# isunLt/U2MKD

Measured on AMD Instinct MI355X. Metric: LiDAR points/sec/node fwd+bwd (teacher+student+KD), 1/2/4/8 MI355X, higher is better.
Workload: dtype f32 (fp32 products emulated on the 16-bit matrix pipe: f16x2 forward / input gradient, bf16x3 weight gradient; fp32 accumulate)

## Files before the change

include/u2mkd_hip.h:

```cpp
#ifndef U2MKD_HIP_H
#define U2MKD_HIP_H

#include <stddef.h>
#include <stdint.h>

#ifdef __cplusplus
extern "C" {
#endif

typedef void *u2mkd_stream_t;

int u2mkd_version(void);
const char *u2mkd_last_error(void);
int u2mkd_stream_wait_stream(u2mkd_stream_t waiter, u2mkd_stream_t signaler);
void *u2mkd_mailbox_alloc(size_t bytes);
int u2mkd_mailbox_free(void *p);
int u2mkd_mailbox_post(const void *const *srcs, uint32_t is64, int32_t n, int64_t *slot, int64_t seq, u2mkd_stream_t s);

int u2mkd_hash(const int32_t *coords , int64_t n, int64_t *out , u2mkd_stream_t s);
int u2mkd_kernel_hash(const int32_t *coords , const int32_t *offsets , int64_t n,
                      int32_t k, int64_t *out , u2mkd_stream_t s);

size_t u2mkd_hash_table_bytes(int64_t n_refs);
int u2mkd_hash_table_build(const int64_t *refs, int64_t n_refs, void *table, u2mkd_stream_t s);
// ... 52 lines not shown
                                const int32_t *n_items, int64_t n_out, int32_t k, int32_t kflip, int32_t arith,
                                const float *scale , const float *shift , const float *res ,
                                int32_t relu, float *out, u2mkd_stream_t s);
int32_t u2mkd_pairs_gather_sum_stats_slab_rows(void);
int32_t u2mkd_pairs_gather_sum_stats_supported(int32_t cout);
int u2mkd_pairs_gather_sum_stats(const float *y, const int32_t *pos, int64_t n_rows, int32_t k, int32_t cout, float *out,
                                 float *partial, u2mkd_stream_t s);
int u2mkd_pairs_gather_sum_ep(const float *y, const int32_t *pos, int64_t n_rows, int32_t k, int32_t cout, const float *scale,
                              const float *shift, const float *res, int32_t relu, float *out, u2mkd_stream_t s);
int u2mkd_debug_conv_forward_sorted(const float *in, int64_t n_in, int32_t cin, const float *wt, int32_t cout,
                                    const int32_t *nbr_sorted, const int32_t *order, const int32_t *tile_order,
                                    int64_t n_out, int32_t k, int32_t kflip, int32_t variant, float *out,
                                    u2mkd_stream_t s);
int u2mkd_debug_conv_tile_pairs_stamps(const float *in, int64_t n_in, const void *wf ,
                                       const int32_t *nbr_sorted, const int32_t *order, const int32_t *items,
                                       const int32_t *n_items, int64_t n_out, int32_t k, int32_t arith, float *out,
                                       uint64_t *stamps, u2mkd_stream_t s);
int u2mkd_debug_wgrad_stamps(const float *a, const float *b, const int32_t *pairs, const int32_t *plan, int64_t n_rows,
                             int32_t k, void *workspace, uint64_t *stamps, u2mkd_stream_t s);
int u2mkd_conv_forward_pairs(const float *in, int64_t n_in, int32_t cin, const float *wt, int32_t cout,
                             const int32_t *pair_idx, const int32_t *tile_k, const int32_t *meta, int64_t capacity,
                             int32_t k, int32_t kc, float *y , u2mkd_stream_t s);
int32_t u2mkd_conv_pairs_x3_supported(int32_t cin, int32_t cout);
int u2mkd_conv_forward_pairs_x3(const float *in, int64_t n_in, int32_t cin, const void *wf, int32_t cout,
                                const int32_t *pair_idx, const int32_t *tile_k, const int32_t *meta, int64_t capacity,
                                int32_t k, float *y , u2mkd_stream_t s);
int u2mkd_linear_forward(const float *x , int64_t n, int32_t cin, const float *w , int32_t cout,
                         const float *bias , int32_t kc, float *y, u2mkd_stream_t s);
int u2mkd_linear_forward_x3(const float *x , int64_t n, int32_t cin, const void *wf, int32_t cout,
                            const float *bias , float *y , u2mkd_stream_t s);
int32_t u2mkd_conv_pairs_f16x2_supported(int32_t cin, int32_t cout);
int u2mkd_conv_forward_pairs_f16x2(const float *in, int64_t n_in, int32_t cin, const void *wf, int32_t cout,
                                    const int32_t *pair_idx, const int32_t *tile_k, const int32_t *meta, int64_t capacity,
                                    int32_t k, float *y, u2mkd_stream_t s);
int u2mkd_linear_forward_f16x2(const float *x, int64_t n, int32_t cin, const void *wf, int32_t cout, const float *bias,
                               float *y, u2mkd_stream_t s);
int u2mkd_pairs_gather_sum(const float *y, const int32_t *pos , int64_t n_rows, int32_t k, int32_t cout,
                           float *out , u2mkd_stream_t s);
int u2mkd_kmap_rowmask(const int32_t *nbr , int64_t n_out, int32_t k, int32_t *mask ,
                       u2mkd_stream_t s);
int u2mkd_conv_forward_tiles_bf16(const void *in , int64_t n_in, int32_t cin, const void *wf, int32_t cout,
                                  const int32_t *nbr_sorted, const int32_t *order, const int32_t *items,
                                  const int32_t *n_items, int64_t n_out, int32_t k, int32_t kflip,
                                  void *out , u2mkd_stream_t s);
int u2mkd_conv_wgrad_pairs_bf16(const void *a , int32_t ca, const void *b , int32_t cb,
                                const int32_t *pairs, const int32_t *plan, int64_t n_rows, int32_t k, int32_t swap,
                                void *workspace, size_t workspace_bytes, float *dw , u2mkd_stream_t s);
int u2mkd_conv_forward_tiles_f16(const void *in , int64_t n_in, int32_t cin, const void *wf, int32_t cout,
                                 const int32_t *nbr_sorted, const int32_t *order, const int32_t *items,
                                 const int32_t *n_items, int64_t n_out, int32_t k, int32_t kflip,
                                 void *out , u2mkd_stream_t s);
int u2mkd_conv_wgrad_pairs_f16(const void *a , int32_t ca, const void *b , int32_t cb,
                               const int32_t *pairs, const int32_t *plan, int64_t n_rows, int32_t k, int32_t swap,
                               void *workspace, size_t workspace_bytes, float *dw , u2mkd_stream_t s);
int u2mkd_conv_forward_pairs_f16(const void *in , int64_t n_in, int32_t cin, const void *wf, int32_t cout,
                                  const int32_t *pair_idx, const int32_t *tile_k, const int32_t *meta, int64_t capacity,
                                  int32_t k, void *y , u2mkd_stream_t s);
int u2mkd_linear_forward_f16(const void *x , int64_t n, int32_t cin, const void *wf, int32_t cout,
                             const float *bias , void *y , u2mkd_stream_t s);
int u2mkd_pairs_gather_sum_f16(const void *y , const int32_t *pos , int64_t n_rows, int32_t k,
                               int32_t cout, void *out , u2mkd_stream_t s);
int u2mkd_conv_forward_pairs_bf16(const void *in , int64_t n_in, int32_t cin, const void *wf, int32_t cout,
                                   const int32_t *pair_idx, const int32_t *tile_k, const int32_t *meta, int64_t capacity,
                                   int32_t k, void *y , u2mkd_stream_t s);
int u2mkd_linear_forward_bf16(const void *x , int64_t n, int32_t cin, const void *wf, int32_t cout,
                              const float *bias , void *y , u2mkd_stream_t s);
int u2mkd_pairs_gather_sum_bf16(const void *y , const int32_t *pos , int64_t n_rows, int32_t k,
                                int32_t cout, void *out , u2mkd_stream_t s);
size_t u2mkd_tile_schedule_workspace_bytes(int64_t n_rows);
int u2mkd_tile_schedule(const int32_t *mask , const int32_t *order , int64_t n_rows,
                        int32_t k, int32_t split0, int32_t split1, void *workspace, int32_t *tile_order,
                        int32_t *items, int32_t *n_items, u2mkd_stream_t s);
int32_t u2mkd_wgrad_plan_ints(int32_t k);
int u2mkd_wgrad_plan(const int32_t *nbsizes , int32_t k, int64_t n_rows, int32_t *plan, u2mkd_stream_t s);
size_t u2mkd_conv_wgrad_pairs_workspace_bytes(int64_t n_rows, int32_t ca, int32_t cb, int32_t k);
int u2mkd_conv_wgrad_pairs(const float *a, int32_t ca, const float *b, int32_t cb, const int32_t *pairs ,
                           const int32_t *plan, int64_t n_rows, int32_t k, int32_t swap, void *workspace,
                           size_t workspace_bytes, float *dw , u2mkd_stream_t s);

size_t u2mkd_convolution_workspace_bytes(int64_t n_in_rows, int64_t n_out_rows, int32_t cin, int32_t cout,
                                         const int32_t *nbsizes_host , int32_t k);
int u2mkd_convolution_forward(const float *in_feat , int64_t n_in_rows, int32_t cin,
                              float *out_feat , int64_t n_out_rows, int32_t cout,
                              const float *kernel , const int32_t *nbmaps ,
                              const int32_t *nbsizes_host , int32_t k, int32_t transpose, void *workspace,
                              size_t workspace_bytes, u2mkd_stream_t s);
int u2mkd_convolution_backward(const float *in_feat , int64_t n_in_rows, int32_t cin,
                               float *grad_in_feat , const float *grad_out_feat ,
                               int64_t n_out_rows, int32_t cout, const float *kernel ,
                               float *grad_kernel , const int32_t *nbmaps, const int32_t *nbsizes_host,
                               int32_t k, int32_t transpose, void *workspace, size_t workspace_bytes, u2mkd_stream_t s);

int u2mkd_count(const int32_t *idx , int64_t n, int32_t *counts , int64_t num,
                u2mkd_stream_t s);
int u2mkd_voxelize_forward(const float *feats , const int32_t *idx , const int32_t *counts ,
                           int64_t n, int64_t nv, int32_t c, float *out , u2mkd_stream_t s);
int u2mkd_voxelize_backward(const float *grad_out , const int32_t *idx, const int32_t *counts, int64_t n,
                            int64_t nv, int32_t c, float *grad_feats , u2mkd_stream_t s);
int u2mkd_devoxelize_forward(const float *feats , const int32_t *idx , const float *w ,
                             int64_t n, int32_t c, float *out , u2mkd_stream_t s);
int u2mkd_devoxelize_backward(const float *grad_out , const int32_t *idx , const float *w ,
                              int64_t n, int64_t nv, int32_t c, float *grad_feats ,
                              u2mkd_stream_t s);
int u2mkd_segment_sum(const float *src , int32_t c, const int32_t *entry_row ,
                      const float *entry_w , const int32_t *seg_offsets , int64_t nv,
                      int32_t mean, float *out , u2mkd_stream_t s);
int u2mkd_voxelize_backward_bf16(const void *grad_out , const int32_t *idx, const int32_t *counts, int64_t n,
                                 int64_t nv, int32_t c, void *grad_feats , u2mkd_stream_t s);
int u2mkd_devoxelize_forward_bf16(const void *feats , const int32_t *idx , const float *w ,
                                  int64_t n, int32_t c, void *out , u2mkd_stream_t s);
int u2mkd_segment_sum_bf16(const void *src , int32_t c, const int32_t *entry_row ,
                           const float *entry_w , const int32_t *seg_offsets , int64_t nv,
                           int32_t mean, void *out , u2mkd_stream_t s);
int u2mkd_voxelize_backward_f16(const void *grad_out , const int32_t *idx, const int32_t *counts, int64_t n,
                                int64_t nv, int32_t c, void *grad_feats , u2mkd_stream_t s);
int u2mkd_devoxelize_forward_f16(const void *feats , const int32_t *idx , const float *w ,
                                 int64_t n, int32_t c, void *out , u2mkd_stream_t s);
int u2mkd_segment_sum_f16(const void *src , int32_t c, const int32_t *entry_row ,
                          const float *entry_w , const int32_t *seg_offsets , int64_t nv,
                          int32_t mean, void *out , u2mkd_stream_t s);
size_t u2mkd_csr_workspace_bytes(int64_t n_entries, int64_t nv);
int u2mkd_csr_build(const int32_t *keys , int64_t n_entries, int64_t nv, void *workspace,
                    int32_t *order , int32_t *seg , u2mkd_stream_t s);
size_t u2mkd_devoxelize_plan_workspace_bytes(int64_t n, int64_t nv);
int u2mkd_devoxelize_plan(const int32_t *idx8 , const float *w8 , int64_t n, int64_t nv, void *workspace,
                          int32_t *entry_row , float *entry_w , int32_t *seg , u2mkd_stream_t s);
int u2mkd_ti_weights(const float *coords , const int64_t *idx_kn , int64_t n,
                     float scale, float *w_n8 , int32_t *idx_n8 , u2mkd_stream_t s);

int u2mkd_up_plan(const int32_t *idx8 , int64_t n, int32_t H, int32_t W, int32_t h, int32_t w, float rh, float rw,
                  int32_t *idx_out , float *w_out , u2mkd_stream_t s);
int u2mkd_upbn_stats(const float *x, int32_t n_img, int32_t c, int32_t h, int32_t w, const float *a, const float *b,
                     const float *ay, const float *ax, int32_t rows_per_chunk, float *partial, u2mkd_stream_t s);
int u2mkd_upbn_dense_grad(const float *x, int32_t n_img, int32_t c, int32_t h, int32_t w, const float *a, const float *b,
                          const float *ay, const float *ax, const float *c0 , const float *c1 ,
                          int32_t rows_per_chunk, float *dx, u2mkd_stream_t s);

int u2mkd_up_bilinear_forward(const float *x, const float *skip , int64_t planes, int32_t h, int32_t w, int32_t H,
                              int32_t W, float rh, float rw, float *y, u2mkd_stream_t s);
int u2mkd_up_bilinear_backward(const float *g, int64_t planes, int32_t h, int32_t w, int32_t H, int32_t W, const int32_t *taps_y,
                               const float *wy, const int32_t *taps_x, const float *wx, int32_t tiled, float *dx, u2mkd_stream_t s);

int u2mkd_maxpool3s2_forward(const float *x, int64_t planes, int32_t h, int32_t w, float *y, uint8_t *code, u2mkd_stream_t s);
int u2mkd_maxpool3s2_backward(const float *dy, const uint8_t *code, int64_t planes, int32_t h, int32_t w, float *dx,
                              u2mkd_stream_t s);

int u2mkd_transpose_batched(const float *in, float *out, int32_t batch, int32_t rows, int32_t cols, u2mkd_stream_t s);
int u2mkd_transpose_batched_scaled(const float *in, float *out, int32_t batch, int32_t rows, int32_t cols, float scale,
                                   u2mkd_stream_t s);

int u2mkd_l2c_combine_forward(const float *g0, const float *g1, const float *g2, const float *g3, int32_t n_grids, int32_t n_img,
                              int32_t h, int32_t w, int32_t c, int32_t ch1, int32_t cw1, int32_t ch2, int32_t cw2, int32_t ch3,
                              int32_t cw3, float *out_rows, u2mkd_stream_t s);
int u2mkd_l2c_combine_backward(const float *g_rows, int32_t n_img, int32_t h, int32_t w, int32_t c, int32_t ch, int32_t cw,
                               float *d_grid, u2mkd_stream_t s);

int32_t u2mkd_select_mse_partials(void);
int u2mkd_select_mse_forward(const float *gathered, const float *pseudo, const uint8_t *fov, int64_t n, int32_t c, float *out,
                             float *partial, float *stats, u2mkd_stream_t s);
int u2mkd_select_mse_backward(const float *g_out, const float *g_loss, const float *stats, const float *gathered,
                              const float *pseudo, const uint8_t *fov, int64_t n, int32_t c, float *d_gathered, float *d_pseudo,
                              u2mkd_stream_t s);
int u2mkd_lovasz_errors(const float *probas, const int64_t *labels, int32_t ignore_index, int64_t n, int32_t c, float *errors,
                        double *keys, u2mkd_stream_t s);
int u2mkd_lovasz_gather(const int64_t *perm, const int64_t *labels, int32_t ignore_index, int64_t n, int32_t c,
                        int32_t *fg_sorted, u2mkd_stream_t s);
int64_t u2mkd_lovasz_partials(int64_t n, int32_t c);
int u2mkd_lovasz_terms(const int64_t *perm, const float *errors, const int64_t *csum, const int32_t *fg_sorted, int64_t n,
                       int32_t c, float *jgrad, float *partial, float *stats, u2mkd_stream_t s);
int u2mkd_lovasz_backward(const float *g_out, const float *stats, const int64_t *perm, const float *jgrad, const float *probas,
                          const int64_t *labels, int32_t ignore_index, int64_t n, int32_t c, float *d_probas, u2mkd_stream_t s);
int64_t u2mkd_ce_partials(int64_t n);
int u2mkd_ce_forward(const float *x, const int64_t *labels, int32_t ignore_index, int64_t n, int32_t c, float *lse, float *partial,
                     float *stats, u2mkd_stream_t s);
int u2mkd_ce_backward(const float *g_out, const float *stats, const float *x, const float *lse, const int64_t *labels,
                      int32_t ignore_index, int64_t n, int32_t c, float *dx, u2mkd_stream_t s);
int u2mkd_kl_forward(const float *s_logits, const float *t_logits, const int64_t *t_index, int64_t n, int32_t c, float *rows,
                     float *partial, float *stats, u2mkd_stream_t s);
int u2mkd_kl_backward(const float *g_out, const float *s_logits, const float *t_logits, const int64_t *t_index, const float *rows,
                      int64_t n, int32_t c, float *ds, u2mkd_stream_t s);
int u2mkd_c2l_plan(const float *pixel_coords, const uint8_t *mask, int32_t ncam, int64_t n, int32_t sample, int32_t h,
                   int32_t w, int32_t *idx8 , float *w8 , u2mkd_stream_t s);
int u2mkd_l2c_keys(const float *pixel_coords, const uint8_t *mask, int32_t ncam, int64_t n, int32_t sample, int64_t row0,
                   int64_t e0, int32_t ch, int32_t cw, int32_t *pix, int32_t *key_d, int32_t *key_s, int32_t *row,
                   u2mkd_stream_t s);
int u2mkd_l2c_finish(const int32_t *order_d, const int32_t *seg_d, const int32_t *order_s, const int32_t *pix,
                     const int32_t *row, int64_t n_entries, int32_t *fwd_row, float *fwd_w, int32_t *bwd_pix, float *bwd_w,
                     u2mkd_stream_t s);

int64_t u2mkd_bn_num_slabs(int64_t n);
int u2mkd_bn_train_forward(const void *x, const void *res, int32_t row_dtype, int64_t n, int32_t c, const float *gamma,
                           const float *beta, float eps, float momentum, float *running_mean, float *running_var,
                           int64_t *num_batches_tracked, int32_t relu, float *partial, float *mean ,
                           float *invstd , void *y, u2mkd_stream_t s);
int u2mkd_bn_train_forward_from_partial(const float *x, const float *res, int64_t n, int32_t c, const float *gamma,
                                        const float *beta, float eps, float momentum, float *running_mean, float *running_var,
                                        int64_t *num_batches_tracked, int32_t relu, const float *partial, int32_t slab_rows,
                                        float *mean , float *invstd , float *y, u2mkd_stream_t s);
int u2mkd_bn_eval_forward(const void *x, const void *res, int32_t row_dtype, int64_t n, int32_t c, const float *gamma,
                          const float *beta, float eps, const float *running_mean, const float *running_var, int32_t relu,
                          float *invstd , void *y, u2mkd_stream_t s);
int u2mkd_bn_backward(const void *dy, const void *x, const void *res, int32_t row_dtype, int64_t n, int32_t c,
                      const float *mean, const float *invstd, const float *gamma, const float *beta, int32_t relu,
                      int32_t training, float *partial, float *dgamma , float *dbeta , void *dx, void *dres,
                      u2mkd_stream_t s);

int u2mkd_bn_local_stats(const void *x, int32_t row_dtype, int64_t n, int32_t c, float *partial ,
                         float *stats , u2mkd_stream_t s);
int u2mkd_bn_merge_stats(const float *gathered , int32_t world, int32_t c, float eps, float momentum,
                         float *running_mean, float *running_var, float *mean , float *invstd ,
                         float *total , int64_t *num_batches_tracked, u2mkd_stream_t s);
int u2mkd_bn_apply(const void *x, const void *res, int32_t row_dtype, int64_t n, int32_t c, const float *mean,
                   const float *invstd, const float *gamma, const float *beta, int32_t relu, void *y, u2mkd_stream_t s);
int u2mkd_bn_backward_local(const void *dy, const void *x, const void *res, int32_t row_dtype, int64_t n, int32_t c,
                            const float *mean, const float *invstd, const float *gamma, const float *beta, int32_t relu,
                            float *partial , float *sums , float *keep ,
                            u2mkd_stream_t s);
int u2mkd_bn_backward_apply(const void *dy, const void *x, const void *res, int32_t row_dtype, int64_t n, int32_t c,
                            const float *total_n , const float *mean, const float *invstd, const float *gamma,
                            const float *beta, int32_t relu, const float *sums , void *dx, void *dres,
                            u2mkd_stream_t s);

int u2mkd_sptr_window_keys(const float *xyz , const int32_t *batch , int64_t n, const float *lo4,
                           const float *hi4, float sx, float sy, float sz, int64_t *keys , u2mkd_stream_t s);
size_t u2mkd_sptr_plan_prepare_workspace_bytes(void);
int u2mkd_sptr_plan_prepare(const float *xyz , const int32_t *batch , int64_t n, float cx, float cy, float cz,
                            float sx, float sy, float sz, float *sphere, float *bounds, int64_t *keys_cubic,
                            int64_t *keys_sphere, void *workspace, u2mkd_stream_t s);
int u2mkd_sptr_window_ranges(const int64_t *sorted_keys, int64_t n, int32_t *wstart , int32_t *wlen ,
                             u2mkd_stream_t s);
int u2mkd_sptr_quant_coords(const float *xyz , const int32_t *sort_idx , int64_t n, const float *lo,
                            float wx, float wy, float wz, float qx, float qy, float qz, int32_t *qc ,
                            float *radial , u2mkd_stream_t s);
int u2mkd_sptr_attention_forward(const float *q, const float *k, const float *v, const int32_t *sort_idx,
                                 const int32_t *wstart, const int32_t *wlen, const int32_t *qc, const float *radial,
                                 const float *tq, const float *tk, const float *tv, int32_t L, int32_t qgl,
                                 float split_a, int64_t n, int32_t h, int32_t hdim, float *out, float *lse,
                                 u2mkd_stream_t s);
size_t u2mkd_sptr_backward_workspace_bytes(int64_t n, int32_t h, int32_t L);
int u2mkd_sptr_attention_backward(const float *q, const float *k, const float *v, const float *out, const float *dout,
                                  const float *lse, const int32_t *sort_idx, const int32_t *wstart,
                                  const int32_t *wlen, const int32_t *qc, const float *radial, const float *tq,
                                  const float *tk, const float *tv, int32_t L, int32_t qgl, float split_a,
                                  int32_t qc_span, int64_t n, int32_t h, int32_t hdim, float *delta ,
                                  void *workspace, size_t workspace_bytes, float *dq, float *dk, float *dv, float *dtq,
                                  float *dtk, float *dtv, u2mkd_stream_t s);
int u2mkd_sptr_attention_forward_strided(const float *q, const float *k, const float *v, int64_t ld_qkv, float q_scale,
                                         const int32_t *sort_idx, const int32_t *wstart, const int32_t *wlen,
                                         const int32_t *qc, const float *radial, const float *tq, const float *tk,
                                         const float *tv, int32_t L, int32_t qgl, float split_a, int64_t n, int32_t h,
                                         int32_t hdim, float *out, int64_t ld_out, float *lse, u2mkd_stream_t s);
int u2mkd_sptr_attention_backward_strided(const float *q, const float *k, const float *v, int64_t ld_qkv, float q_scale,
                                          const float *out, const float *dout, int64_t ld_out, const float *lse,
                                          const int32_t *sort_idx, const int32_t *wstart, const int32_t *wlen,
                                          const int32_t *qc, const float *radial, const float *tq, const float *tk,
                                          const float *tv, int32_t L, int32_t qgl, float split_a, int32_t qc_span,
                                          int64_t n, int32_t h, int32_t hdim, float *delta ,
                                          void *workspace, size_t workspace_bytes, float *dq, float *dk, float *dv,
                                          int64_t ld_grad, float *dtq, float *dtk, float *dtv, u2mkd_stream_t s);

int u2mkd_sptr_table_reduce(const void *workspace, int64_t n, int32_t h, int32_t L, float split_a, float *dtq, float *dtk,
                            float *dtv, u2mkd_stream_t s);

int u2mkd_sptr_precompute_all(int32_t N, int32_t n, uint32_t n_max, const int32_t *counts, const int32_t *offsets,
                              const int32_t *sq_offsets, int32_t *index_0_offsets, int32_t *index_1_offsets,
                              int32_t *index_0, int32_t *index_1, u2mkd_stream_t s);
int u2mkd_sptr_attention_step1_forward(int32_t N_q, int32_t N_k, int32_t M, int32_t h, int32_t hdim, uint32_t n_max,
                                       const float *q, const float *k, const int32_t *index0, const int32_t *index1,
                                       float *attn, u2mkd_stream_t s);
int u2mkd_sptr_attention_step1_backward(int32_t N, int32_t M, int32_t h, int32_t hdim, uint32_t n_max,
                                        const float *grad_out, const int32_t *index0, const int32_t *index0_offsets,
                                        const int32_t *index1, const int32_t *index1_offsets, const float *q,
                                        const float *k, float *grad_q, float *grad_k, u2mkd_stream_t s);
int u2mkd_sptr_attention_step2_forward(int32_t N, int32_t M, int32_t h, int32_t hdim, int32_t n_max, const float *attn,
                                       const float *v, const int32_t *index0_offsets, const int32_t *index1,
                                       float *output, u2mkd_stream_t s);
int u2mkd_sptr_attention_step2_backward(int32_t N, int32_t M, int32_t h, int32_t hdim, int32_t n_max,
                                        const float *grad_out, const int32_t *index0, const int32_t *index0_offsets,
                                        const int32_t *index1, const int32_t *index1_offsets, const float *attn,
                                        const float *v, float *grad_attn, float *grad_v, u2mkd_stream_t s);
int u2mkd_sptr_dot_prod_with_idx_forward(int32_t N, int32_t M, int32_t h, int32_t hdim, int32_t n_max, int32_t L,
                                         const float *q, const int32_t *index_q, const int32_t *index_q_offsets,
                                         const float *k, const int32_t *index_k, const float *table_q,
                                         const float *table_k, const int32_t *rel_idx, float *output,
                                         u2mkd_stream_t s);
int u2mkd_sptr_dot_prod_with_idx_all_forward(int32_t N, int32_t M, int32_t h, int32_t hdim, int32_t n_max, int32_t L,
                                             const float *q, const int32_t *index_q, const int32_t *index_q_offsets,
                                             const float *k, const int32_t *index_k, const float *table_q,
                                             const float *table_k, const int32_t *rel_idx, float *output,
                                             u2mkd_stream_t s);
int u2mkd_sptr_dot_prod_with_idx_backward(int32_t N, int32_t M, int32_t h, int32_t hdim, int32_t n_max, int32_t L,
                                          const float *grad_out, const float *q, const int32_t *index_q_offsets,
                                          const float *k, const int32_t *index_k_offsets, const int32_t *index_k,
                                          const float *table_q, const float *table_k, const int32_t *rel_idx,
                                          float *grad_q, float *grad_k, float *grad_table_q, float *grad_table_k,
                                          u2mkd_stream_t s);
int u2mkd_sptr_attention_step2_with_rel_pos_value_forward(int32_t N, int32_t M, int32_t h, int32_t hdim, int32_t n_max,
                                                          const float *attn, const float *v,
                                                          const int32_t *index0_offsets, const int32_t *index1,
                                                          const float *table, const int32_t *rel_idx, float *output,
                                                          u2mkd_stream_t s);
int u2mkd_sptr_attention_step2_with_rel_pos_value_backward(int32_t N, int32_t M, int32_t h, int32_t hdim, int32_t L,
                                                           int32_t n_max, const float *grad_out, const int32_t *index0,
                                                           const int32_t *index0_offsets, const int32_t *index1,
                                                           const int32_t *index1_offsets, const float *attn,
                                                           const float *v, const float *table, const int32_t *rel_idx,
                                                           float *grad_attn, float *grad_v, float *grad_table,
                                                           u2mkd_stream_t s);
// ... 47 lines not shown
```

u2mkd_amd/_lib.py:

```python
from __future__ import annotations

import ctypes as C
import os

import torch

_HERE = os.path.dirname(os.path.abspath(__file__))
LIB_PATH = os.path.join(_HERE, 'lib', 'libu2mkd_hip%s.so' % os.environ.get('U2MKD_LIB_SUFFIX', ''))

_i32, _i64, _sz, _f32, _p = C.c_int32, C.c_int64, C.c_size_t, C.c_float, C.c_void_p

SIGNATURES = {
    'u2mkd_version': (C.c_int, []),
    'u2mkd_last_error': (C.c_char_p, []),
    'u2mkd_hash': (C.c_int, [_p, _i64, _p, _p]),
    'u2mkd_kernel_hash': (C.c_int, [_p, _p, _i64, _i32, _p, _p]),
    'u2mkd_hash_table_bytes': (_sz, [_i64]),
    'u2mkd_hash_table_build': (C.c_int, [_p, _i64, _p, _p]),
    'u2mkd_hash_table_query': (C.c_int, [_p, _i64, _p, _i64, _p, _p]),
    'u2mkd_hash_table_query2': (C.c_int, [_p, _i64, _p, _i64, _p, _p, _p]),
    'u2mkd_kmap_build_table': (C.c_int, [_p, _i64, _p, _i64, _p, _i32, _p, _p]),
    'u2mkd_kmap_invert': (C.c_int, [_p, _i64, _i32, _i64, _p, _p]),
    'u2mkd_kmap_sizes': (C.c_int, [_p, _i64, _i32, _p, _p, _p]),
    'u2mkd_kmap_compact': (C.c_int, [_p, _i64, _i32, _p, _p, _p, _p]),
    'u2mkd_downsample_keys': (C.c_int, [_p, _i64, _i32, _i32, _i32, _p, _p]),
    'u2mkd_downsample_keys_checked': (C.c_int, [_p, _i64, _i32, _i32, _i32, _p, _p, _p]),
    'u2mkd_downsample_keys_general': (C.c_int, [_p, _i64] + [_i32] * 9 + [_p, _i32, _p, _p, _p]),
    'u2mkd_floor_coords': (C.c_int, [_p, _i64, _i32, _p, _p]),
    'u2mkd_unpack_keys': (C.c_int, [_p, _i64, _p, _p]),
    'u2mkd_transpose_weights': (C.c_int, [_p, _i32, _i32, _i32, _p, _p]),
    'u2mkd_conv_forward': (C.c_int, [_p, _i64, _i32, _p, _i32, _p, _i64, _i32, _i32, _p, _p]),
    'u2mkd_conv_forward_sorted': (C.c_int, [_p, _i64, _i32, _p, _i32, _p, _p, _p, _i64, _i32, _i32, _p, _p]),
    'u2mkd_debug_conv_forward_sorted': (C.c_int, [_p, _i64, _i32, _p, _i32, _p, _p, _p, _i64, _i32, _i32, _i32, _p, _p]),
    'u2mkd_stream_wait_stream': (C.c_int, [_p, _p]),
    'u2mkd_sgd_chunk_elements': (_i32, []),
    'u2mkd_sgd_batch': (C.c_int, [_p, _i32, _i64, _f32, _f32, _f32, _i32, _i32, _p]),
    'u2mkd_grads_unscale_check': (C.c_int, [_p, _i32, _i64, _p, _p, _p]),
    'u2mkd_sgd_batch_amp': (C.c_int, [_p, _i32, _i64, _f32, _f32, _f32, _i32, _i32, _p, _p, _p]),
    'u2mkd_mailbox_alloc': (_p, [_sz]),
    'u2mkd_mailbox_free': (C.c_int, [_p]),
    'u2mkd_mailbox_post': (C.c_int, [_p, C.c_uint32, _i32, _p, _i64, _p]),
    'u2mkd_conv_tiles_supported': (_i32, [_i32, _i32, _i32]),
    'u2mkd_conv_tiles_arith': (_i32, [_i32, _i32, _i32]),
    'u2mkd_weight_fragments_bytes': (_sz, [_i32, _i32, _i32, _i32]),
    'u2mkd_weight_fragments': (C.c_int, [_p, _i32, _i32, _i32, _i32, _i32, _p, _p]),
    'u2mkd_weight_fragments_batch': (C.c_int, [_p, _i32, _i64, _p]),
    'u2mkd_conv_forward_tiles': (C.c_int, [_p, _i64, _i32, _p, _i32, _p, _p, _p, _p, _i64, _i32, _i32, _i32, _p, _p]),
    'u2mkd_conv_forward_tiles_ep': (C.c_int, [_p, _i64, _i32, _p, _i32, _p, _p, _p, _p, _i64, _i32, _i32, _i32, _p, _p, _p, _i32, _p, _p]),
    'u2mkd_pairs_gather_sum_ep': (C.c_int, [_p, _p, _i64, _i32, _i32, _p, _p, _p, _i32, _p, _p]),
    'u2mkd_pairs_gather_sum_stats_slab_rows': (_i32, []),
    'u2mkd_pairs_gather_sum_stats_supported': (_i32, [_i32]),
    'u2mkd_pairs_gather_sum_stats': (C.c_int, [_p, _p, _i64, _i32, _i32, _p, _p, _p]),
    'u2mkd_debug_conv_tile_pairs_stamps': (C.c_int, [_p, _i64, _p, _p, _p, _p, _p, _i64, _i32, _i32, _p, _p, _p]),
    'u2mkd_debug_wgrad_stamps': (C.c_int, [_p, _p, _p, _p, _i64, _i32, _p, _p, _p]),
    'u2mkd_conv_forward_pairs': (C.c_int, [_p, _i64, _i32, _p, _i32, _p, _p, _p, _i64, _i32, _i32, _p, _p]),
    'u2mkd_conv_pairs_x3_supported': (_i32, [_i32, _i32]),
    'u2mkd_conv_forward_pairs_x3': (C.c_int, [_p, _i64, _i32, _p, _i32, _p, _p, _p, _i64, _i32, _p, _p]),
    'u2mkd_linear_forward': (C.c_int, [_p, _i64, _i32, _p, _i32, _p, _i32, _p, _p]),
    'u2mkd_bn2d_workspace_bytes': (C.c_size_t, [_i64, _i32, _i64]),
    'u2mkd_bn2d_train_forward': (C.c_int, [_p, _p, _i64, _i32, _i64, _p, _p, C.c_float, C.c_float, _i32, _p, _p, _p, _p, _p, _p, _p, _p]),
    'u2mkd_bn2d_eval_forward': (C.c_int, [_p, _p, _i64, _i32, _i64, _p, _p, C.c_float, _i32, _p, _p, _p, _p]),
    'u2mkd_bn2d_backward': (C.c_int, [_p, _p, _p, _i64, _i32, _i64, _p, _p, _p, _p, _i32, _i32, _p, _p, _p, _p, _p, _p]),
    'u2mkd_bn2d_local_stats': (C.c_int, [_p, _i64, _i32, _i64, _p, _p, _p]),
    'u2mkd_bn2d_apply': (C.c_int, [_p, _p, _i64, _i32, _i64, _p, _p, _p, _p, _i32, _p, _p]),
    'u2mkd_bn2d_backward_local': (C.c_int, [_p, _p, _p, _i64, _i32, _i64, _p, _p, _p, _p, _i32, _p, _p, _p, _p]),
    'u2mkd_bn2d_backward_apply': (C.c_int, [_p, _p, _p, _i64, _i32, _i64, _p, _p, _p, _p, _p, _i32, _p, _p, _p, _p]),
    'u2mkd_linear_forward_x3': (C.c_int, [_p, _i64, _i32, _p, _i32, _p, _p, _p]),
    'u2mkd_conv_pairs_f16x2_supported': (_i32, [_i32, _i32]),
    'u2mkd_conv_forward_pairs_f16x2': (C.c_int, [_p, _i64, _i32, _p, _i32, _p, _p, _p, _i64, _i32, _p, _p]),
    'u2mkd_linear_forward_f16x2': (C.c_int, [_p, _i64, _i32, _p, _i32, _p, _p, _p]),
    'u2mkd_pairs_capacity': (_i64, [_i64, _i64, _i32]),
    'u2mkd_pairs_build': (C.c_int, [_p, _i64, _i64, _i32, _p, _p, _p, _p, _p, _p, _p, _p, _p]),
    'u2mkd_pairs_gather_sum': (C.c_int, [_p, _p, _i64, _i32, _i32, _p, _p]),
    'u2mkd_kmap_rowmask': (C.c_int, [_p, _i64, _i32, _p, _p]),
    'u2mkd_tile_schedule_workspace_bytes': (_sz, [_i64]),
    'u2mkd_tile_schedule': (C.c_int, [_p, _p, _i64, _i32, _i32, _i32, _p, _p, _p, _p, _p]),
    'u2mkd_wgrad_plan_ints': (_i32, [_i32]),
    'u2mkd_wgrad_plan': (C.c_int, [_p, _i32, _i64, _p, _p]),
    'u2mkd_conv_wgrad_pairs_workspace_bytes': (_sz, [_i64, _i32, _i32, _i32]),
    'u2mkd_conv_wgrad_pairs': (C.c_int, [_p, _i32, _p, _i32, _p, _p, _i64, _i32, _i32, _p, _sz, _p, _p]),
    'u2mkd_conv_forward_tiles_bf16': (C.c_int, [_p, _i64, _i32, _p, _i32, _p, _p, _p, _p, _i64, _i32, _i32, _p, _p]),
    'u2mkd_conv_forward_tiles_f16': (C.c_int, [_p, _i64, _i32, _p, _i32, _p, _p, _p, _p, _i64, _i32, _i32, _p, _p]),
    'u2mkd_conv_wgrad_pairs_bf16': (C.c_int, [_p, _i32, _p, _i32, _p, _p, _i64, _i32, _i32, _p, _sz, _p, _p]),
    'u2mkd_conv_wgrad_pairs_f16': (C.c_int, [_p, _i32, _p, _i32, _p, _p, _i64, _i32, _i32, _p, _sz, _p, _p]),
    'u2mkd_conv_forward_pairs_bf16': (C.c_int, [_p, _i64, _i32, _p, _i32, _p, _p, _p, _i64, _i32, _p, _p]),
    'u2mkd_conv_forward_pairs_f16': (C.c_int, [_p, _i64, _i32, _p, _i32, _p, _p, _p, _i64, _i32, _p, _p]),
    'u2mkd_linear_forward_bf16': (C.c_int, [_p, _i64, _i32, _p, _i32, _p, _p, _p]),
    'u2mkd_linear_forward_f16': (C.c_int, [_p, _i64, _i32, _p, _i32, _p, _p, _p]),
    'u2mkd_pairs_gather_sum_bf16': (C.c_int, [_p, _p, _i64, _i32, _i32, _p, _p]),
    'u2mkd_pairs_gather_sum_f16': (C.c_int, [_p, _p, _i64, _i32, _i32, _p, _p]),
    'u2mkd_convolution_workspace_bytes': (_sz, [_i64, _i64, _i32, _i32, _p, _i32]),
    'u2mkd_convolution_forward': (C.c_int, [_p, _i64, _i32, _p, _i64, _i32, _p, _p, _p, _i32, _i32, _p, _sz, _p]),
    'u2mkd_convolution_backward': (C.c_int, [_p, _i64, _i32, _p, _p, _i64, _i32, _p, _p, _p, _p, _i32, _i32, _p, _sz, _p]),
    'u2mkd_bn_num_slabs': (_i64, [_i64]),
    'u2mkd_bn_train_forward': (C.c_int, [_p, _p, _i32, _i64, _i32, _p, _p, _f32, _f32, _p, _p, _p, _i32, _p, _p, _p, _p, _p]),
    'u2mkd_bn_train_forward_from_partial': (C.c_int, [_p, _p, _i64, _i32, _p, _p, _f32, _f32, _p, _p, _p, _i32, _p, _i32, _p, _p, _p, _p]),
    'u2mkd_bn_eval_forward': (C.c_int, [_p, _p, _i32, _i64, _i32, _p, _p, _f32, _p, _p, _i32, _p, _p, _p]),
    'u2mkd_bn_backward': (C.c_int, [_p, _p, _p, _i32, _i64, _i32, _p, _p, _p, _p, _i32, _i32, _p, _p, _p, _p, _p, _p]),
    'u2mkd_bn_local_stats': (C.c_int, [_p, _i32, _i64, _i32, _p, _p, _p]),
    'u2mkd_bn_merge_stats': (C.c_int, [_p, _i32, _i32, _f32, _f32, _p, _p, _p, _p, _p, _p, _p]),
    'u2mkd_bn_apply': (C.c_int, [_p, _p, _i32, _i64, _i32, _p, _p, _p, _p, _i32, _p, _p]),
    'u2mkd_bn_backward_local': (C.c_int, [_p, _p, _p, _i32, _i64, _i32, _p, _p, _p, _p, _i32, _p, _p, _p, _p]),
    'u2mkd_bn_backward_apply': (C.c_int, [_p, _p, _p, _i32, _i64, _i32, _p, _p, _p, _p, _p, _i32, _p, _p, _p, _p]),
    'u2mkd_sptr_window_keys': (C.c_int, [_p, _p, _i64, _p, _p, _f32, _f32, _f32, _p, _p]),
    'u2mkd_select_mse_partials': (_i32, []),
    'u2mkd_select_mse_forward': (C.c_int, [_p, _p, _p, _i64, _i32, _p, _p, _p, _p]),
    'u2mkd_select_mse_backward': (C.c_int, [_p, _p, _p, _p, _p, _p, _i64, _i32, _p, _p, _p]),
    'u2mkd_sptr_plan_prepare_workspace_bytes': (_sz, []),
    'u2mkd_sptr_plan_prepare': (C.c_int, [_p, _p, _i64, _f32, _f32, _f32, _f32, _f32, _f32, _p, _p, _p, _p, _p, _p]),
    'u2mkd_sptr_window_ranges': (C.c_int, [_p, _i64, _p, _p, _p]),
    'u2mkd_sptr_quant_coords': (C.c_int, [_p, _p, _i64, _p, _f32, _f32, _f32, _f32, _f32, _f32, _p, _p, _p]),
    'u2mkd_sptr_attention_forward': (C.c_int, [_p, _p, _p, _p, _p, _p, _p, _p, _p, _p, _p, _i32, _i32, _f32, _i64, _i32, _i32, _p, _p, _p]),
    'u2mkd_sptr_backward_workspace_bytes': (_sz, [_i64, _i32, _i32]),
    'u2mkd_sptr_attention_backward': (C.c_int, [_p] * 14 + [_i32, _i32, _f32, _i32, _i64, _i32, _i32] + [_p, _p, _sz] + [_p] * 7),
    'u2mkd_sptr_tiles_workspace_bytes': (_sz, [_i64, _i32]),
    'u2mkd_sptr_attention_forward_tiles': (C.c_int, [_p, _p, _p, _i64, _f32] + [_p] * 8 + [_i32, _i32, _f32, _i64, _i32, _i32, _p, _i64, _p, _p, _sz, _p]),
    'u2mkd_sptr_attention_forward_strided': (C.c_int, [_p, _p, _p, _i64, _f32] + [_p] * 8 + [_i32, _i32, _f32, _i64, _i32, _i32, _p, _i64, _p, _p]),
    'u2mkd_sptr_attention_backward_strided': (C.c_int, [_p, _p, _p, _i64, _f32, _p, _p, _i64] + [_p] * 9 + [_i32, _i32, _f32, _i32, _i64, _i32, _i32]
                                              + [_p, _p, _sz] + [_p, _p, _p, _i64, _p, _p, _p, _p]),
    'u2mkd_sptr_table_reduce': (C.c_int, [_p, _i64, _i32, _i32, _f32, _p, _p, _p, _p]),
    'u2mkd_sptr_precompute_all': (C.c_int, [_i32, _i32, C.c_uint32] + [_p] * 8),
    'u2mkd_sptr_attention_step1_forward': (C.c_int, [_i32, _i32, _i32, _i32, _i32, C.c_uint32] + [_p] * 6),
    'u2mkd_sptr_attention_step1_backward': (C.c_int, [_i32, _i32, _i32, _i32, C.c_uint32] + [_p] * 10),
    'u2mkd_sptr_attention_step2_forward': (C.c_int, [_i32] * 5 + [_p] * 6),
    'u2mkd_sptr_attention_step2_backward': (C.c_int, [_i32] * 5 + [_p] * 10),
    'u2mkd_sptr_dot_prod_with_idx_forward': (C.c_int, [_i32] * 6 + [_p] * 10),
    'u2mkd_sptr_dot_prod_with_idx_all_forward': (C.c_int, [_i32] * 6 + [_p] * 10),
    'u2mkd_sptr_dot_prod_with_idx_backward': (C.c_int, [_i32] * 6 + [_p] * 14),
    'u2mkd_sptr_attention_step2_with_rel_pos_value_forward': (C.c_int, [_i32] * 5 + [_p] * 8),
    'u2mkd_sptr_attention_step2_with_rel_pos_value_backward': (C.c_int, [_i32] * 6 + [_p] * 13),
    'u2mkd_count': (C.c_int, [_p, _i64, _p, _i64, _p]),
    'u2mkd_voxelize_forward': (C.c_int, [_p, _p, _p, _i64, _i64, _i32, _p, _p]),
    'u2mkd_voxelize_backward': (C.c_int, [_p, _p, _p, _i64, _i64, _i32, _p, _p]),
    'u2mkd_devoxelize_forward': (C.c_int, [_p, _p, _p, _i64, _i32, _p, _p]),
    'u2mkd_devoxelize_backward': (C.c_int, [_p, _p, _p, _i64, _i64, _i32, _p, _p]),
    'u2mkd_segment_sum': (C.c_int, [_p, _i32, _p, _p, _p, _i64, _i32, _p, _p]),
    'u2mkd_voxelize_backward_bf16': (C.c_int, [_p, _p, _p, _i64, _i64, _i32, _p, _p]),
    'u2mkd_voxelize_backward_f16': (C.c_int, [_p, _p, _p, _i64, _i64, _i32, _p, _p]),
    'u2mkd_devoxelize_forward_bf16': (C.c_int, [_p, _p, _p, _i64, _i32, _p, _p]),
    'u2mkd_devoxelize_forward_f16': (C.c_int, [_p, _p, _p, _i64, _i32, _p, _p]),
    'u2mkd_segment_sum_bf16': (C.c_int, [_p, _i32, _p, _p, _p, _i64, _i32, _p, _p]),
    'u2mkd_segment_sum_f16': (C.c_int, [_p, _i32, _p, _p, _p, _i64, _i32, _p, _p]),
    'u2mkd_c2l_plan': (C.c_int, [_p, _p, _i32, _i64, _i32, _i32, _i32, _p, _p, _p]),
    'u2mkd_l2c_keys': (C.c_int, [_p, _p, _i32, _i64, _i32, _i64, _i64, _i32, _i32, _p, _p, _p, _p, _p]),
    'u2mkd_l2c_finish': (C.c_int, [_p, _p, _p, _p, _p, _i64, _p, _p, _p, _p, _p]),
    'u2mkd_up_bilinear_forward': (C.c_int, [_p, _p, _i64, _i32, _i32, _i32, _i32, _f32, _f32, _p, _p]),
    'u2mkd_up_bilinear_backward': (C.c_int, [_p, _i64, _i32, _i32, _i32, _i32, _p, _p, _p, _p, _i32, _p, _p]),
    'u2mkd_maxpool3s2_forward': (C.c_int, [_p, _i64, _i32, _i32, _p, _p, _p]),
    'u2mkd_maxpool3s2_backward': (C.c_int, [_p, _p, _i64, _i32, _i32, _p, _p]),
    'u2mkd_transpose_batched': (C.c_int, [_p, _p, _i32, _i32, _i32, _p]),
    'u2mkd_transpose_batched_scaled': (C.c_int, [_p, _p, _i32, _i32, _i32, C.c_float, _p]),
    'u2mkd_l2c_combine_forward': (C.c_int, [_p, _p, _p, _p] + [_i32] * 11 + [_p, _p]),
    'u2mkd_l2c_combine_backward': (C.c_int, [_p] + [_i32] * 6 + [_p, _p]),
    'u2mkd_up_plan': (C.c_int, [_p, _i64, _i32, _i32, _i32, _i32, _f32, _f32, _p, _p, _p]),
    'u2mkd_upbn_stats': (C.c_int, [_p, _i32, _i32, _i32, _i32, _p, _p, _p, _p, _i32, _p, _p]),
    'u2mkd_upbn_dense_grad': (C.c_int, [_p, _i32, _i32, _i32, _i32, _p, _p, _p, _p, _p, _p, _i32, _p, _p]),
    'u2mkd_csr_workspace_bytes': (_sz, [_i64, _i64]),
    'u2mkd_lovasz_errors': (C.c_int, [_p, _p, _i32, _i64, _i32, _p, _p, _p]),
    'u2mkd_lovasz_gather': (C.c_int, [_p, _p, _i32, _i64, _i32, _p, _p]),
    'u2mkd_lovasz_partials': (_i64, [_i64, _i32]),
    'u2mkd_lovasz_terms': (C.c_int, [_p, _p, _p, _p, _i64, _i32, _p, _p, _p, _p]),
    'u2mkd_ce_partials': (_i64, [_i64]),
    'u2mkd_ce_forward': (C.c_int, [_p, _p, _i32, _i64, _i32, _p, _p, _p, _p]),
    'u2mkd_ce_backward': (C.c_int, [_p, _p, _p, _p, _p, _i32, _i64, _i32, _p, _p]),
    'u2mkd_kl_forward': (C.c_int, [_p, _p, _p, _i64, _i32, _p, _p, _p, _p]),
    'u2mkd_kl_backward': (C.c_int, [_p, _p, _p, _p, _p, _i64, _i32, _p, _p]),
    'u2mkd_lovasz_backward': (C.c_int, [_p, _p, _p, _p, _p, _p, _i32, _i64, _i32, _p, _p]),
    'u2mkd_csr_build': (C.c_int, [_p, _i64, _i64, _p, _p, _p, _p]),
    'u2mkd_devoxelize_plan_workspace_bytes': (C.c_size_t, [_i64, _i64]),
    'u2mkd_devoxelize_plan': (C.c_int, [_p, _p, _i64, _i64, _p, _p, _p, _p, _p]),
    'u2mkd_ti_weights': (C.c_int, [_p, _p, _i64, _f32, _p, _p, _p]),
}

_lib = None
_raw_stream = torch._C._cuda_getCurrentRawStream
_current_device = torch._C._cuda_getDevice


def load():
    global _lib
    if _lib is not None:
        return _lib
    if not os.path.exists(LIB_PATH):
        raise RuntimeError(
            f'{LIB_PATH} is missing: build it with `python -m u2mkd_amd.build` '
            '(u2mkd_amd has no CPU or PyTorch fallback path)')
    lib = C.CDLL(LIB_PATH)
    for name, (res, args) in SIGNATURES.items():
        fn = getattr(lib, name)
        fn.restype = res
        fn.argtypes = args
    _lib = lib
    return lib


def stream() -> int:
    return _raw_stream(_current_device())


def ptr(t):
    if t is None:
        return None
    return t.data_ptr()


_fns = {}


def call(name: str, *args):
    fn = _fns.get(name)
    if fn is None:
        fn = _fns[name] = getattr(load(), name)
    rc = fn(*args)
    if rc != 0:
        msg = load().u2mkd_last_error().decode('utf-8', 'replace')
        raise RuntimeError(f'{name} failed (rc={rc}): {msg}')


def require_cuda(*tensors):
    for t in tensors:
        if t is not None and not t.is_cuda:
            raise RuntimeError('u2mkd_amd operators run on the HIP device only (got a CPU tensor); '
                               'there is no CPU fallback')
```

u2mkd_amd/csrc/bn.hip:

```cpp
#include "common.h"

#include <cstdlib>

namespace u2mkd {

constexpr int kBnThreads = 256;
constexpr int kBnSlabRows = 128;

struct BnLayout {
    int c4, rl;
};
__device__ __forceinline__ BnLayout bn_layout(int c) {
    BnLayout l;
    l.c4 = c >> 2;
    l.rl = kBnThreads / l.c4;
    if (l.rl < 1) l.rl = 1;
    return l;
}

constexpr int kBnRegRows = 16;

template <typename T>
__global__ void __launch_bounds__(kBnThreads)
bn_stats_partial_reg_kernel(const T *__restrict__ x, int64_t n, int c, float *__restrict__ partial) {
// ... 244 lines not shown
    const int nloop = (c4 + kBnThreads - 1) / kBnThreads;
    const int64_t r0 = (int64_t)blockIdx.x * kBnSlabRows;
    const int rows = (int)min((int64_t)kBnSlabRows, n - r0);
    for (int it = 0; it < nloop; ++it) {
        const int rl = c4 >= kBnThreads ? 1 : kBnThreads / c4;
        const int j = c4 >= kBnThreads ? it * kBnThreads + threadIdx.x : threadIdx.x % c4;
        const int ry = c4 >= kBnThreads ? 0 : threadIdx.x / c4;
        const bool live = j < c4 && ry < rl;
        const int cw = c4 >= kBnThreads ? kBnThreads : c4;
        const int jl = c4 >= kBnThreads ? threadIdx.x : j;
        float4 s1 = make_float4(0.f, 0.f, 0.f, 0.f), s2 = s1;
        if (live) {
            float4 m = *reinterpret_cast<const float4 *>(mean + 4 * j);
            float4 is = *reinterpret_cast<const float4 *>(invstd + 4 * j);
            float4 g = gamma ? *reinterpret_cast<const float4 *>(gamma + 4 * j) : make_float4(1.f, 1.f, 1.f, 1.f);
            float4 b = beta ? *reinterpret_cast<const float4 *>(beta + 4 * j) : make_float4(0.f, 0.f, 0.f, 0.f);
            for (int rr0 = ry; rr0 < rows; rr0 += 4 * rl) {
                float4 vv[4], dd[4], rr4[4];
#pragma unroll
                for (int u = 0; u < 4; ++u) {
                    const int rr = rr0 + u * rl;
                    const bool ok = rr < rows;
                    vv[u] = ok ? ld4(x, (r0 + rr) * c4 + j) : make_float4(0.f, 0.f, 0.f, 0.f);
                    dd[u] = ok ? ld4(dy, (r0 + rr) * c4 + j) : make_float4(0.f, 0.f, 0.f, 0.f);
                    rr4[u] = (ok && relu && res) ? ld4(res, (r0 + rr) * c4 + j) : make_float4(0.f, 0.f, 0.f, 0.f);
                }
#pragma unroll
                for (int u = 0; u < 4; ++u) {
                    if (rr0 + u * rl >= rows) break;
                    const float4 v = vv[u], rv = rr4[u];
                    float4 d = dd[u];
                    float hx = (v.x - m.x) * is.x, hy = (v.y - m.y) * is.y, hz = (v.z - m.z) * is.z, hw = (v.w - m.w) * is.w;
                    if (relu) {
                        if (hx * g.x + b.x + rv.x <= 0.f) d.x = 0.f;
                        if (hy * g.y + b.y + rv.y <= 0.f) d.y = 0.f;
                        if (hz * g.z + b.z + rv.z <= 0.f) d.z = 0.f;
                        if (hw * g.w + b.w + rv.w <= 0.f) d.w = 0.f;
                    }
                    s1.x += d.x; s1.y += d.y; s1.z += d.z; s1.w += d.w;
                    s2.x += d.x * hx; s2.y += d.y * hy; s2.z += d.z * hz; s2.w += d.w * hw;
                }
            }
            red[ry * cw + jl] = s1;
            red[(rl + ry) * cw + jl] = s2;
        }
        __syncthreads();
        if (live && ry == 0) {
            float4 t1 = make_float4(0.f, 0.f, 0.f, 0.f), t2 = t1;
            for (int gq = 0; gq < rl; ++gq) {
                float4 a = red[gq * cw + jl], bq = red[(rl + gq) * cw + jl];
                t1.x += a.x; t1.y += a.y; t1.z += a.z; t1.w += a.w;
                t2.x += bq.x; t2.y += bq.y; t2.z += bq.z; t2.w += bq.w;
            }
            float *p = partial + (size_t)blockIdx.x * 2 * c;
            *reinterpret_cast<float4 *>(p + 4 * j) = t1;
            *reinterpret_cast<float4 *>(p + c + 4 * j) = t2;
        }
        __syncthreads();
    }
}

__global__ void __launch_bounds__(256)
bn_bwd_finalize_kernel(const float *__restrict__ partial, int nslab, int c, float *__restrict__ dbeta,
                       float *__restrict__ dgamma, float *__restrict__ keep = nullptr) {
    __shared__ float s_1[kBnFinLanes][kBnFinCh], s_2[kBnFinLanes][kBnFinCh];
    const int cl = threadIdx.x & (kBnFinCh - 1), g = threadIdx.x / kBnFinCh;
    const int ch = blockIdx.x * kBnFinCh + cl;
    float s1 = 0.f, s2 = 0.f;
    if (ch < c) {
        for (int b0 = g; b0 < nslab; b0 += 4 * kBnFinLanes) {
            float p1[4], p2[4];
#pragma unroll
            for (int u = 0; u < 4; ++u) {
                int b = b0 + u * kBnFinLanes;
                p1[u] = b < nslab ? partial[(size_t)b * 2 * c + ch] : 0.f;
                p2[u] = b < nslab ? partial[(size_t)b * 2 * c + c + ch] : 0.f;
            }
#pragma unroll
            for (int u = 0; u < 4; ++u) { s1 += p1[u]; s2 += p2[u]; }
        }
    }
    s_1[g][cl] = s1; s_2[g][cl] = s2;
    __syncthreads();
    if (g != 0 || ch >= c) return;
    for (int i = 1; i < kBnFinLanes; ++i) { s1 += s_1[i][cl]; s2 += s_2[i][cl]; }
    dbeta[ch] = s1;
    dgamma[ch] = s2;
    if (keep) { keep[ch] = s1; keep[c + ch] = s2; }
}

template <typename T>
__global__ void bn_bwd_apply_kernel(const T *__restrict__ dy, const T *__restrict__ x, int64_t total4, int c4,
                                    float inv_n_host, const float *__restrict__ total_n,
                                    const float *__restrict__ mean, const float *__restrict__ invstd,
                                    const float *__restrict__ gamma, const float *__restrict__ beta, int relu,
                                    const float *__restrict__ dbeta, const float *__restrict__ dgamma,
                                    T *__restrict__ dx, const T *__restrict__ res = nullptr,
                                    T *__restrict__ dres = nullptr) {
    int64_t t = (int64_t)blockIdx.x * blockDim.x + threadIdx.x;
    if (t >= total4) return;
    const float inv_n = total_n ? 1.f / *total_n : inv_n_host;
    int j = (int)(t % c4) * 4;
    float4 v = ld4(x, t);
    float4 d = ld4(dy, t);
    float4 m = *reinterpret_cast<const float4 *>(mean + j);
    float4 is = *reinterpret_cast<const float4 *>(invstd + j);
    float4 g = gamma ? *reinterpret_cast<const float4 *>(gamma + j) : make_float4(1.f, 1.f, 1.f, 1.f);
    float4 b = beta ? *reinterpret_cast<const float4 *>(beta + j) : make_float4(0.f, 0.f, 0.f, 0.f);
    float4 db = *reinterpret_cast<const float4 *>(dbeta + j);
    float4 dg = *reinterpret_cast<const float4 *>(dgamma + j);
    float hx = (v.x - m.x) * is.x, hy = (v.y - m.y) * is.y, hz = (v.z - m.z) * is.z, hw = (v.w - m.w) * is.w;
    if (relu) {
        const float4 rv = res ? ld4(res, t) : make_float4(0.f, 0.f, 0.f, 0.f);
        if (hx * g.x + b.x + rv.x <= 0.f) d.x = 0.f;
        if (hy * g.y + b.y + rv.y <= 0.f) d.y = 0.f;
        if (hz * g.z + b.z + rv.z <= 0.f) d.z = 0.f;
        if (hw * g.w + b.w + rv.w <= 0.f) d.w = 0.f;
    }
    if (dres) st4(dres, t, d);
    float4 o;
    o.x = g.x * is.x * (d.x - db.x * inv_n - hx * dg.x * inv_n);
    o.y = g.y * is.y * (d.y - db.y * inv_n - hy * dg.y * inv_n);
    o.z = g.z * is.z * (d.z - db.z * inv_n - hz * dg.z * inv_n);
    o.w = g.w * is.w * (d.w - db.w * inv_n - hw * dg.w * inv_n);
    st4(dx, t, o);
}

template <typename T>
__global__ void bn_bwd_eval_kernel(const T *__restrict__ dy, const T *__restrict__ x, int64_t total4, int c4,
                                   const float *__restrict__ mean, const float *__restrict__ invstd,
                                   const float *__restrict__ gamma, const float *__restrict__ beta, int relu,
                                   T *__restrict__ dx, const T *__restrict__ res = nullptr,
                                   T *__restrict__ dres = nullptr) {
    int64_t t = (int64_t)blockIdx.x * blockDim.x + threadIdx.x;
    if (t >= total4) return;
    int j = (int)(t % c4) * 4;
    float4 v = ld4(x, t);
    float4 d = ld4(dy, t);
    float4 m = *reinterpret_cast<const float4 *>(mean + j);
    float4 is = *reinterpret_cast<const float4 *>(invstd + j);
    float4 g = gamma ? *reinterpret_cast<const float4 *>(gamma + j) : make_float4(1.f, 1.f, 1.f, 1.f);
    float4 b = beta ? *reinterpret_cast<const float4 *>(beta + j) : make_float4(0.f, 0.f, 0.f, 0.f);
    if (relu) {
        const float4 rv = res ? ld4(res, t) : make_float4(0.f, 0.f, 0.f, 0.f);
        if ((v.x - m.x) * is.x * g.x + b.x + rv.x <= 0.f) d.x = 0.f;
        if ((v.y - m.y) * is.y * g.y + b.y + rv.y <= 0.f) d.y = 0.f;
        if ((v.z - m.z) * is.z * g.z + b.z + rv.z <= 0.f) d.z = 0.f;
        if ((v.w - m.w) * is.w * g.w + b.w + rv.w <= 0.f) d.w = 0.f;
    }
    if (dres) st4(dres, t, d);
    st4(dx, t, make_float4(d.x * g.x * is.x, d.y * g.y * is.y, d.z * g.z * is.z, d.w * g.w * is.w));
}

__global__ void bn_invstd_kernel(const float *__restrict__ var, int c, float eps, float *__restrict__ invstd) {
    int ch = blockIdx.x * blockDim.x + threadIdx.x;
    if (ch < c) invstd[ch] = 1.f / sqrtf(var[ch] + eps);
}

__global__ void bn_sync_merge_kernel(const float *__restrict__ gathered, int world, int c, float eps, float momentum,
                                     float *__restrict__ running_mean, float *__restrict__ running_var,
                                     float *__restrict__ mean_out, float *__restrict__ invstd_out,
                                     float *__restrict__ total_out, int64_t *__restrict__ num_batches_tracked = nullptr) {
    int ch = blockIdx.x * blockDim.x + threadIdx.x;
    if (num_batches_tracked && ch == 0) *num_batches_tracked += 1;
    if (ch >= c) return;
    const int row = 2 * c + 1;
    float na = 0.f, mean = 0.f, m2 = 0.f;
    for (int r = 0; r < world; ++r) {
        float nb = gathered[(size_t)r * row + 2 * c];
        if (nb == 0.f) continue;
        float mb = gathered[(size_t)r * row + ch], qb = gathered[(size_t)r * row + c + ch];
        float tot = na + nb;
        float delta = mb - mean;
        mean += delta * (nb / tot);
        m2 += qb + delta * delta * (na * nb / tot);
        na = tot;
    }
    float var = na > 0.f ? m2 / na : 0.f;
    mean_out[ch] = mean;
    invstd_out[ch] = 1.f / sqrtf(var + eps);
    if (ch == 0) *total_out = na;
    if (running_mean) {
        float unbiased = na > 1.f ? m2 / (na - 1.f) : var;
        running_mean[ch] = (1.f - momentum) * running_mean[ch] + momentum * mean;
        running_var[ch] = (1.f - momentum) * running_var[ch] + momentum * unbiased;
    }
}

static size_t bn_lds_bytes(int c, int arrays) {
    int c4 = c / 4;
    int rl = c4 >= kBnThreads ? 1 : kBnThreads / c4;
    int cw = c4 >= kBnThreads ? kBnThreads : c4;
    return (size_t)arrays * rl * cw * sizeof(float4);
}

static bool bn_stats_serial() {
    static const bool on = [] { const char *e = getenv("U2MKD_BN_STATS_SERIAL"); return e && e[0] == '1'; }();
    return on;
}

template <typename T>
static void bn_launch_stats_partial(hipStream_t st, int nslab, const T *x, int64_t n, int c, float *partial) {
    const int c4 = c / 4;
    if (c4 <= 32 && kBnSlabRows / (kBnThreads / c4) <= kBnRegRows && !bn_stats_serial())
        hipLaunchKernelGGL(bn_stats_partial_reg_kernel<T>, dim3(nslab), dim3(kBnThreads), bn_lds_bytes(c, 1), st, x, n, c, partial);
    else
        hipLaunchKernelGGL(bn_stats_partial_kernel<T>, dim3(nslab), dim3(kBnThreads), bn_lds_bytes(c, 1), st, x, n, c, partial);
}

template <typename T>
static int bn_train_forward_impl(const T *x, const T *res, int64_t n, int32_t c, const float *gamma, const float *beta,
                                 float eps, float momentum, float *running_mean, float *running_var,
                                 int64_t *num_batches_tracked, int32_t relu, float *partial, float *mean, float *invstd, T *y,
                                 u2mkd_stream_t s) {
    U2_REQUIRE(c > 0 && c % 4 == 0 && c <= 1024, "u2mkd_bn_train_forward: c=%d must be a multiple of 4 in 4..1024", c);
    U2_REQUIRE(n > 0, "u2mkd_bn_train_forward: empty batch (n=%lld)", (long long)n);
    U2_REQUIRE(x && partial && mean && invstd && y, "u2mkd_bn_train_forward: null pointer");
    hipStream_t st = as_stream(s);
    int nslab = (int)u2mkd_bn_num_slabs(n);
#ifndef U2MKD_EXP_SKIP_BN_STATS
    bn_launch_stats_partial<T>(st, nslab, x, n, c, partial);
#endif
    hipLaunchKernelGGL(bn_stats_finalize_kernel, dim3((unsigned)ceil_div(c, kBnFinCh)), dim3(256), 0, st, partial, nslab, n, c,
                       eps, momentum, running_mean, running_var, mean, invstd, (float *)nullptr, num_batches_tracked);
    int64_t total4 = n * (c / 4);
    hipLaunchKernelGGL(bn_apply_kernel<T>, dim3((unsigned)ceil_div(total4, 256)), dim3(256), 0, st, x, total4, c / 4, mean,
                       invstd, gamma, beta, relu, y, res);
    return check_launch("u2mkd_bn_train_forward");
}

static int bn_train_forward_from_partial_impl(const float *x, const float *res, int64_t n, int32_t c, const float *gamma,
                                              const float *beta, float eps, float momentum, float *running_mean,
                                              float *running_var, int64_t *num_batches_tracked, int32_t relu,
                                              const float *partial, int32_t slab_rows, float *mean, float *invstd, float *y,
                                              u2mkd_stream_t s) {
    U2_REQUIRE(c > 0 && c % 4 == 0 && c <= 1024, "u2mkd_bn_train_forward_from_partial: c=%d must be a multiple of 4 in 4..1024", c);
    U2_REQUIRE(n > 0 && slab_rows > 0, "u2mkd_bn_train_forward_from_partial: n=%lld rows in slabs of %d", (long long)n, slab_rows);
    U2_REQUIRE(x && partial && mean && invstd && y, "u2mkd_bn_train_forward_from_partial: null pointer");
    U2_REQUIRE(res == nullptr || relu, "u2mkd_bn_train_forward_from_partial: a residual input is only fused with the ReLU form");
    hipStream_t st = as_stream(s);
    const int64_t nslab = ceil_div(n, (int64_t)slab_rows);
    U2_REQUIRE(nslab < ((int64_t)1 << 31), "u2mkd_bn_train_forward_from_partial: too many slabs");
    hipLaunchKernelGGL(bn_stats_finalize_kernel, dim3((unsigned)ceil_div(c, kBnFinCh)), dim3(256), 0, st, partial, (int)nslab, n, c,
                       eps, momentum, running_mean, running_var, mean, invstd, (float *)nullptr, num_batches_tracked, (int)slab_rows);
    int64_t total4 = n * (c / 4);
    hipLaunchKernelGGL(bn_apply_kernel<float>, dim3((unsigned)ceil_div(total4, 256)), dim3(256), 0, st, x, total4, c / 4, mean,
                       invstd, gamma, beta, relu, y, res);
    return check_launch("u2mkd_bn_train_forward_from_partial");
}

template <typename T>
static int bn_eval_forward_impl(const T *x, const T *res, int64_t n, int32_t c, const float *gamma, const float *beta,
                                float eps, const float *running_mean, const float *running_var, int32_t relu, float *invstd,
                                T *y, u2mkd_stream_t s) {
    U2_REQUIRE(c > 0 && c % 4 == 0, "u2mkd_bn_eval_forward: c=%d must be a positive multiple of 4", c);
    if (n == 0) return 0;
    U2_REQUIRE(x && running_mean && running_var && invstd && y, "u2mkd_bn_eval_forward: null pointer");
    hipStream_t st = as_stream(s);
    int64_t total4 = n * (c / 4);
    hipLaunchKernelGGL(bn_apply_eval_kernel<T>, dim3((unsigned)ceil_div(total4, 256)), dim3(256), 0, st, x, total4, c / 4,
                       running_mean, running_var, eps, gamma, beta, relu, invstd, y, res);
    return check_launch("u2mkd_bn_eval_forward");
}

template <typename T>
static int bn_backward_impl(const T *dy, const T *x, const T *res, int64_t n, int32_t c, const float *mean,
                            const float *invstd, const float *gamma, const float *beta, int32_t relu, int32_t training,
                            float *partial, float *dgamma, float *dbeta, T *dx, T *dres, u2mkd_stream_t s) {
    U2_REQUIRE(c > 0 && c % 4 == 0 && c <= 1024, "u2mkd_bn_backward: c=%d must be a multiple of 4 in 4..1024", c);
    U2_REQUIRE((res == nullptr) == (dres == nullptr), "u2mkd_bn_backward: res and dres go together");
    U2_REQUIRE(res == nullptr || relu, "u2mkd_bn_backward: a residual input is only fused with the ReLU form");
    if (n == 0) return 0;
    U2_REQUIRE(dy && x && mean && invstd && partial && dgamma && dbeta && dx, "u2mkd_bn_backward: null pointer");
    hipStream_t st = as_stream(s);
    int nslab = (int)u2mkd_bn_num_slabs(n);
    hipLaunchKernelGGL(bn_bwd_partial_kernel<T>, dim3(nslab), dim3(kBnThreads), bn_lds_bytes(c, 2), st, dy, x, n, c, mean,
                       invstd, gamma, beta, relu, partial, res);
    hipLaunchKernelGGL(bn_bwd_finalize_kernel, dim3((unsigned)ceil_div(c, kBnFinCh)), dim3(256), 0, st, partial, nslab, c,
                       dbeta, dgamma);
    int64_t total4 = n * (c / 4);
    if (training)
        hipLaunchKernelGGL(bn_bwd_apply_kernel<T>, dim3((unsigned)ceil_div(total4, 256)), dim3(256), 0, st, dy, x, total4,
                           c / 4, 1.f / (float)n, (const float *)nullptr, mean, invstd, gamma, beta, relu, dbeta, dgamma,
                           dx, res, dres);
    else
        hipLaunchKernelGGL(bn_bwd_eval_kernel<T>, dim3((unsigned)ceil_div(total4, 256)), dim3(256), 0, st, dy, x, total4,
                           c / 4, mean, invstd, gamma, beta, relu, dx, res, dres);
    return check_launch("u2mkd_bn_backward");
}

template <typename T>
static int bn_local_stats_impl(const T *x, int64_t n, int32_t c, float *partial, float *stats, u2mkd_stream_t s) {
    U2_REQUIRE(c > 0 && c % 4 == 0 && c <= 1024, "u2mkd_bn_local_stats: c=%d must be a multiple of 4 in 4..1024", c);
    U2_REQUIRE(stats && (n == 0 || (x && partial)), "u2mkd_bn_local_stats: null pointer");
    hipStream_t st = as_stream(s);
    if (n == 0) {
        (void)hipMemsetAsync(stats, 0, (size_t)(2 * c + 1) * sizeof(float), st);
        return check_launch("u2mkd_bn_local_stats");
    }
    int nslab = (int)u2mkd_bn_num_slabs(n);
    bn_launch_stats_partial<T>(st, nslab, x, n, c, partial);
    hipLaunchKernelGGL(bn_stats_finalize_kernel, dim3((unsigned)ceil_div(c, kBnFinCh)), dim3(256), 0, st, partial, nslab,
                       n, c, 0.f, 0.f, (float *)nullptr, (float *)nullptr, stats, (float *)nullptr, stats + c);
    return check_launch("u2mkd_bn_local_stats");
}

template <typename T>
static int bn_apply_impl(const T *x, const T *res, int64_t n, int32_t c, const float *mean, const float *invstd,
                         const float *gamma, const float *beta, int32_t relu, T *y, u2mkd_stream_t s) {
    U2_REQUIRE(c > 0 && c % 4 == 0, "u2mkd_bn_apply: c=%d must be a positive multiple of 4", c);
    if (n == 0) return 0;
    U2_REQUIRE(x && mean && invstd && y, "u2mkd_bn_apply: null pointer");
    int64_t total4 = n * (c / 4);
    hipLaunchKernelGGL(bn_apply_kernel<T>, dim3((unsigned)ceil_div(total4, 256)), dim3(256), 0, as_stream(s), x, total4,
                       c / 4, mean, invstd, gamma, beta, relu, y, res);
    return check_launch("u2mkd_bn_apply");
}

template <typename T>
static int bn_backward_local_impl(const T *dy, const T *x, const T *res, int64_t n, int32_t c, const float *mean,
                                  const float *invstd, const float *gamma, const float *beta, int32_t relu, float *partial,
                                  float *sums, float *keep, u2mkd_stream_t s) {
    U2_REQUIRE(c > 0 && c % 4 == 0 && c <= 1024, "u2mkd_bn_backward_local: c=%d must be a multiple of 4 in 4..1024", c);
    U2_REQUIRE(sums, "u2mkd_bn_backward_local: null pointer");
    hipStream_t st = as_stream(s);
    if (n == 0) {
        (void)hipMemsetAsync(sums, 0, (size_t)2 * c * sizeof(float), st);
        if (keep) (void)hipMemsetAsync(keep, 0, (size_t)2 * c * sizeof(float), st);
        return check_launch("u2mkd_bn_backward_local");
    }
    U2_REQUIRE(dy && x && mean && invstd && partial, "u2mkd_bn_backward_local: null pointer");
    int nslab = (int)u2mkd_bn_num_slabs(n);
    hipLaunchKernelGGL(bn_bwd_partial_kernel<T>, dim3(nslab), dim3(kBnThreads), bn_lds_bytes(c, 2), st, dy, x, n, c, mean,
                       invstd, gamma, beta, relu, partial, res);
    hipLaunchKernelGGL(bn_bwd_finalize_kernel, dim3((unsigned)ceil_div(c, kBnFinCh)), dim3(256), 0, st, partial, nslab, c,
                       sums, sums + c, keep);
    return check_launch("u2mkd_bn_backward_local");
}

template <typename T>
static int bn_backward_apply_impl(const T *dy, const T *x, const T *res, int64_t n, int32_t c, const float *total_n,
                                  const float *mean, const float *invstd, const float *gamma, const float *beta, int32_t relu,
                                  const float *sums, T *dx, T *dres, u2mkd_stream_t s) {
    U2_REQUIRE(c > 0 && c % 4 == 0, "u2mkd_bn_backward_apply: c=%d must be a positive multiple of 4", c);
    if (n == 0) return 0;
    U2_REQUIRE(dy && x && total_n && mean && invstd && sums && dx, "u2mkd_bn_backward_apply: null pointer");
    int64_t total4 = n * (c / 4);
    hipLaunchKernelGGL(bn_bwd_apply_kernel<T>, dim3((unsigned)ceil_div(total4, 256)), dim3(256), 0, as_stream(s), dy, x,
                       total4, c / 4, 0.f, total_n, mean, invstd, gamma, beta, relu, sums, sums + c, dx, res, dres);
    return check_launch("u2mkd_bn_backward_apply");
}

}

using namespace u2mkd;

#define BF(p) reinterpret_cast<const bf16row *>(p)
#define BFW(p) reinterpret_cast<bf16row *>(p)
#define H16(p) reinterpret_cast<const _Float16 *>(p)
#define H16W(p) reinterpret_cast<_Float16 *>(p)
#define U2_ROW_DTYPE(who) U2_REQUIRE(row_dtype >= 0 && row_dtype <= 2, who ": row dtype %d must be 0 (fp32), 1 (bf16) or 2 (fp16)", row_dtype)
#define F32(p) reinterpret_cast<const float *>(p)
#define F32W(p) reinterpret_cast<float *>(p)

extern "C" {

int64_t u2mkd_bn_num_slabs(int64_t n) { return n > 0 ? (n + kBnSlabRows - 1) / kBnSlabRows : 0; }

int u2mkd_bn_train_forward(const void *x, const void *res, int32_t row_dtype, int64_t n, int32_t c, const float *gamma,
                           const float *beta, float eps, float momentum, float *running_mean, float *running_var,
                           int64_t *num_batches_tracked, int32_t relu, float *partial, float *mean, float *invstd, void *y,
                           u2mkd_stream_t s) {
    U2_ROW_DTYPE("u2mkd_bn_train_forward");
    if (row_dtype == 2)
        return bn_train_forward_impl<_Float16>(H16(x), H16(res), n, c, gamma, beta, eps, momentum, running_mean, running_var,
                                              num_batches_tracked, relu, partial, mean, invstd, H16W(y), s);
    if (row_dtype == 1)
        return bn_train_forward_impl<bf16row>(BF(x), BF(res), n, c, gamma, beta, eps, momentum, running_mean, running_var,
                                              num_batches_tracked, relu, partial, mean, invstd, BFW(y), s);
    return bn_train_forward_impl<float>(F32(x), F32(res), n, c, gamma, beta, eps, momentum, running_mean, running_var,
                                        num_batches_tracked, relu, partial, mean, invstd, F32W(y), s);
}

int u2mkd_bn_train_forward_from_partial(const float *x, const float *res, int64_t n, int32_t c, const float *gamma,
                                        const float *beta, float eps, float momentum, float *running_mean, float *running_var,
                                        int64_t *num_batches_tracked, int32_t relu, const float *partial, int32_t slab_rows,
                                        float *mean, float *invstd, float *y, u2mkd_stream_t s) {
    return bn_train_forward_from_partial_impl(x, res, n, c, gamma, beta, eps, momentum, running_mean, running_var,
                                              num_batches_tracked, relu, partial, slab_rows, mean, invstd, y, s);
}

int u2mkd_bn_eval_forward(const void *x, const void *res, int32_t row_dtype, int64_t n, int32_t c, const float *gamma,
                          const float *beta, float eps, const float *running_mean, const float *running_var, int32_t relu,
                          float *invstd, void *y, u2mkd_stream_t s) {
    U2_ROW_DTYPE("u2mkd_bn_eval_forward");
    if (row_dtype == 2)
        return bn_eval_forward_impl<_Float16>(H16(x), H16(res), n, c, gamma, beta, eps, running_mean, running_var, relu, invstd,
                                             H16W(y), s);
    if (row_dtype == 1)
        return bn_eval_forward_impl<bf16row>(BF(x), BF(res), n, c, gamma, beta, eps, running_mean, running_var, relu, invstd,
                                             BFW(y), s);
    return bn_eval_forward_impl<float>(F32(x), F32(res), n, c, gamma, beta, eps, running_mean, running_var, relu, invstd,
                                       F32W(y), s);
}

int u2mkd_bn_backward(const void *dy, const void *x, const void *res, int32_t row_dtype, int64_t n, int32_t c,
                      const float *mean, const float *invstd, const float *gamma, const float *beta, int32_t relu,
                      int32_t training, float *partial, float *dgamma, float *dbeta, void *dx, void *dres, u2mkd_stream_t s) {
    U2_ROW_DTYPE("u2mkd_bn_backward");
    if (row_dtype == 2)
        return bn_backward_impl<_Float16>(H16(dy), H16(x), H16(res), n, c, mean, invstd, gamma, beta, relu, training, partial,
                                         dgamma, dbeta, H16W(dx), H16W(dres), s);
    if (row_dtype == 1)
        return bn_backward_impl<bf16row>(BF(dy), BF(x), BF(res), n, c, mean, invstd, gamma, beta, relu, training, partial,
                                         dgamma, dbeta, BFW(dx), BFW(dres), s);
    return bn_backward_impl<float>(F32(dy), F32(x), F32(res), n, c, mean, invstd, gamma, beta, relu, training, partial, dgamma,
                                   dbeta, F32W(dx), F32W(dres), s);
}

int u2mkd_bn_local_stats(const void *x, int32_t row_dtype, int64_t n, int32_t c, float *partial, float *stats,
                         u2mkd_stream_t s) {
    U2_ROW_DTYPE("u2mkd_bn_local_stats");
    if (row_dtype == 2) return bn_local_stats_impl<_Float16>(H16(x), n, c, partial, stats, s);
    if (row_dtype == 1) return bn_local_stats_impl<bf16row>(BF(x), n, c, partial, stats, s);
    return bn_local_stats_impl<float>(F32(x), n, c, partial, stats, s);
}

int u2mkd_bn_merge_stats(const float *gathered, int32_t world, int32_t c, float eps, float momentum, float *running_mean,
                         float *running_var, float *mean, float *invstd, float *total, int64_t *num_batches_tracked,
                         u2mkd_stream_t s) {
    U2_REQUIRE(gathered && mean && invstd && total && world > 0 && c > 0, "u2mkd_bn_merge_stats: bad arguments");
    hipLaunchKernelGGL(bn_sync_merge_kernel, dim3((unsigned)ceil_div(c, 64)), dim3(64), 0, as_stream(s), gathered, world, c,
                       eps, momentum, running_mean, running_var, mean, invstd, total, num_batches_tracked);
    return check_launch("u2mkd_bn_merge_stats");
}

int u2mkd_bn_apply(const void *x, const void *res, int32_t row_dtype, int64_t n, int32_t c, const float *mean,
                   const float *invstd, const float *gamma, const float *beta, int32_t relu, void *y, u2mkd_stream_t s) {
    U2_ROW_DTYPE("u2mkd_bn_apply");
    if (row_dtype == 2) return bn_apply_impl<_Float16>(H16(x), H16(res), n, c, mean, invstd, gamma, beta, relu, H16W(y), s);
    if (row_dtype == 1) return bn_apply_impl<bf16row>(BF(x), BF(res), n, c, mean, invstd, gamma, beta, relu, BFW(y), s);
    return bn_apply_impl<float>(F32(x), F32(res), n, c, mean, invstd, gamma, beta, relu, F32W(y), s);
}

int u2mkd_bn_backward_local(const void *dy, const void *x, const void *res, int32_t row_dtype, int64_t n, int32_t c,
                            const float *mean, const float *invstd, const float *gamma, const float *beta, int32_t relu,
                            float *partial, float *sums, float *keep, u2mkd_stream_t s) {
    U2_ROW_DTYPE("u2mkd_bn_backward_local");
    if (row_dtype == 2)
        return bn_backward_local_impl<_Float16>(H16(dy), H16(x), H16(res), n, c, mean, invstd, gamma, beta, relu, partial, sums,
                                               keep, s);
    if (row_dtype == 1)
        return bn_backward_local_impl<bf16row>(BF(dy), BF(x), BF(res), n, c, mean, invstd, gamma, beta, relu, partial, sums,
                                               keep, s);
    return bn_backward_local_impl<float>(F32(dy), F32(x), F32(res), n, c, mean, invstd, gamma, beta, relu, partial, sums, keep,
                                         s);
}

int u2mkd_bn_backward_apply(const void *dy, const void *x, const void *res, int32_t row_dtype, int64_t n, int32_t c,
                            const float *total_n, const float *mean, const float *invstd, const float *gamma,
                            const float *beta, int32_t relu, const float *sums, void *dx, void *dres, u2mkd_stream_t s) {
    U2_ROW_DTYPE("u2mkd_bn_backward_apply");
    if (row_dtype == 2)
        return bn_backward_apply_impl<_Float16>(H16(dy), H16(x), H16(res), n, c, total_n, mean, invstd, gamma, beta, relu, sums,
                                               H16W(dx), H16W(dres), s);
    if (row_dtype == 1)
        return bn_backward_apply_impl<bf16row>(BF(dy), BF(x), BF(res), n, c, total_n, mean, invstd, gamma, beta, relu, sums,
                                               BFW(dx), BFW(dres), s);
    return bn_backward_apply_impl<float>(F32(dy), F32(x), F32(res), n, c, total_n, mean, invstd, gamma, beta, relu, sums,
                                         F32W(dx), F32W(dres), s);
}

}
```

u2mkd_amd/csrc/pixhead.hip:

```cpp
#include "common.h"

namespace u2mkd {

constexpr int kPhThreads = 256;

__global__ void __launch_bounds__(kPhThreads)
up_plan_kernel(const int32_t *__restrict__ idx8, int64_t n, int H, int W, int h, int w, float rh, float rw,
               int32_t *__restrict__ idx_out, float *__restrict__ w_out) {
#pragma clang fp contract(off)
    const int64_t t = (int64_t)blockIdx.x * blockDim.x + threadIdx.x;
    if (t >= n * 4) return;
    const int64_t f = idx8[(t >> 2) * 8 + (t & 3)];
    int32_t *oi = idx_out + t * 8;
    float *ow = w_out + t * 8;
#pragma unroll
    for (int s = 0; s < 8; ++s) { oi[s] = -1; ow[s] = 0.f; }
    if (f < 0) return;
    const int64_t hw_full = (int64_t)H * W;
    const int64_t img = f / hw_full;
    const int rem = (int)(f - img * hw_full);
    const int y = rem / W, x = rem - y * W;
    const float h1r = rh * (float)y, w1r = rw * (float)x;
    const int h1 = (int)h1r, w1 = (int)w1r;
    const int h1p = h1 < h - 1 ? 1 : 0, w1p = w1 < w - 1 ? 1 : 0;
    const float hl1 = h1r - (float)h1, wl1 = w1r - (float)w1;
    const float hl0 = 1.f - hl1, wl0 = 1.f - wl1;
    const int64_t base = img * (int64_t)h * w;
    oi[0] = (int32_t)(base + (int64_t)h1 * w + w1);                 ow[0] = hl0 * wl0;
    oi[1] = (int32_t)(base + (int64_t)h1 * w + w1 + w1p);           ow[1] = hl0 * wl1;
    oi[2] = (int32_t)(base + (int64_t)(h1 + h1p) * w + w1);         ow[2] = hl1 * wl0;
    oi[3] = (int32_t)(base + (int64_t)(h1 + h1p) * w + w1 + w1p);   ow[3] = hl1 * wl1;
}

__device__ __forceinline__ void stage_rows(const float *__restrict__ xp, int h, int w, int r0, int r1, float k0, float *s_x) {
    const int n = (r1 - r0 + 2) * w;
    for (int e = threadIdx.x; e < n; e += blockDim.x) {
        const int r = r0 - 1 + e / w;
        s_x[e] = (r >= 0 && r < h) ? xp[(int64_t)r * w + (e % w)] - k0 : 0.f;
    }
    __syncthreads();
}

__device__ __forceinline__ float stencil_lds(const float *s_x, int li, int j, int i, int h, int w, const float *__restrict__ ay,
                                             const float *__restrict__ ax) {
    const float al = j > 0 ? ax[j] : 0.f, am = ax[w + j], au = j < w - 1 ? ax[2 * w + j] : 0.f;
    const int jl = j > 0 ? j - 1 : j, ju = j < w - 1 ? j + 1 : j;
    float t = 0.f;
#pragma unroll
    for (int di = 0; di < 3; ++di) {
        const float *row = s_x + (li + di) * w;
        t += ay[di * h + i] * (al * row[jl] + am * row[j] + au * row[ju]);
    }
    return t;
}

__global__ void __launch_bounds__(kPhThreads)
upbn_stats_kernel(const float *__restrict__ X, int C, int h, int w, const float *__restrict__ a, const float *__restrict__ b,
                  const float *__restrict__ ay, const float *__restrict__ ax, int rows_per_chunk,
                  float *__restrict__ partial) {
    extern __shared__ __attribute__((aligned(16))) float s_x[];
    __shared__ float red[2][kPhThreads / 64];
    const int plane = blockIdx.x, chunk = blockIdx.y;
    const int c = plane % C;
    const float k0 = X[(int64_t)c * h * w];
    const float *xp = X + (int64_t)plane * h * w;
    const int r0 = chunk * rows_per_chunk, r1 = min(h, r0 + rows_per_chunk);
    stage_rows(xp, h, w, r0, r1, k0, s_x);
    float s1 = 0.f, s2 = 0.f;
    for (int e = threadIdx.x; e < (r1 - r0) * w; e += kPhThreads) {
        const int li = e / w, j = e - li * w, i = r0 + li;
        const float xc = s_x[(li + 1) * w + j];
        s1 += a[i] * b[j] * xc;
        s2 += xc * stencil_lds(s_x, li, j, i, h, w, ay, ax);
    }
#pragma unroll
    for (int off = 32; off >= 1; off >>= 1) {
        s1 += __shfl_down(s1, off);
        s2 += __shfl_down(s2, off);
    }
    if ((threadIdx.x & 63) == 0) {
        red[0][threadIdx.x >> 6] = s1;
        red[1][threadIdx.x >> 6] = s2;
    }
    __syncthreads();
    if (threadIdx.x == 0) {
        float *o = partial + ((int64_t)plane * gridDim.y + chunk) * 2;
        o[0] = red[0][0] + red[0][1] + red[0][2] + red[0][3];
        o[1] = red[1][0] + red[1][1] + red[1][2] + red[1][3];
    }
}

__global__ void __launch_bounds__(kPhThreads)
upbn_dense_grad_kernel(const float *__restrict__ X, int C, int h, int w, const float *__restrict__ a,
                       const float *__restrict__ b, const float *__restrict__ ay, const float *__restrict__ ax,
                       const float *__restrict__ c0, const float *__restrict__ c1, int rows_per_chunk,
                       float *__restrict__ dX) {
    extern __shared__ __attribute__((aligned(16))) float s_x[];
    const int plane = blockIdx.x, chunk = blockIdx.y;
    const int c = plane % C;
    const float *xp = X + (int64_t)plane * h * w;
    float *dp = dX + (int64_t)plane * h * w;
    const int r0 = chunk * rows_per_chunk, r1 = min(h, r0 + rows_per_chunk);
    stage_rows(xp, h, w, r0, r1, 0.f, s_x);
    const float k0c = c0[c], k1c = c1[c];
    for (int e = threadIdx.x; e < (r1 - r0) * w; e += kPhThreads) {
        const int li = e / w, j = e - li * w, i = r0 + li;
        dp[(int64_t)i * w + j] = k0c * a[i] * b[j] + k1c * stencil_lds(s_x, li, j, i, h, w, ay, ax);
    }
}

constexpr int kTrTile = 64;
__global__ void __launch_bounds__(256)
transpose_kernel(const float *__restrict__ in, float *__restrict__ out, int rows, int cols, float scale = 1.f) {
    __shared__ float tile[kTrTile][kTrTile + 1];
    const size_t plane = (size_t)blockIdx.z * rows * cols;
    const int c0 = blockIdx.x * kTrTile, r0 = blockIdx.y * kTrTile;
    const int tx = threadIdx.x & 63, ty = threadIdx.x >> 6;
#pragma unroll
    for (int k = 0; k < kTrTile; k += 4) {
        const int r = r0 + ty + k, c = c0 + tx;
        if (r < rows && c < cols) tile[ty + k][tx] = in[plane + (size_t)r * cols + c];
    }
    __syncthreads();
#pragma unroll
    for (int k = 0; k < kTrTile; k += 4) {
        const int c = c0 + ty + k, r = r0 + tx;
        if (c < cols && r < rows) out[plane + (size_t)c * rows + r] = tile[tx][ty + k] * scale;
    }
}

struct L2cGrids {
    const float *g[4];
    int ch[4], cw[4];
    float ry[4], rx[4];
    int n;
};

__device__ __forceinline__ void l2c_taps(int d, float r, int n_src, int &i0, int &i1, float &f) {
    const float s = r * (float)d;
    i0 = (int)s;
    if (i0 > n_src - 1) i0 = n_src - 1;
    f = s - (float)i0;
    i1 = i0 + (i0 < n_src - 1 ? 1 : 0);
}

__global__ void __launch_bounds__(256)
l2c_combine_rows_kernel(L2cGrids G, int n_img, int H, int W, int c4, float4 *__restrict__ out) {
    const int64_t t = (int64_t)blockIdx.x * 256 + threadIdx.x;
    if (t >= (int64_t)n_img * H * W * c4) return;
    const int c = (int)(t % c4);
    const int64_t pix = t / c4;
    const int x = (int)(pix % W), y = (int)((pix / W) % H), img = (int)(pix / ((int64_t)W * H));
    float4 acc = reinterpret_cast<const float4 *>(G.g[0])[t];
#pragma unroll
    for (int s = 1; s < 4; ++s) {
        if (s >= G.n) break;
        int y0, y1, x0, x1;
        float fy, fx;
        l2c_taps(y, G.ry[s], G.ch[s], y0, y1, fy);
        l2c_taps(x, G.rx[s], G.cw[s], x0, x1, fx);
        const float4 *g = reinterpret_cast<const float4 *>(G.g[s]) + (int64_t)img * G.ch[s] * G.cw[s] * c4 + c;
        const float4 a = g[((int64_t)y0 * G.cw[s] + x0) * c4], b = g[((int64_t)y0 * G.cw[s] + x1) * c4];
        const float4 d = g[((int64_t)y1 * G.cw[s] + x0) * c4], e = g[((int64_t)y1 * G.cw[s] + x1) * c4];
        const float w00 = (1.f - fy) * (1.f - fx), w01 = (1.f - fy) * fx, w10 = fy * (1.f - fx), w11 = fy * fx;
        acc.x += w00 * a.x + w01 * b.x + w10 * d.x + w11 * e.x;
        acc.y += w00 * a.y + w01 * b.y + w10 * d.y + w11 * e.y;
        acc.z += w00 * a.z + w01 * b.z + w10 * d.z + w11 * e.z;
        acc.w += w00 * a.w + w01 * b.w + w10 * d.w + w11 * e.w;
    }
    out[t] = acc;
}

__global__ void __launch_bounds__(256)
l2c_combine_rows_bwd_kernel(const float4 *__restrict__ g, int n_img, int H, int W, int c4, int ch, int cw, float ry, float rx,
                            float4 *__restrict__ d) {
    const int64_t t = (int64_t)blockIdx.x * 256 + threadIdx.x;
    if (t >= (int64_t)n_img * ch * cw * c4) return;
    const int c = (int)(t % c4);
    const int64_t cell = t / c4;
    const int j = (int)(cell % cw), i = (int)((cell / cw) % ch), img = (int)(cell / ((int64_t)cw * ch));
    int ylo = 0, yhi = H - 1, xlo = 0, xhi = W - 1;
    if (ry > 0.f) { ylo = max(0, (int)floorf((float)(i - 1) / ry) - 1); yhi = min(H - 1, (int)ceilf((float)(i + 1) / ry) + 1); }
    if (rx > 0.f) { xlo = max(0, (int)floorf((float)(j - 1) / rx) - 1); xhi = min(W - 1, (int)ceilf((float)(j + 1) / rx) + 1); }
    float4 acc = make_float4(0.f, 0.f, 0.f, 0.f);
    for (int y = ylo; y <= yhi; ++y) {
        int y0, y1;
        float fy;
        l2c_taps(y, ry, ch, y0, y1, fy);
        const float wy = (y0 == i ? 1.f - fy : 0.f) + (y1 == i ? fy : 0.f);
        if (wy == 0.f) continue;
        const float4 *row = g + ((int64_t)img * H + y) * W * c4 + c;
        for (int x = xlo; x <= xhi; ++x) {
            int x0, x1;
            float fx;
            l2c_taps(x, rx, cw, x0, x1, fx);
            const float w = wy * ((x0 == j ? 1.f - fx : 0.f) + (x1 == j ? fx : 0.f));
            if (w == 0.f) continue;
            const float4 v = row[(int64_t)x * c4];
            acc.x += w * v.x; acc.y += w * v.y; acc.z += w * v.z; acc.w += w * v.w;
        }
    }
    d[t] = acc;
}

__global__ void __launch_bounds__(256)
maxpool3s2_fwd_kernel(const float *__restrict__ x, int h, int w, int oh, int ow, float *__restrict__ y,
                      uint8_t *__restrict__ code) {
    const uint32_t pix = blockIdx.x * blockDim.x + threadIdx.x;
    if (pix >= (uint32_t)(oh * ow)) return;
    const int oy = (int)(pix / (uint32_t)ow), ox = (int)(pix - (uint32_t)oy * (uint32_t)ow);
    const int64_t plane = blockIdx.y;
    const int64_t e = plane * oh * ow + pix;
    const float *xp = x + plane * (int64_t)h * w;
    const int y0 = 2 * oy - 1, x0 = 2 * ox - 1;
    float best = -INFINITY;
    int bc = 0;
    bool first = true;
#pragma unroll
    for (int dy = 0; dy < 3; ++dy) {
        const int yy = y0 + dy;
        if (yy < 0 || yy >= h) continue;
#pragma unroll
        for (int dx = 0; dx < 3; ++dx) {
            const int xx = x0 + dx;
            if (xx < 0 || xx >= w) continue;
            const float v = xp[(int64_t)yy * w + xx];
            if (first || v > best || v != v) { best = v; bc = dy * 3 + dx; first = false; }
        }
    }
    y[e] = best;
    code[e] = (uint8_t)bc;
}

__global__ void __launch_bounds__(256)
maxpool3s2_bwd_kernel(const float *__restrict__ dy, const uint8_t *__restrict__ code, int h, int w, int oh, int ow,
                      float *__restrict__ dx) {
    const uint32_t pix = blockIdx.x * blockDim.x + threadIdx.x;
    if (pix >= (uint32_t)(h * w)) return;
    const int yy = (int)(pix / (uint32_t)w), xx = (int)(pix - (uint32_t)yy * (uint32_t)w);
    const int64_t plane = blockIdx.y;
    const int64_t e = plane * h * w + pix;
    const float *gp = dy + plane * (int64_t)oh * ow;
    const uint8_t *cp = code + plane * (int64_t)oh * ow;
    float g = 0.f;
    const int oy0 = yy >> 1, oy1 = (yy + 1) >> 1, ox0 = xx >> 1, ox1 = (xx + 1) >> 1;
#pragma unroll
    for (int a = 0; a < 2; ++a) {
        const int oy = a ? oy1 : oy0;
        if ((a && oy1 == oy0) || oy >= oh) continue;
        const int dyw = yy - (2 * oy - 1);
#pragma unroll
        for (int b = 0; b < 2; ++b) {
            const int ox = b ? ox1 : ox0;
            if ((b && ox1 == ox0) || ox >= ow) continue;
            const int dxw = xx - (2 * ox - 1);
            if (cp[(int64_t)oy * ow + ox] == dyw * 3 + dxw) g += gp[(int64_t)oy * ow + ox];
        }
    }
    dx[e] = g;
}

__global__ void __launch_bounds__(256)
maxpool3s2_bwd4_kernel(const float *__restrict__ dy, const uint8_t *__restrict__ code, int h, int w, int oh, int ow,
                       float *__restrict__ dx) {
    const int w4 = w >> 2;
    const uint32_t q = blockIdx.x * blockDim.x + threadIdx.x;
    if (q >= (uint32_t)(h * w4)) return;
    const int yy = (int)(q / (uint32_t)w4), x0 = 4 * (int)(q - (uint32_t)yy * (uint32_t)w4);
    const int64_t plane = blockIdx.y;
    const float *gp = dy + plane * (int64_t)oh * ow;
    const uint8_t *cp = code + plane * (int64_t)oh * ow;
    const int oy0 = yy >> 1, oy1 = (yy + 1) >> 1, oxb = x0 >> 1;
    float g[4] = {0.f, 0.f, 0.f, 0.f};
#pragma unroll
    for (int a = 0; a < 2; ++a) {
        const int oy = a ? oy1 : oy0;
        if ((a && oy1 == oy0) || oy >= oh) continue;
        const int dyw = yy - (2 * oy - 1);
#pragma unroll
        for (int b = 0; b < 3; ++b) {
            const int ox = oxb + b;
            if (ox >= ow) continue;
            const int sel = (int)cp[(int64_t)oy * ow + ox] - 3 * dyw;
            const float v = gp[(int64_t)oy * ow + ox];
            const int col = 2 * ox - 1 + sel - x0;
#pragma unroll
            for (int i = 0; i < 4; ++i) g[i] += (sel >= 0 && sel < 3 && col == i) ? v : 0.f;
        }
    }
    *reinterpret_cast<float4 *>(dx + plane * (int64_t)h * w + (int64_t)yy * w + x0) = make_float4(g[0], g[1], g[2], g[3]);
}

__device__ __forceinline__ void up_source(float scale, int dst, int &i0, float &lambda1) {
#pragma clang fp contract(off)
    const float src = scale * (float)dst;
    i0 = (int)src;
    lambda1 = src - (float)i0;
}

__global__ void __launch_bounds__(256)
up_bilinear_fwd_kernel(const float *__restrict__ x, const float *__restrict__ skip, int64_t total, int h, int w, int H, int W,
                       float rh, float rw, float *__restrict__ y) {
    const int64_t e = (int64_t)blockIdx.x * blockDim.x + threadIdx.x;
    if (e >= total) return;
    const int ox = (int)(e % W);
    const int64_t r = e / W;
    const int oy = (int)(r % H);
    const int64_t plane = r / H;
    int h1, w1;
    float h1l, w1l;
    up_source(rh, oy, h1, h1l);
    up_source(rw, ox, w1, w1l);
    const int h1p = h1 < h - 1 ? 1 : 0, w1p = w1 < w - 1 ? 1 : 0;
    const float h0l = 1.f - h1l, w0l = 1.f - w1l;
    const float *xp = x + plane * (int64_t)h * w + (int64_t)h1 * w + w1;
    float v = h0l * (w0l * xp[0] + w1l * xp[w1p]) + h1l * (w0l * xp[(int64_t)h1p * w] + w1l * xp[(int64_t)h1p * w + w1p]);
    if (skip) v += skip[e];
    y[e] = v;
}

constexpr int kUpTaps = 8;
__global__ void __launch_bounds__(256)
up_bilinear_bwd_kernel(const float *__restrict__ g, int64_t total_in, int h, int w, int H, int W, const int2 *__restrict__ ty,
                       const float *__restrict__ wy, const int2 *__restrict__ tx, const float *__restrict__ wx,
                       float *__restrict__ dx) {
    const int64_t e = (int64_t)blockIdx.x * blockDim.x + threadIdx.x;
    if (e >= total_in) return;
    const int j = (int)(e % w);
    const int64_t r = e / w;
    const int i = (int)(r % h);
    const int64_t plane = r / h;
    const float *gp = g + plane * (int64_t)H * W;
    const int2 ry = ty[i], rx = tx[j];
    float acc = 0.f;
    for (int a = 0; a < ry.y; ++a) {
        const float *row = gp + (int64_t)(ry.x + a) * W + rx.x;
        float t = 0.f;
        for (int b = 0; b < rx.y; ++b) t += wx[j * kUpTaps + b] * row[b];
        acc += wy[i * kUpTaps + a] * t;
    }
    dx[e] = acc;
}

constexpr int kUpTi = 16, kUpTj = 64, kUpLr = 40, kUpLc = 136;
__global__ void __launch_bounds__(256)
up_bilinear_bwd_tiled_kernel(const float *__restrict__ g, int h, int w, int H, int W, const int2 *__restrict__ ty,
                             const float *__restrict__ wy, const int2 *__restrict__ tx, const float *__restrict__ wx,
                             float *__restrict__ dx) {
    __shared__ float win[kUpLr][kUpLc + 1];
    const int j0 = blockIdx.x * kUpTj, i0 = blockIdx.y * kUpTi;
    const int64_t plane = blockIdx.z;
    const int i1 = min(i0 + kUpTi, h) - 1, j1 = min(j0 + kUpTj, w) - 1;
    const int r_lo = ty[i0].x, r_hi = ty[i1].x + ty[i1].y, c_lo = tx[j0].x, c_hi = tx[j1].x + tx[j1].y;
    const int nr = r_hi - r_lo, nc = c_hi - c_lo;
    const float *gp = g + plane * (int64_t)H * W;
    for (int rr = threadIdx.x / 64; rr < nr; rr += 4)
        for (int cc = threadIdx.x % 64; cc < nc; cc += 64) win[rr][cc] = gp[(int64_t)(r_lo + rr) * W + c_lo + cc];
    __syncthreads();
    const int j = j0 + threadIdx.x % 64;
    if (j > j1) return;
    const int2 rx = tx[j];
    float wxj[kUpTaps];
#pragma unroll
    for (int b = 0; b < kUpTaps; ++b) wxj[b] = wx[j * kUpTaps + b];
    const int cb = rx.x - c_lo;
    for (int i = i0 + threadIdx.x / 64; i <= i1; i += 4) {
        const int2 ry = ty[i];
        float acc = 0.f;
        for (int a = 0; a < ry.y; ++a) {
            const float *row = &win[ry.x - r_lo + a][cb];
            float t = 0.f;
#pragma unroll
            for (int b = 0; b < kUpTaps; ++b)
                if (b < rx.y) t += wxj[b] * row[b];
            acc += wy[i * kUpTaps + a] * t;
        }
        dx[plane * (int64_t)h * w + (int64_t)i * w + j] = acc;
    }
}

}

using namespace u2mkd;

extern "C" {

int u2mkd_up_plan(const int32_t *idx8, int64_t n, int32_t H, int32_t W, int32_t h, int32_t w, float rh, float rw,
                  int32_t *idx_out, float *w_out, u2mkd_stream_t s) {
    if (n == 0) return 0;
    U2_REQUIRE(idx8 && idx_out && w_out, "u2mkd_up_plan: null pointer");
    U2_REQUIRE(H > 0 && W > 0 && h > 0 && w > 0 && h <= H && w <= W, "u2mkd_up_plan: bad sizes %dx%d <- %dx%d", H, W, h, w);
    U2_REQUIRE(n * 4 < ((int64_t)1 << 31), "u2mkd_up_plan: more than 2^31 samples");
    hipLaunchKernelGGL(up_plan_kernel, dim3((unsigned)ceil_div(n * 4, kPhThreads)), dim3(kPhThreads), 0, as_stream(s), idx8, n,
                       H, W, h, w, rh, rw, idx_out, w_out);
    return check_launch("u2mkd_up_plan");
}

int u2mkd_upbn_stats(const float *x, int32_t n_img, int32_t c, int32_t h, int32_t w, const float *a, const float *b,
                     const float *ay, const float *ax, int32_t rows_per_chunk, float *partial, u2mkd_stream_t s) {
    U2_REQUIRE(x && a && b && ay && ax && partial, "u2mkd_upbn_stats: null pointer");
    U2_REQUIRE(n_img > 0 && c > 0 && h > 0 && w > 0 && rows_per_chunk > 0, "u2mkd_upbn_stats: bad shape");
    const int chunks = (int)ceil_div(h, rows_per_chunk);
    U2_REQUIRE((int64_t)n_img * c < ((int64_t)1 << 31) && chunks <= 65535, "u2mkd_upbn_stats: grid too large");
    const size_t lds = (size_t)(rows_per_chunk + 2) * w * sizeof(float);
    U2_REQUIRE(lds <= 60 * 1024, "u2mkd_upbn_stats: %d rows of %d floats do not fit the LDS stage", rows_per_chunk + 2, w);
    hipLaunchKernelGGL(upbn_stats_kernel, dim3((unsigned)(n_img * c), (unsigned)chunks), dim3(kPhThreads), lds, as_stream(s), x,
                       c, h, w, a, b, ay, ax, rows_per_chunk, partial);
    return check_launch("u2mkd_upbn_stats");
}

int u2mkd_upbn_dense_grad(const float *x, int32_t n_img, int32_t c, int32_t h, int32_t w, const float *a, const float *b,
                          const float *ay, const float *ax, const float *c0, const float *c1, int32_t rows_per_chunk,
                          float *dx, u2mkd_stream_t s) {
    U2_REQUIRE(x && a && b && ay && ax && c0 && c1 && dx, "u2mkd_upbn_dense_grad: null pointer");
    U2_REQUIRE(n_img > 0 && c > 0 && h > 0 && w > 0 && rows_per_chunk > 0, "u2mkd_upbn_dense_grad: bad shape");
    const int chunks = (int)ceil_div(h, rows_per_chunk);
    const size_t lds = (size_t)(rows_per_chunk + 2) * w * sizeof(float);
    U2_REQUIRE(lds <= 60 * 1024 && chunks <= 65535, "u2mkd_upbn_dense_grad: %d rows of %d floats do not fit the LDS stage",
               rows_per_chunk + 2, w);
    hipLaunchKernelGGL(upbn_dense_grad_kernel, dim3((unsigned)(n_img * c), (unsigned)chunks), dim3(kPhThreads), lds, as_stream(s),
                       x, c, h, w, a, b, ay, ax, c0, c1, rows_per_chunk, dx);
    return check_launch("u2mkd_upbn_dense_grad");
}

int u2mkd_transpose_batched(const float *in, float *out, int32_t batch, int32_t rows, int32_t cols, u2mkd_stream_t s) {
    if (batch == 0 || rows == 0 || cols == 0) return 0;
    U2_REQUIRE(in && out && batch > 0 && rows > 0 && cols > 0, "u2mkd_transpose_batched: bad arguments");
    U2_REQUIRE(batch <= 65535 && ceil_div(rows, kTrTile) <= 65535, "u2mkd_transpose_batched: grid too large");
    hipLaunchKernelGGL(transpose_kernel, dim3((unsigned)ceil_div(cols, kTrTile), (unsigned)ceil_div(rows, kTrTile), (unsigned)batch),
                       dim3(256), 0, as_stream(s), in, out, rows, cols);
    return check_launch("u2mkd_transpose_batched");
}

int u2mkd_transpose_batched_scaled(const float *in, float *out, int32_t batch, int32_t rows, int32_t cols, float scale,
                                   u2mkd_stream_t s) {
    if (batch == 0 || rows == 0 || cols == 0) return 0;
    U2_REQUIRE(in && out && batch > 0 && rows > 0 && cols > 0, "u2mkd_transpose_batched_scaled: bad arguments");
    U2_REQUIRE(batch <= 65535 && ceil_div(rows, kTrTile) <= 65535, "u2mkd_transpose_batched_scaled: grid too large");
    hipLaunchKernelGGL(transpose_kernel, dim3((unsigned)ceil_div(cols, kTrTile), (unsigned)ceil_div(rows, kTrTile), (unsigned)batch),
                       dim3(256), 0, as_stream(s), in, out, rows, cols, scale);
    return check_launch("u2mkd_transpose_batched_scaled");
}

static float l2c_ratio(int n_src, int n_dst) { return n_dst > 1 ? (float)(n_src - 1) / (float)(n_dst - 1) : 0.f; }

int u2mkd_l2c_combine_forward(const float *g0, const float *g1, const float *g2, const float *g3, int32_t n_grids, int32_t n_img,
                              int32_t h, int32_t w, int32_t c, int32_t ch1, int32_t cw1, int32_t ch2, int32_t cw2, int32_t ch3,
                              int32_t cw3, float *out_rows, u2mkd_stream_t s) {
    U2_REQUIRE(n_grids >= 1 && n_grids <= 4 && c > 0 && c % 4 == 0 && n_img > 0 && h > 0 && w > 0,
               "u2mkd_l2c_combine_forward: %d grids of %d channels (1..4 grids, channels a multiple of 4)", n_grids, c);
    U2_REQUIRE(g0 && out_rows && (n_grids < 2 || g1) && (n_grids < 3 || g2) && (n_grids < 4 || g3), "u2mkd_l2c_combine_forward: null pointer");
    L2cGrids G;
    const float *gp[4] = {g0, g1, g2, g3};
    const int chs[4] = {h, ch1, ch2, ch3}, cws[4] = {w, cw1, cw2, cw3};
    for (int i = 0; i < 4; ++i) {
        G.g[i] = gp[i]; G.ch[i] = chs[i]; G.cw[i] = cws[i];
        G.ry[i] = l2c_ratio(chs[i], h); G.rx[i] = l2c_ratio(cws[i], w);
        U2_REQUIRE(i >= n_grids || (chs[i] > 0 && cws[i] > 0 && chs[i] <= h && cws[i] <= w), "u2mkd_l2c_combine_forward: grid %d is %dx%d", i, chs[i], cws[i]);
    }
    G.n = n_grids;
    const int64_t total = (int64_t)n_img * h * w * (c / 4);
    hipLaunchKernelGGL(l2c_combine_rows_kernel, dim3((unsigned)ceil_div(total, 256)), dim3(256), 0, as_stream(s), G, n_img, h, w,
                       c / 4, reinterpret_cast<float4 *>(out_rows));
    return check_launch("u2mkd_l2c_combine_forward");
}

int u2mkd_l2c_combine_backward(const float *g_rows, int32_t n_img, int32_t h, int32_t w, int32_t c, int32_t ch, int32_t cw,
                               float *d_grid, u2mkd_stream_t s) {
    U2_REQUIRE(g_rows && d_grid && c > 0 && c % 4 == 0 && n_img > 0 && h > 0 && w > 0 && ch > 0 && cw > 0 && ch <= h && cw <= w,
               "u2mkd_l2c_combine_backward: bad arguments");
    const int64_t total = (int64_t)n_img * ch * cw * (c / 4);
    hipLaunchKernelGGL(l2c_combine_rows_bwd_kernel, dim3((unsigned)ceil_div(total, 256)), dim3(256), 0, as_stream(s),
                       reinterpret_cast<const float4 *>(g_rows), n_img, h, w, c / 4, ch, cw, l2c_ratio(ch, h), l2c_ratio(cw, w),
                       reinterpret_cast<float4 *>(d_grid));
    return check_launch("u2mkd_l2c_combine_backward");
}

int u2mkd_maxpool3s2_forward(const float *x, int64_t planes, int32_t h, int32_t w, float *y, uint8_t *code, u2mkd_stream_t s) {
    if (planes == 0) return 0;
    U2_REQUIRE(x && y && code && planes > 0 && h > 0 && w > 0, "u2mkd_maxpool3s2_forward: bad arguments");
    const int oh = (h + 2 - 3) / 2 + 1, ow = (w + 2 - 3) / 2 + 1;
    U2_REQUIRE(planes <= 65535 && (int64_t)h * w < ((int64_t)1 << 31), "u2mkd_maxpool3s2_forward: at most 65535 planes of < 2^31 pixels");
    hipLaunchKernelGGL(maxpool3s2_fwd_kernel, dim3((unsigned)ceil_div((int64_t)oh * ow, 256), (unsigned)planes), dim3(256), 0,
                       as_stream(s), x, h, w, oh, ow, y, code);
    return check_launch("u2mkd_maxpool3s2_forward");
}

int u2mkd_maxpool3s2_backward(const float *dy, const uint8_t *code, int64_t planes, int32_t h, int32_t w, float *dx,
                              u2mkd_stream_t s) {
    if (planes == 0) return 0;
    U2_REQUIRE(dy && code && dx && planes > 0 && h > 0 && w > 0, "u2mkd_maxpool3s2_backward: bad arguments");
    const int oh = (h + 2 - 3) / 2 + 1, ow = (w + 2 - 3) / 2 + 1;
    U2_REQUIRE(planes <= 65535 && (int64_t)h * w < ((int64_t)1 << 31), "u2mkd_maxpool3s2_backward: at most 65535 planes of < 2^31 pixels");
    if (w % 4 == 0 && (reinterpret_cast<uintptr_t>(dx) & 15) == 0)
        hipLaunchKernelGGL(maxpool3s2_bwd4_kernel, dim3((unsigned)ceil_div((int64_t)h * (w / 4), 256), (unsigned)planes), dim3(256), 0,
                           as_stream(s), dy, code, h, w, oh, ow, dx);
    else
        hipLaunchKernelGGL(maxpool3s2_bwd_kernel, dim3((unsigned)ceil_div((int64_t)h * w, 256), (unsigned)planes), dim3(256), 0,
                           as_stream(s), dy, code, h, w, oh, ow, dx);
    return check_launch("u2mkd_maxpool3s2_backward");
}

int u2mkd_up_bilinear_forward(const float *x, const float *skip, int64_t planes, int32_t h, int32_t w, int32_t H, int32_t W,
                              float rh, float rw, float *y, u2mkd_stream_t s) {
    if (planes == 0) return 0;
    U2_REQUIRE(x && y && planes > 0 && h > 0 && w > 0 && H > 0 && W > 0, "u2mkd_up_bilinear_forward: bad arguments");
    const int64_t total = planes * H * W;
    hipLaunchKernelGGL(up_bilinear_fwd_kernel, dim3((unsigned)ceil_div(total, 256)), dim3(256), 0, as_stream(s), x, skip, total, h,
                       w, H, W, rh, rw, y);
    return check_launch("u2mkd_up_bilinear_forward");
}

int u2mkd_up_bilinear_backward(const float *g, int64_t planes, int32_t h, int32_t w, int32_t H, int32_t W, const int32_t *taps_y,
                               const float *wy, const int32_t *taps_x, const float *wx, int32_t tiled, float *dx, u2mkd_stream_t s) {
    if (planes == 0) return 0;
    U2_REQUIRE(g && taps_y && wy && taps_x && wx && dx && planes > 0 && h > 0 && w > 0 && H > 0 && W > 0,
               "u2mkd_up_bilinear_backward: bad arguments");
    U2_REQUIRE(!tiled || planes <= 65535, "u2mkd_up_bilinear_backward: the tiled form takes at most 65535 planes");
    const int64_t total = planes * h * w;
    if (tiled) {
        hipLaunchKernelGGL(up_bilinear_bwd_tiled_kernel, dim3((unsigned)ceil_div(w, kUpTj), (unsigned)ceil_div(h, kUpTi), (unsigned)planes),
                           dim3(256), 0, as_stream(s), g, h, w, H, W, reinterpret_cast<const int2 *>(taps_y), wy,
                           reinterpret_cast<const int2 *>(taps_x), wx, dx);
        return check_launch("u2mkd_up_bilinear_backward");
    }
    hipLaunchKernelGGL(up_bilinear_bwd_kernel, dim3((unsigned)ceil_div(total, 256)), dim3(256), 0, as_stream(s), g, total, h, w, H,
                       W, reinterpret_cast<const int2 *>(taps_y), wy, reinterpret_cast<const int2 *>(taps_x), wx, dx);
    return check_launch("u2mkd_up_bilinear_backward");
}

}
```

u2mkd_amd/fusion.py:

```python
import os

import torch
import torch.nn.functional as F
from torch import nn

from .camera import BatchNorm2d, bn_act

__all__ = ['IA_Layer', 'Atten_Fusion_Conv', 'L2CAILayer', 'L2CFusion', 'feature_gather', 'c2l_gather',
           'l2c_scatter', 'feature_fetch', 'l2c_scatter_torch', 'c2l_gather_torch']


def _rows_linear(x, weight, bias, before=None):
    w = weight.squeeze(-1) if weight.dim() == 3 else weight
    if x.is_cuda and w.shape[1] % 4 == 0:
        from .torchsparse.nn import functional as spf
        return spf.linear(x, w, bias, bias_feeds_batchnorm=before is not None and before.training)
    return F.linear(x, w, bias)


def _rows_bn(bn, x, relu=False):
    if x.is_cuda and x.shape[1] % 4 == 0:
        from .torchsparse.nn import functional as spf
        return spf.batch_norm(x, bn, relu)
    y = bn(x)
    return F.relu(y) if relu else y


class IA_Layer(nn.Module):

    def __init__(self, channels):
        super().__init__()
        self.ic, self.pc = channels
        rc = self.pc // 4
        self.conv1 = nn.Sequential(nn.Conv1d(self.ic, self.pc, 1), nn.BatchNorm1d(self.pc), nn.ReLU(True))
        self.fc1 = nn.Sequential(nn.BatchNorm1d(self.ic), nn.ReLU(True), nn.Linear(self.ic, rc))
        self.fc2 = nn.Linear(self.pc, rc)
        self.fc3 = nn.Linear(rc, 1)

    def forward(self, img_feats, point_feats):
        img_feats = img_feats.contiguous()
        ri = _rows_linear(_rows_bn(self.fc1[0], img_feats, relu=True), self.fc1[2].weight, self.fc1[2].bias)
        rp = _rows_linear(point_feats.contiguous(), self.fc2.weight, self.fc2.bias)
        att = torch.sigmoid(_rows_linear(torch.tanh(ri + rp), self.fc3.weight, self.fc3.bias))
        img = _rows_bn(self.conv1[1], _rows_linear(img_feats, self.conv1[0].weight, self.conv1[0].bias, before=self.conv1[1]), relu=True)
        return img * att


class Atten_Fusion_Conv(nn.Module):
    def __init__(self, inplanes_I, inplanes_P, outplanes):
        super().__init__()
        self.ai_layer = IA_Layer(channels=[inplanes_I, inplanes_P])
        self.conv1 = nn.Conv1d(inplanes_P + inplanes_P, outplanes, 1)
        self.bn1 = nn.BatchNorm1d(outplanes)

    def forward(self, point_features, img_features):
        img = self.ai_layer(img_features, point_features)
        fused = torch.cat([point_features, img], dim=1)
        return _rows_bn(self.bn1, _rows_linear(fused, self.conv1.weight, self.conv1.bias, before=self.bn1), relu=True)


class L2CAILayer(nn.Module):
    def __init__(self, channels):
        super().__init__()
        self.ic, self.pc = channels
        rc = self.ic // 4
        self.conv1 = nn.Sequential(nn.Conv2d(self.pc, self.ic, 1), BatchNorm2d(self.ic), nn.ReLU(True))
        self.fc1 = nn.Conv2d(self.ic, rc, kernel_size=1)
        self.fc2 = nn.Conv2d(self.pc, rc, kernel_size=1)
        self.fc3 = nn.Conv2d(rc, 1, kernel_size=1)

    def forward(self, img_feats, point_feats):
        att = torch.sigmoid(self.fc3(torch.tanh(self.fc1(img_feats.contiguous()) + self.fc2(point_feats.contiguous()))))
        return bn_act(self.conv1[1], self.conv1[0](point_feats), relu=True) * att


class L2CFusion(nn.Module):
    def __init__(self, inplanes_I, inplanes_P, outplanes):
        super().__init__()
        self.conv1 = nn.Conv2d(inplanes_I + inplanes_I, outplanes, kernel_size=1)
        self.bn1 = BatchNorm2d(outplanes)
        self.l2c_ai_layer = L2CAILayer(channels=[inplanes_I, inplanes_P])

    def forward(self, point_features, img_features):
        l2c = self.l2c_ai_layer(img_features, point_features)
        fused = self.bn1(self.conv1(torch.cat([img_features, l2c], dim=1)))
        return F.relu(fused), fused


def feature_gather(feature_map, xy, mode='bilinear'):
    return F.grid_sample(feature_map, xy.unsqueeze(1), padding_mode='zeros', align_corners=True, mode=mode).squeeze(2)


def _last_camera(mask):
    ncam = mask.shape[0]
    rank = torch.arange(1, ncam + 1, device=mask.device).view(-1, 1) * mask.to(torch.int64)
    best = rank.max(0)[0]
    return (best - 1).clamp(min=0), best > 0


class _NchwToRows(torch.autograd.Function):

    @staticmethod
    def forward(ctx, fm):
        ctx.shape = fm.shape
        B, ncam, C, h, w = fm.shape
        if fm.is_cuda and fm.dtype == torch.float32 and fm.is_contiguous() and B * ncam <= 65535 and fm.numel():
            from . import _lib as L
            out = torch.empty(B * ncam * h * w, C, dtype=torch.float32, device=fm.device)
            L.call('u2mkd_transpose_batched', L.ptr(fm), L.ptr(out), B * ncam, C, h * w, L.stream())
            return out
        return fm.permute(0, 1, 3, 4, 2).contiguous().view(B * ncam * h * w, C)

    @staticmethod
    def backward(ctx, g):
        B, ncam, C, h, w = ctx.shape
        if g.is_cuda and g.dtype == torch.float32 and B * ncam <= 65535 and g.numel():
            from . import _lib as L
            g = g.contiguous()
            out = torch.empty(B, ncam, C, h, w, dtype=torch.float32, device=g.device)
            L.call('u2mkd_transpose_batched', L.ptr(g), L.ptr(out), B * ncam, h * w, C, L.stream())
            return out
        return g.view(B, ncam, h, w, C).permute(0, 1, 4, 2, 3).contiguous()


def _c2l_plan_torch(pixel_coordinates, masks, h, w):
    ncam = masks[0].shape[0]
    idx, wts = [], []
    for b, (coord, mask) in enumerate(zip(pixel_coordinates, masks)):
        cam, seen = _last_camera(mask)
        xy = coord.gather(0, cam.view(1, -1, 1).expand(1, -1, 2)).squeeze(0).float()
        x = (xy[:, 0] + 1.0) * 0.5 * (w - 1)
        y = (xy[:, 1] + 1.0) * 0.5 * (h - 1)
        x0, y0 = torch.floor(x), torch.floor(y)
        fx, fy = x - x0, y - y0
        base = (b * ncam + cam) * (h * w)
        ii, ww = [], []
        for dy, wy in ((0, 1.0 - fy), (1, fy)):
            for dx, wx in ((0, 1.0 - fx), (1, fx)):
                xi, yi = x0.long() + dx, y0.long() + dy
                ok = seen & (xi >= 0) & (xi < w) & (yi >= 0) & (yi < h)
                ii.append(torch.where(ok, base + yi * w + xi, torch.full_like(xi, -1)))
                ww.append(torch.where(ok, wx * wy, torch.zeros_like(wx)))
        pad_i = torch.full_like(ii[0], -1)
        pad_w = torch.zeros_like(ww[0])
        idx.append(torch.stack(ii + [pad_i] * 4, 1))
        wts.append(torch.stack(ww + [pad_w] * 4, 1))
    return torch.cat(idx, 0).int().contiguous(), torch.cat(wts, 0).float().contiguous()


def _mask_bytes(m):
    return m.contiguous().view(torch.uint8) if m.dtype == torch.bool else m.contiguous().to(torch.uint8)


def _c2l_plan(pixel_coordinates, masks, h, w):
    from . import _lib as L
    ncam = masks[0].shape[0]
    n_tot = sum(m.shape[1] for m in masks)
    dev = masks[0].device
    idx8 = torch.empty(n_tot, 8, dtype=torch.int32, device=dev)
    w8 = torch.empty(n_tot, 8, dtype=torch.float32, device=dev)
    cur = 0
    for b, (coord, mask) in enumerate(zip(pixel_coordinates, masks)):
        n = mask.shape[1]
        pc, mb = coord.contiguous().float(), _mask_bytes(mask)
        L.call('u2mkd_c2l_plan', L.ptr(pc), L.ptr(mb), ncam, n, b, h, w, L.ptr(idx8[cur:]), L.ptr(w8[cur:]), L.stream())
        cur += n
    return idx8, w8


def c2l_plan(pixel_coordinates, masks, h, w):
    from .torchsparse.nn import functional as spf
    return spf._plan(masks[0], 'c2l_%d_%d' % (h, w), lambda: _c2l_plan(pixel_coordinates, masks, h, w),
                     *masks[1:], *pixel_coordinates)


def l2c_plan(pixel_coordinates, masks, ch, cw):
    from .torchsparse.nn import functional as spf
    return spf._plan(masks[0], 'l2c_%d_%d' % (ch, cw), lambda: _l2c_plan(pixel_coordinates, masks, ch, cw),
                     *masks[1:], *pixel_coordinates)


def _l2c_grids(ifh, ifw, n_scales):
    cnt = 1
    for _ in range(n_scales):
        yield int(round(float(ifh) / cnt + 0.01)), int(round(float(ifw) / cnt + 0.01))
        cnt *= 2


def prefetch_plans(pixel_coordinates, masks, shapes):
    from .torchsparse.nn import functional as spf
    n_img = len(masks) * masks[0].shape[0]
    for ifh, ifw, n_scales in shapes:
        idx8, w8 = c2l_plan(pixel_coordinates, masks, ifh, ifw)
        spf.devoxelize_plan(idx8, w8, n_img * ifh * ifw)
        for ch, cw in _l2c_grids(ifh, ifw, n_scales):
            l2c_plan(pixel_coordinates, masks, ch, cw)


def c2l_gather(feature_maps, pixel_coordinates, masks):
    from . import _lib
    _lib.require_cuda(feature_maps)
    from .torchsparse.nn import functional as spf
    B, ncam, C, h, w = feature_maps.shape
    idx8, w8 = c2l_plan(pixel_coordinates, masks, h, w)
    rows = _NchwToRows.apply(feature_maps)
    if C % 4:
        rows = F.pad(rows, (0, 4 - C % 4))
    return spf.spdevoxelize(rows, idx8, w8)[:, :C]


def c2l_gather_torch(feature_maps, pixel_coordinates, masks):
    out = []
    for fmap, coord, mask in zip(feature_maps, pixel_coordinates, masks):
        sampled = feature_gather(fmap, coord)
        cam, seen = _last_camera(mask)
        pick = sampled.gather(0, cam.view(1, 1, -1).expand(1, sampled.shape[1], -1)).squeeze(0)
        out.append((pick * seen.to(pick.dtype).unsqueeze(0)).t())
    return torch.cat(out, dim=0)


def feature_fetch(masks, pixel_coordinates, imfeats, mode='bilinear'):
    return c2l_gather(imfeats, pixel_coordinates, masks)


class _SegmentMap(torch.autograd.Function):

    @staticmethod
    def forward(ctx, src, fwd, bwd, n_dst):
        from .torchsparse.nn import functional as spf
        ctx.bwd, ctx.n_src, ctx.in_dtype = bwd, src.shape[0], src.dtype
        erow, ew, seg = fwd
        return spf._segment_sum(spf._rows(src, spf._moved16(src.dtype)), erow, ew, seg, n_dst, False)

    @staticmethod
    def backward(ctx, g):
        from .torchsparse.nn import functional as spf
        erow, ew, seg = ctx.bwd
        gs = spf._segment_sum(spf._rows(g, spf._moved16(g.dtype)), erow, ew, seg, ctx.n_src, False)
        return (gs if gs.dtype == ctx.in_dtype else gs.to(ctx.in_dtype)), None, None, None


def _flat_entries(pixel_coordinates, masks):
    ncam = masks[0].shape[0]
    dev = masks[0].device
    coords = torch.cat([c.reshape(-1, 2) for c in pixel_coordinates], 0)
    mask = torch.cat([m.reshape(-1) for m in masks], 0)
    slot, row = [], []
    cur = 0
    for b, m in enumerate(masks):
        n = m.shape[1]
        slot.append((torch.arange(ncam, device=dev) + b * ncam).repeat_interleave(n))
        row.append((torch.arange(n, device=dev) + cur).repeat(ncam))
        cur += n
    return coords, mask, torch.cat(slot), torch.cat(row), cur


def _l2c_plan_torch(pixel_coordinates, masks, ch, cw):
    from .torchsparse.nn import functional as spf
    coords, mask, slot, row, n_pts = _flat_entries(pixel_coordinates, masks)
    u = torch.floor((coords[:, 0] + 1.0) / 2 * (cw - 1.0)).long().clamp(0, cw - 1)
    v = torch.floor((coords[:, 1] + 1.0) / 2 * (ch - 1.0)).long().clamp(0, ch - 1)
    pix = (slot * ch + v) * cw + u
    n_dst = len(masks) * masks[0].shape[0] * ch * cw
    key_d = torch.where(mask, pix, torch.full_like(pix, -1)).int()
    num = spf.spcount(key_d, n_dst).clamp(min=1).float()
    w = 1.0 / num[pix]
    order_d, seg_d = spf._csr_by_destination(key_d, n_dst)
    od = order_d.long()
    key_s = torch.where(mask, row, torch.full_like(row, -1)).int()
    order_s, seg_s = spf._csr_by_destination(key_s, n_pts)
    os_ = order_s.long()
    fwd = (row[od].int().contiguous(), w[od].contiguous(), seg_d)
    bwd = (pix[os_].int().contiguous(), w[os_].contiguous(), seg_s)
    return fwd, bwd, n_dst


def _l2c_plan(pixel_coordinates, masks, ch, cw):
    from . import _lib as L
    from .torchsparse.nn import functional as spf
    ncam = masks[0].shape[0]
    dev = masks[0].device
    n_pts = sum(m.shape[1] for m in masks)
    e = ncam * n_pts
    n_dst = len(masks) * ncam * ch * cw
    pix = torch.empty(e, dtype=torch.int32, device=dev)
    key_d = torch.empty_like(pix)
    row = torch.empty_like(pix)

    def keys(key_s):
        row0 = e0 = 0
        for b, (coord, mask) in enumerate(zip(pixel_coordinates, masks)):
            n = mask.shape[1]
            pc, mb = coord.contiguous().float(), _mask_bytes(mask)
            L.call('u2mkd_l2c_keys', L.ptr(pc), L.ptr(mb), ncam, n, b, row0, e0, ch, cw, L.ptr(pix), L.ptr(key_d),
                   L.ptr(key_s), L.ptr(row), L.stream())
            row0 += n
            e0 += ncam * n

    def by_source():
        key_s = torch.empty_like(pix)
        keys(key_s)
        return spf._csr_by_destination(key_s, n_pts) + (True,)
    hit = masks[0].__dict__.get('_u2mkd_plans', {}).get('l2c_by_source')
    order_s, seg_s, fresh = spf._plan(masks[0], 'l2c_by_source', by_source, *masks[1:])
    if hit is not None or not fresh:
        keys(None)
    masks[0].__dict__['_u2mkd_plans']['l2c_by_source'] = (masks[0].__dict__['_u2mkd_plans']['l2c_by_source'][0], (order_s, seg_s, False))
    order_d, seg_d = spf._csr_by_destination(key_d, n_dst)
    fwd_row, bwd_pix = torch.empty_like(pix), torch.empty_like(pix)
    fwd_w = torch.empty(e, dtype=torch.float32, device=dev)
    bwd_w = torch.empty_like(fwd_w)
    L.call('u2mkd_l2c_finish', L.ptr(order_d), L.ptr(seg_d), L.ptr(order_s), L.ptr(pix), L.ptr(row), e, L.ptr(fwd_row),
           L.ptr(fwd_w), L.ptr(bwd_pix), L.ptr(bwd_w), L.stream())
    return (fwd_row, fwd_w, seg_d), (bwd_pix, bwd_w, seg_s), n_dst


_L2C_COMBINE = os.environ.get('U2MKD_L2C_COMBINE', '1') != '0'


class _L2cCombine(torch.autograd.Function):

    @staticmethod
    def forward(ctx, n_img, sizes, *grids):
        from . import _lib as L
        n = len(grids)
        (h, w), c = sizes[0], grids[0].shape[1]
        ctx.meta = (n_img, sizes, c)
        out = torch.empty(n_img, c, h, w, dtype=torch.float32, device=grids[0].device)
        if n == 1:
            rows = grids[0]
        else:
            rows = torch.empty(n_img * h * w, c, dtype=torch.float32, device=grids[0].device)
            gp = [L.ptr(g) for g in grids] + [None] * (4 - n)
            dims = [v for s in list(sizes[1:]) + [(0, 0)] * (4 - n) for v in s]
            L.call('u2mkd_l2c_combine_forward', *gp, n, n_img, h, w, c, *dims, L.ptr(rows), L.stream())
        L.call('u2mkd_transpose_batched_scaled', L.ptr(rows), L.ptr(out), n_img, h * w, c, 1.0 / n, L.stream())
        return out

    @staticmethod
    @torch.autograd.function.once_differentiable
    def backward(ctx, g):
        from . import _lib as L
        n_img, sizes, c = ctx.meta
        n = len(sizes)
        h, w = sizes[0]
        g = g.contiguous()
        g_rows = torch.empty(n_img * h * w, c, dtype=torch.float32, device=g.device)
        L.call('u2mkd_transpose_batched_scaled', L.ptr(g), L.ptr(g_rows), n_img, c, h * w, 1.0 / n, L.stream())
        grads = [g_rows]
        for ch, cw in sizes[1:]:
            d = torch.empty(n_img * ch * cw, c, dtype=torch.float32, device=g.device)
            L.call('u2mkd_l2c_combine_backward', L.ptr(g_rows), n_img, h, w, c, ch, cw, L.ptr(d), L.stream())
            grads.append(d)
        return (None, None) + tuple(grads)


def l2c_scatter(point_feats, pixel_coordinates, masks, ifh, ifw, n_scales):
    from . import _lib
    _lib.require_cuda(point_feats)
    if point_feats.shape[1] % 4:
        return l2c_scatter_torch(point_feats, pixel_coordinates, masks, ifh, ifw, n_scales)
    from .torchsparse.nn import functional as spf
    B, ncam, C = len(masks), masks[0].shape[0], point_feats.shape[1]
    sizes = list(_l2c_grids(ifh, ifw, n_scales))
    if (_L2C_COMBINE and point_feats.dtype == torch.float32 and spf.row_dtype() is None and 1 <= n_scales <= 4 and B * ncam <= 65535
            and sizes[0] == (ifh, ifw)):
        grids = [_SegmentMap.apply(point_feats, *l2c_plan(pixel_coordinates, masks, ch, cw)) for ch, cw in sizes]
        if all(g.dtype == torch.float32 for g in grids):
            return _L2cCombine.apply(B * ncam, tuple(sizes), *grids)
    total = None
    for ch, cw in sizes:
        fwd, bwd, n_dst = l2c_plan(pixel_coordinates, masks, ch, cw)
        grid = _SegmentMap.apply(point_feats, fwd, bwd, n_dst).view(B * ncam, ch, cw, C).permute(0, 3, 1, 2)
        up = grid if (ch, cw) == (ifh, ifw) else F.interpolate(grid, (ifh, ifw), mode='bilinear', align_corners=True)
        total = up if total is None else total + up
    return (total / n_scales).contiguous()


def l2c_scatter_torch(point_feats, pixel_coordinates, masks, ifh, ifw, n_scales):
    B = len(masks)
    ncam = masks[0].shape[0]
    C = point_feats.shape[1]
    dev, dt = point_feats.device, point_feats.dtype
    sizes = [m.shape[1] for m in masks]
    coords = torch.cat([c.reshape(-1, 2) for c in pixel_coordinates], 0)
    mask = torch.cat([m.reshape(-1) for m in masks], 0)
    slot, row = [], []
    cur = 0
    for b, n in enumerate(sizes):
        slot.append((torch.arange(ncam, device=dev) + b * ncam).repeat_interleave(n))
        row.append((torch.arange(n, device=dev) + cur).repeat(ncam))
        cur += n
    slot, row = torch.cat(slot), torch.cat(row)
    w = mask.to(dt).unsqueeze(1)
    feats = point_feats[row] * w
    total = torch.zeros(B * ncam, C, ifh, ifw, device=dev, dtype=dt)
    cnt = 1
    for _ in range(n_scales):
        ch = int(round(float(ifh) / cnt + 0.01))
        cw = int(round(float(ifw) / cnt + 0.01))
        u = torch.floor((coords[:, 0] + 1.0) / 2 * (cw - 1.0)).long().clamp(0, cw - 1)
        v = torch.floor((coords[:, 1] + 1.0) / 2 * (ch - 1.0)).long().clamp(0, ch - 1)
        pix = (slot * ch + v) * cw + u
        acc = torch.zeros(B * ncam * ch * cw, C, device=dev, dtype=dt).index_add_(0, pix, feats)
        num = torch.zeros(B * ncam * ch * cw, 1, device=dev, dtype=dt).index_add_(0, pix, w)
        grid = (acc / num.clamp(min=1.0)).view(B * ncam, ch, cw, C).permute(0, 3, 1, 2)
        total = total + F.interpolate(grid, (ifh, ifw), mode='bilinear', align_corners=True)
        cnt *= 2
    return total / n_scales
```

u2mkd_amd/kd.py:

```python
from copy import deepcopy

import os

import torch
import torch.nn.functional as F
from torch import nn

from . import torchsparse
from .camera import BNReluConv, SwiftNetRes18
from .graphs import PieceCache, StaticPiece
from .fusion import Atten_Fusion_Conv, L2CFusion, c2l_gather, feature_fetch, l2c_scatter
from .pixel_head import sampled_head_applies, sampled_pixel_logits
from .lidar.blocks import (BasicConvolutionBlock, BasicDeconvolutionBlock, FusedSequential, PointBatchNorm1d, PointLinear,
                           ResidualBlock)
from .lidar.point_voxel import (initial_voxelize, point_to_voxel, prepare_geometry, prepare_geometry_many, prepare_geometry_staged,
                                voxel_to_point)
from .torchsparse.nn import functional as spf
from .lidar.sphereformer import SphereFormer
from .lidar.spvcnn_spformer import SPVCNN_SPFORMER
from .losses import MixLovaszCrossEntropy, kl_div_logits
from .torchsparse import PointTensor
from .torchsparse import nn as spnn

__all__ = ['StudentMSP2IFM', 'TSDFull', 'teacher_to_student', 'kd_losses', 'KDCriterion']

_BASE_CHANNELS = (32, 32, 64, 128, 256, 256, 128, 96, 96)


class StudentMSP2IFM(nn.Module):

    def __init__(self, cr, in_channel, num_classes, window_size, window_size_sphere, quant_size, quant_size_sphere,
                 window_size_scale, drop_path_rate, a, pres, vres, imagenet_pretrain=None, run_pix_decoder=True):
        super().__init__()
        cs = [int(cr * c) for c in _BASE_CHANNELS]
        self.cs = cs
        self.pix_branch = SwiftNetRes18(num_feature=(128, 128, 128), pretrained_path=imagenet_pretrain)
        img_cs = self.pix_branch.img_cs
        self.in_channel, self.num_classes, self.out_channel = in_channel, num_classes, cs[-1]
        self.pres, self.vres = pres, vres
        self._fusion_shapes = {}

        self.stem = FusedSequential(
            spnn.Conv3d(in_channel, cs[0], kernel_size=3, stride=1), spnn.BatchNorm(cs[0]), spnn.ReLU(True),
            spnn.Conv3d(cs[0], cs[0], kernel_size=3, stride=1), spnn.BatchNorm(cs[0]), spnn.ReLU(True))
        self.vox_downs = nn.ModuleList([
            nn.Sequential(BasicConvolutionBlock(cs[i], cs[i], ks=2, stride=2, dilation=1),
                          ResidualBlock(cs[i], cs[i + 1], ks=3, stride=1, dilation=1),
                          ResidualBlock(cs[i + 1], cs[i + 1], ks=3, stride=1, dilation=1))
            for i in range(4)])

        self.window_size, self.window_size_sphere = window_size, window_size_sphere
        self.quant_size, self.quant_size_sphere = quant_size, quant_size_sphere
        dpr = [x.item() for x in torch.linspace(0, drop_path_rate, 7)]
        self.transformer_blocks = nn.ModuleList()
        for idx in range(1, 5):
            self.transformer_blocks.append(SphereFormer(
                cs[idx], cs[idx] // 16, self.window_size, self.window_size_sphere, self.quant_size,
                self.quant_size_sphere, indice_key='sphereformer{}'.format(idx + 1), drop_path=dpr[idx], a=a))
            sc, ss = window_size_scale
            self.window_size = self.window_size * sc
            self.quant_size = self.quant_size * sc
            self.window_size_sphere[0] = self.window_size_sphere[0] * ss
            self.window_size_sphere[1] = self.window_size_sphere[1] * ss
            self.quant_size_sphere[0] = self.quant_size_sphere[0] * ss
            self.quant_size_sphere[1] = self.quant_size_sphere[1] * ss

        self.c2l_fusion_blocks = nn.ModuleList(
            [Atten_Fusion_Conv(inplanes_I=img_cs[i], inplanes_P=cs[i], outplanes=cs[i]) for i in range(1, 5)])
        self.l2c_fusion_blocks = nn.ModuleList(
            [L2CFusion(inplanes_I=img_cs[i], inplanes_P=cs[i], outplanes=img_cs[i]) for i in range(1, 5)])
        self.learner = nn.ModuleList([
            FusedSequential(PointLinear(cs[i], img_cs[i]), PointBatchNorm1d(img_cs[i]), nn.ReLU(True),
                            PointLinear(img_cs[i], img_cs[i]), PointBatchNorm1d(img_cs[i]))
            for i in range(1, 5)])
        self.mse = nn.MSELoss()

        self.vox_ups = nn.ModuleList([
            nn.ModuleList([
                BasicDeconvolutionBlock(cs[i], cs[i + 1], ks=2, stride=2),
                nn.Sequential(
                    ResidualBlock(cs[i + 1] + cs[len(cs) - 2 - i], cs[i + 1], ks=3, stride=1, dilation=1),
                    ResidualBlock(cs[i + 1], cs[i + 1], ks=3, stride=1, dilation=1))])
            for i in range(4, len(cs) - 1)])
        self.classifier_vox = nn.Sequential(PointLinear(cs[8], num_classes))
        self.classifier_pix = BNReluConv(self.pix_branch.num_features, num_classes, k=1)
        self.point_transforms = nn.ModuleList([
            FusedSequential(PointLinear(cs[a_], cs[b_]), PointBatchNorm1d(cs[b_]), nn.ReLU(True))
            for a_, b_ in ((0, 4), (4, 6), (6, 8))])
        for m in self.modules():
            if isinstance(m, nn.BatchNorm1d):
                nn.init.constant_(m.weight, 1)
                nn.init.constant_(m.bias, 0)
        self.dropout = nn.Dropout(0.3, True)
        self.run_pix_decoder = run_pix_decoder
        self.adapt_layer = None

    def _camera_stage_eager(self, x_in, idx):
        x_o, skip_o = self.pix_branch.forward_resblock(x_in, getattr(self.pix_branch, 'layer%d' % (idx + 1)))
        if idx == len(self.vox_downs) - 1:
            skip_o = self.pix_branch.spp(skip_o)
        return x_o, skip_o

    def _piece(self, name):
        pieces = self.__dict__.setdefault('_pieces', PieceCache())
        if name not in pieces:
            pb, last = self.pix_branch, len(self.vox_downs) - 1
            if name == 'head':
                fn, mods = (lambda im: self._camera_stage_eager(pb.forward_stem(im), 0)), [pb.conv1, pb.bn1, pb.layer1]
            elif name.startswith('stage'):
                idx = int(name[5:])
                fn = lambda x_in, idx=idx: self._camera_stage_eager(x_in, idx)
                mods = [getattr(pb, 'layer%d' % (idx + 1))] + ([pb.spp] if idx == last else [])
            elif name.startswith('l2c'):
                blk = self.l2c_fusion_blocks[int(name[3:])]
                fn, mods = (lambda fmap, skip: blk(fmap, skip)), [blk]
            elif name == 'decoder_low':
                fn, mods = (lambda *feats: pb.forward_up(list(feats), im_size=None)), [pb.upsample]
            else:
                assert name.startswith('decoder_'), name
                im_size = tuple(int(v) for v in name[8:].split('x'))
                fn = lambda *feats: self.classifier_pix(pb.forward_up(list(feats), im_size=im_size))
                mods = [pb.upsample, self.classifier_pix]
            pieces[name] = StaticPiece(name, fn, mods)
        return pieces[name]

    def _camera_stage(self, x_in, idx):
        return self._piece('head')(x_in) if idx == 0 else self._piece('stage%d' % idx)(x_in)

    def camera_head(self, in_mod):
        im = in_mod['images']
        im = im.reshape(-1, *im.shape[2:])
        return _Fork(im, 'camera', _CAMERA_STREAM and _overlap_ok()).on_side(
            lambda: self._camera_stage(im, 0), im)

    @staticmethod
    def _tokens(coords, stride, zz):
        from .lidar.point_voxel import p2v_maps
        idx_query, counts = p2v_maps(coords, stride, zz)
        return spf.spvoxelize(zz.F, idx_query, counts)[:, :3].contiguous(), coords[:, 3]

    @torch.no_grad()
    def prefetch_plans(self, in_mod):
        from .fusion import prefetch_plans as fusion_plans
        from .lidar.point_voxel import p2v_maps, v2p_maps
        z, x0 = in_mod['_geometry']
        if x0.C.shape[0] == 0:
            return
        zz = PointTensor(x0.F, x0.C.float())
        n_stage = len(self.vox_downs)
        strides = [x0.s] + [tuple(v * 2 ** (i + 1) for v in x0.s) for i in range(n_stage)]
        if any(x0.cmaps.get(s3) is None for s3 in strides):
            return
        tokens = []
        parts = spf._PREFETCH_PARTS
        for i, s3 in enumerate(strides):
            coords = x0.cmaps[s3]
            if 'A' in parts:
                v2p_maps(coords, s3, z, plans=True)
                p2v_maps(coords, s3, z, plans=True)
            if i > 0 and 'C' in parts:
                p2v_maps(coords, s3, zz, plans=True)
                tok = self._tokens(coords, s3, zz)
                self.transformer_blocks[i - 1].attn.plans(tok[0].float(), tok[1], quantised=True)
                tokens.append(tok)
        if 'C' in parts:
            x0.__dict__['_u2mkd_kd_plans'] = {'zz': zz, 'tokens': tokens}
        im = in_mod['images']
        shapes = self._fusion_shapes.get((int(im.shape[-2]), int(im.shape[-1])))
        if shapes is not None and len(shapes) == n_stage and 'D' in parts:
            fusion_plans(in_mod['pixel_coordinates'], in_mod['masks'], [shapes[i] for i in range(n_stage)])

    def forward(self, in_mod):
        x = in_mod['lidar']
        im = in_mod['images']
        ib, ncam, ic, ih, iw = im.shape
        im = im.reshape(-1, ic, ih, iw)
        pixel_coordinates, masks, fov_mask = in_mod['pixel_coordinates'], in_mod['masks'], in_mod['fov_mask']
        fork = _Fork(im, 'camera', _CAMERA_STREAM and _overlap_ok())
        on_side, join = fork.on_side, fork.join
        n_stage = len(self.vox_downs)
        cam_stage = self._camera_stage
        cam = in_mod.get('_camera_head')
        if cam is None:
            cam = self.camera_head(in_mod)
        z, x0 = in_mod.get('_geometry') or prepare_geometry(x, self.pres, self.vres)
        ahead = x0.__dict__.get('_u2mkd_kd_plans')
        zz = ahead['zz'] if ahead is not None else PointTensor(x0.F, x0.C.float())
        x0 = self.stem(x0)
        z0 = voxel_to_point(x0, z, nearest=False)
        vox_feats = [point_to_voxel(x0, z0)]
        img_feats, mse_loss, pts_feats = [], [], []
        x_im_ready = None
        for idx in range(n_stage):
            if idx > 0:
                cam = on_side(lambda: cam_stage(x_im, idx), x_im, after=x_im_ready if _CAMERA_FORK_EARLY else None)
            vox_out = self.vox_downs[idx](vox_feats[idx])
            if ahead is not None:
                coord_xyz, batch = ahead['tokens'][idx]
            else:
                coord_xyz, batch = self._tokens(vox_out.C, vox_out.s, zz)
            vox_out.F = self.transformer_blocks[idx](vox_out.F, coord_xyz, batch)
            pts_feat = voxel_to_point(vox_out, z0)
            if idx == n_stage - 1:
                pts_feats.append(self.adapt_layer(pts_feat.F))

            x_im, skip = cam
            join(x_im, skip)
            _, ifc, ifh, ifw = skip.shape
            self._fusion_shapes.setdefault((ih, iw), {})[idx] = (ifh, ifw, n_stage - idx)

            l2c_feat_map = l2c_scatter(pts_feat.F, pixel_coordinates, masks, ifh, ifw, n_stage - idx)
            x_im, skip = self._piece('l2c%d' % idx)(l2c_feat_map, skip)
            x_im_ready = fork.mark()
            img_feats.append(skip)

            img_feat_tensor = c2l_gather(skip.view(ib, ncam, ifc, ifh, ifw), pixel_coordinates, masks)
            pseudo = self.learner[idx](pts_feat.F)
            img_feat_tensor, mse = _select_and_mse(img_feat_tensor, pseudo, fov_mask)
            mse_loss.append(mse)
            pts_feat.F = self.c2l_fusion_blocks[idx](pts_feat.F, img_feat_tensor)
            vox_feats.append(point_to_voxel(vox_out, pts_feat))

        fused = fork.mark()
        _, x1, x2, x3, x4 = vox_feats
        z1 = pts_feat
        z1.F = z1.F + self.point_transforms[0](z0.F)
        y1 = point_to_voxel(x4, z1)
        y1.F = self.dropout(y1.F)
        y1 = self.vox_ups[0][0](y1)
        y1 = self.vox_ups[0][1](torchsparse.cat([y1, x3]))
        y2 = self.vox_ups[1][0](y1)
        y2 = self.vox_ups[1][1](torchsparse.cat([y2, x2]))
        z2 = voxel_to_point(y2, z1)
        z2.F = z2.F + self.point_transforms[1](z1.F)
        y3 = point_to_voxel(y2, z2)
        y3.F = self.dropout(y3.F)
        y3 = self.vox_ups[2][0](y3)
        y3 = self.vox_ups[2][1](torchsparse.cat([y3, x1]))
        y4 = self.vox_ups[3][0](y3)
        y4 = self.vox_ups[3][1](torchsparse.cat([y4, x0]))
        z3 = voxel_to_point(y4, z2)
        z3.F = z3.F + self.point_transforms[2](z2.F)

        ret = {'x_vox': self.classifier_vox(z3.F), 'num_pts': [c.shape[1] for c in pixel_coordinates],
               'mse_loss': mse_loss, 'pts_feats': pts_feats}
        if self.run_pix_decoder:
            sampled = sampled_head_applies(img_feats[0], self.classifier_pix)

            def pix_decoder():
                if sampled:
                    fmap = self._piece('decoder_low')(*img_feats)
                    return sampled_pixel_logits(fmap, self.classifier_pix, pixel_coordinates, masks, (ih, iw), ib, ncam)
                if ib * ncam * self.pix_branch.num_features * ih * iw * 4 >= 2 ** 32:
                    raise RuntimeError('the dense pixel head would form a %.1f GB tensor, beyond what MIOpen computes '
                                       'correctly: use the sampled head (U2MKD_SAMPLED_PIXEL_HEAD=1, the default)'
                                       % (ib * ncam * self.pix_branch.num_features * ih * iw * 4 / 1e9))
                fmap = self._piece('decoder_%dx%d' % (ih, iw))(*img_feats)
                fmap = fmap.view(ib, ncam, fmap.shape[1], fmap.shape[2], fmap.shape[3])
                return feature_fetch(masks, pixel_coordinates, fmap)
            x_pix = on_side(pix_decoder, *img_feats, after=fused)
            join(x_pix)
            ret['x_pix'] = x_pix
        return ret


class _SelectMSE(torch.autograd.Function):

    @staticmethod
    def forward(ctx, gathered, pseudo, fov):
        from . import _lib as L
        n, c = pseudo.shape
        gathered, pseudo = gathered.contiguous(), pseudo.contiguous()
        fov8 = fov.contiguous().view(torch.uint8)
        out = torch.empty_like(pseudo)
        partial = torch.empty(2 * L.load().u2mkd_select_mse_partials(), dtype=torch.float32, device=pseudo.device)
        stats = torch.empty(2, dtype=torch.float32, device=pseudo.device)
        L.call('u2mkd_select_mse_forward', L.ptr(gathered), L.ptr(pseudo), L.ptr(fov8), n, c, L.ptr(out), L.ptr(partial),
               L.ptr(stats), L.stream())
        ctx.save_for_backward(gathered, pseudo, fov8, stats)
        return out, stats[0]

    @staticmethod
    def backward(ctx, g_out, g_loss):
        from . import _lib as L
        gathered, pseudo, fov8, stats = ctx.saved_tensors
        n, c = pseudo.shape
        g_out = g_out.contiguous() if g_out is not None else None
        g_loss = g_loss.contiguous().float() if g_loss is not None else None
        d_g = torch.empty_like(gathered) if ctx.needs_input_grad[0] else None
        d_p = torch.empty_like(pseudo)
        L.call('u2mkd_select_mse_backward', L.ptr(g_out), L.ptr(g_loss), L.ptr(stats), L.ptr(gathered), L.ptr(pseudo),
               L.ptr(fov8), n, c, L.ptr(d_g), L.ptr(d_p), L.stream())
        return d_g, d_p, None


def _select_and_mse(gathered, pseudo, fov):
    if (pseudo.is_cuda and pseudo.dtype == torch.float32 and gathered.dtype == torch.float32 and pseudo.shape[1] % 4 == 0
            and fov.dtype == torch.bool and not torch.is_autocast_enabled()):
        return _SelectMSE.apply(gathered, pseudo, fov)
    out = torch.where(fov.unsqueeze(1), gathered, pseudo)
    return out, _masked_mse(pseudo, out.detach(), fov)


def _masked_mse(a, b, mask):
    m = mask.to(a.dtype).unsqueeze(1)
    return (((a - b) ** 2) * m).sum() / (m.sum() * a.shape[1]).clamp(min=1.0)


class TSDFull(nn.Module):

    def __init__(self, cr, cr_t, in_channel, in_channel_t, num_classes, spformer: dict, imagenet_pretrain=None,
                 run_pix_decoder=True, debug_val=False):
        super().__init__()
        param_s, param_t = dict(spformer), deepcopy(spformer)
        self.model_s = StudentMSP2IFM(cr=cr, in_channel=in_channel, num_classes=num_classes,
                                      imagenet_pretrain=imagenet_pretrain, run_pix_decoder=run_pix_decoder, **param_s)
        self.model_t = SPVCNN_SPFORMER(cr=cr_t, in_channel=in_channel_t, num_classes=num_classes,
                                       return_pts_feats=True, **param_t)
        self.model_t.requires_grad_(False)
        self.num_classes = num_classes
        self.debug_val = debug_val
        self.model_s.adapt_layer = FusedSequential(
            PointLinear(self.model_s.cs[4], self.model_t.cs[4]), PointBatchNorm1d(self.model_t.cs[4]), nn.ReLU(True))

    def prepare(self, in_mod: dict):
        with torch.no_grad():
            g_s, g_t = prepare_geometry_many([(in_mod['student']['lidar'], self.model_s.pres, self.model_s.vres, 'kd_student'),
                                              (in_mod['teacher']['lidar'], self.model_t.pres, self.model_t.vres, _TEACHER_TAG)])
            in_mod['student']['_geometry'] = g_s
            in_mod['teacher']['_geometry'] = g_t
            if spf.prefetch_plans_enabled():
                self.model_s.prefetch_plans(in_mod['student'])
        return in_mod

    def prepare_staged(self, in_mod: dict):
        g_s, g_t = yield from prepare_geometry_staged([(in_mod['student']['lidar'], self.model_s.pres, self.model_s.vres, 'kd_student'),
                                                       (in_mod['teacher']['lidar'], self.model_t.pres, self.model_t.vres, _TEACHER_TAG)])
        in_mod['student']['_geometry'] = g_s
        in_mod['teacher']['_geometry'] = g_t
        if spf.prefetch_plans_enabled():
            self.model_s.prefetch_plans(in_mod['student'])
        return in_mod

    def forward(self, in_mod: dict):
        want_t = self.training or self.debug_val
        side = _side_stream(in_mod['teacher']['lidar'].F, 'teacher') if want_t and _TEACHER_STREAM and _overlap_ok() else None
        if side is None:
            ret = {'stu': self.model_s(in_mod['student'])}
            if want_t:
                with torch.no_grad():
                    ret['t'] = self.model_t(in_mod['teacher'])
            return ret
        main = torch.cuda.current_stream()
        stu_in = in_mod['student']
        ahead = in_mod['teacher'].pop('_teacher_out', None)
        if ahead is not None:
            t = ahead
            ret = {'stu': self.model_s(stu_in)}
            main.wait_stream(side)
            for v in _tensors(t):
                v.record_stream(main)
            ret['t'] = t
            return ret
        if _CAMERA_STREAM and self.training and _overlap_ok():
            stu_in = dict(stu_in, _camera_head=self.model_s.camera_head(stu_in))
        if 'teacher_after_camera' in _DEBUG_ORDER:
            side.wait_stream(_side_stream(in_mod['teacher']['lidar'].F, 'camera'))
        side.wait_stream(main)
        with torch.cuda.stream(side), torch.no_grad():
# ... 141 lines not shown
```

Before: 1.271 million.

## Run L2C fusion block in row layout with fused gated BN and layout kernels

Adds a row-major (points x channels) path for the lidar-to-camera fusion block. Multi-scale grids are combined and scaled directly into rows, the attention gate and gated BN+ReLU are fused into custom kernels, and the final BN writes NCHW outputs and row outputs together. The row output is then reused by the camera-to-lidar gather, which removes an NCHW-to-rows transpose and several separate elementwise and transpose launches. The cost is a large new kernel surface with restricted channel widths. The path is disabled when graphs are on or the shapes do not qualify, and falls back to the old path.

After: 1.345 million (median of 5 runs). +5.8%, better.

```diff
diff --git a/include/u2mkd_hip.h b/include/u2mkd_hip.h
--- a/include/u2mkd_hip.h
+++ b/include/u2mkd_hip.h
@@ -228,8 +228,36 @@
 int u2mkd_l2c_combine_forward(const float *g0, const float *g1, const float *g2, const float *g3, int32_t n_grids, int32_t n_img,
                               int32_t h, int32_t w, int32_t c, int32_t ch1, int32_t cw1, int32_t ch2, int32_t cw2, int32_t ch3,
                               int32_t cw3, float *out_rows, u2mkd_stream_t s);
+int u2mkd_l2c_combine_forward_scaled(const float *g0, const float *g1, const float *g2, const float *g3, int32_t n_grids,
+                                     int32_t n_img, int32_t h, int32_t w, int32_t c, int32_t ch1, int32_t cw1, int32_t ch2,
+                                     int32_t cw2, int32_t ch3, int32_t cw3, float scale ,
+                                     float *out_rows, u2mkd_stream_t s);
 int u2mkd_l2c_combine_backward(const float *g_rows, int32_t n_img, int32_t h, int32_t w, int32_t c, int32_t ch, int32_t cw,
                                float *d_grid, u2mkd_stream_t s);
+
+int u2mkd_l2c_gate_forward(const float *h1, const float *h2, const float *b1, const float *b2, const float *w3, const float *b3,
+                           int64_t m, int32_t rc, float *att, u2mkd_stream_t s);
+int64_t u2mkd_l2c_gate_partial_floats(int64_t m, int32_t rc);
+int u2mkd_l2c_gate_backward(const float *datt, const float *att, const float *h1, const float *h2, const float *b1,
+                            const float *b2, const float *w3, int64_t m, int32_t rc, float *partial, float *dh, float *sums,
+                            u2mkd_stream_t s);
+int u2mkd_l2c_image_in(const float *img, int32_t n_img, int32_t c, int64_t hw, float *rows, float *cat, int32_t ld_cat,
+                       u2mkd_stream_t s);
+int u2mkd_l2c_image_in_backward(const float *g_rows, const float *g_cat, int32_t ld_cat, int32_t n_img, int32_t c, int64_t hw,
+                                float *g_img, u2mkd_stream_t s);
+int u2mkd_l2c_grad_in(const float *g_skip, const float *g_x_im, const float *fused, const float *g_rows, int32_t n_img, int32_t c,
+                      int64_t hw, float *dy_rows, u2mkd_stream_t s);
+int u2mkd_bn_gated_train_forward(const float *x, const float *att, int64_t n, int32_t c, const float *gamma, const float *beta,
+                                 float eps, float momentum, float *running_mean, float *running_var,
+                                 int64_t *num_batches_tracked, float *partial, float *mean, float *invstd, float *y, int32_t ld_y,
+                                 u2mkd_stream_t s);
+int u2mkd_bn_gated_backward(const float *gy, int32_t ld_g, const float *x, const float *att, int64_t n, int32_t c,
+                            const float *mean, const float *invstd, const float *gamma, const float *beta, float *partial,
+                            float *dgamma, float *dbeta, float *dx, float *datt, u2mkd_stream_t s);
+int u2mkd_bn_train_forward_rows_nchw(const float *u, int32_t n_img, int64_t hw, int32_t c, const float *gamma, const float *beta,
+                                     float eps, float momentum, float *running_mean, float *running_var,
+                                     int64_t *num_batches_tracked, float *partial, float *mean, float *invstd, float *fused_nchw,
+                                     float *relu_nchw, float *fused_rows, u2mkd_stream_t s);
 
 int32_t u2mkd_select_mse_partials(void);
 int u2mkd_select_mse_forward(const float *gathered, const float *pseudo, const uint8_t *fov, int64_t n, int32_t c, float *out,
diff --git a/u2mkd_amd/_lib.py b/u2mkd_amd/_lib.py
--- a/u2mkd_amd/_lib.py
+++ b/u2mkd_amd/_lib.py
@@ -151,7 +151,17 @@
     'u2mkd_transpose_batched': (C.c_int, [_p, _p, _i32, _i32, _i32, _p]),
     'u2mkd_transpose_batched_scaled': (C.c_int, [_p, _p, _i32, _i32, _i32, C.c_float, _p]),
     'u2mkd_l2c_combine_forward': (C.c_int, [_p, _p, _p, _p] + [_i32] * 11 + [_p, _p]),
+    'u2mkd_l2c_combine_forward_scaled': (C.c_int, [_p, _p, _p, _p] + [_i32] * 11 + [_f32, _p, _p]),
     'u2mkd_l2c_combine_backward': (C.c_int, [_p] + [_i32] * 6 + [_p, _p]),
+    'u2mkd_l2c_gate_forward': (C.c_int, [_p] * 6 + [_i64, _i32, _p, _p]),
+    'u2mkd_l2c_gate_partial_floats': (_i64, [_i64, _i32]),
+    'u2mkd_l2c_gate_backward': (C.c_int, [_p] * 7 + [_i64, _i32, _p, _p, _p, _p]),
+    'u2mkd_l2c_image_in': (C.c_int, [_p, _i32, _i32, _i64, _p, _p, _i32, _p]),
+    'u2mkd_l2c_image_in_backward': (C.c_int, [_p, _p, _i32, _i32, _i32, _i64, _p, _p]),
+    'u2mkd_l2c_grad_in': (C.c_int, [_p, _p, _p, _p, _i32, _i32, _i64, _p, _p]),
+    'u2mkd_bn_gated_train_forward': (C.c_int, [_p, _p, _i64, _i32, _p, _p, _f32, _f32, _p, _p, _p, _p, _p, _p, _p, _i32, _p]),
+    'u2mkd_bn_gated_backward': (C.c_int, [_p, _i32, _p, _p, _i64, _i32] + [_p] * 10),
+    'u2mkd_bn_train_forward_rows_nchw': (C.c_int, [_p, _i32, _i64, _i32, _p, _p, _f32, _f32] + [_p] * 10),
     'u2mkd_up_plan': (C.c_int, [_p, _i64, _i32, _i32, _i32, _i32, _f32, _f32, _p, _p, _p]),
     'u2mkd_upbn_stats': (C.c_int, [_p, _i32, _i32, _i32, _i32, _p, _p, _p, _p, _i32, _p, _p]),
     'u2mkd_upbn_dense_grad': (C.c_int, [_p, _i32, _i32, _i32, _i32, _p, _p, _p, _p, _p, _p, _i32, _p, _p]),
diff --git a/u2mkd_amd/csrc/bn.hip b/u2mkd_amd/csrc/bn.hip
--- a/u2mkd_amd/csrc/bn.hip
+++ b/u2mkd_amd/csrc/bn.hip
@@ -420,6 +420,156 @@
     st4(dx, t, make_float4(d.x * g.x * is.x, d.y * g.y * is.y, d.z * g.z * is.z, d.w * g.w * is.w));
 }
 
+__device__ __forceinline__ float bn_row_lanes_sum(float v, int lanes) {
+    for (int o = lanes >> 1; o >= 1; o >>= 1) v += __shfl_xor(v, o, kWave);
+    return v;
+}
+
+__global__ void bn_gated_apply_kernel(const float *__restrict__ x, const float *__restrict__ att, int64_t total4, int c4,
+                                      const float *__restrict__ mean, const float *__restrict__ invstd,
+                                      const float *__restrict__ gamma, const float *__restrict__ beta, float *__restrict__ y,
+                                      int ld_y4) {
+    int64_t t = (int64_t)blockIdx.x * blockDim.x + threadIdx.x;
+    if (t >= total4) return;
+    const int jj = (int)(t % c4), j = jj * 4;
+    const int64_t row = t / c4;
+    const float a = att[row];
+    float4 v = ld4(x, t);
+    float4 m = *reinterpret_cast<const float4 *>(mean + j);
+    float4 is = *reinterpret_cast<const float4 *>(invstd + j);
+    float4 g = gamma ? *reinterpret_cast<const float4 *>(gamma + j) : make_float4(1.f, 1.f, 1.f, 1.f);
+    float4 b = beta ? *reinterpret_cast<const float4 *>(beta + j) : make_float4(0.f, 0.f, 0.f, 0.f);
+    float4 o;
+    o.x = fmaxf((v.x - m.x) * is.x * g.x + b.x, 0.f) * a;
+    o.y = fmaxf((v.y - m.y) * is.y * g.y + b.y, 0.f) * a;
+    o.z = fmaxf((v.z - m.z) * is.z * g.z + b.z, 0.f) * a;
+    o.w = fmaxf((v.w - m.w) * is.w * g.w + b.w, 0.f) * a;
+    st4(y, row * ld_y4 + jj, o);
+}
+
+__global__ void __launch_bounds__(kBnThreads)
+bn_gated_bwd_partial_kernel(const float *__restrict__ gy, int ld_g4, const float *__restrict__ x, const float *__restrict__ att,
+                            int64_t n, int c, const float *__restrict__ mean, const float *__restrict__ invstd,
+                            const float *__restrict__ gamma, const float *__restrict__ beta, float *__restrict__ partial,
+                            float *__restrict__ datt) {
+    extern __shared__ __attribute__((aligned(16))) float4 red[];
+    const int c4 = c >> 2, rl = kBnThreads / c4;
+    const int64_t r0 = (int64_t)blockIdx.x * kBnSlabRows;
+    const int rows = (int)min((int64_t)kBnSlabRows, n - r0);
+    const int j = threadIdx.x % c4, ry = threadIdx.x / c4;
+    float4 s1 = make_float4(0.f, 0.f, 0.f, 0.f), s2 = s1;
+    const float4 m = *reinterpret_cast<const float4 *>(mean + 4 * j);
+    const float4 is = *reinterpret_cast<const float4 *>(invstd + 4 * j);
+    const float4 g = gamma ? *reinterpret_cast<const float4 *>(gamma + 4 * j) : make_float4(1.f, 1.f, 1.f, 1.f);
+    const float4 b = beta ? *reinterpret_cast<const float4 *>(beta + 4 * j) : make_float4(0.f, 0.f, 0.f, 0.f);
+    for (int rr = ry; rr < rows; rr += rl) {
+        const int64_t row = r0 + rr;
+        const float4 v = ld4(x, row * c4 + j);
+        float4 d = ld4(gy, row * ld_g4 + j);
+        const float a = att[row];
+        const float hx = (v.x - m.x) * is.x, hy = (v.y - m.y) * is.y, hz = (v.z - m.z) * is.z, hw = (v.w - m.w) * is.w;
+        const float yx = fmaxf(hx * g.x + b.x, 0.f), yy = fmaxf(hy * g.y + b.y, 0.f), yz = fmaxf(hz * g.z + b.z, 0.f),
+                    yw = fmaxf(hw * g.w + b.w, 0.f);
+        const float p = bn_row_lanes_sum(d.x * yx + d.y * yy + d.z * yz + d.w * yw, c4);
+        if (j == 0) datt[row] = p;
+        d.x = yx > 0.f ? d.x * a : 0.f;
+        d.y = yy > 0.f ? d.y * a : 0.f;
+        d.z = yz > 0.f ? d.z * a : 0.f;
+        d.w = yw > 0.f ? d.w * a : 0.f;
+        s1.x += d.x; s1.y += d.y; s1.z += d.z; s1.w += d.w;
+        s2.x += d.x * hx; s2.y += d.y * hy; s2.z += d.z * hz; s2.w += d.w * hw;
+    }
+    red[ry * c4 + j] = s1;
+    red[(rl + ry) * c4 + j] = s2;
+    __syncthreads();
+    if (ry != 0) return;
+    float4 t1 = make_float4(0.f, 0.f, 0.f, 0.f), t2 = t1;
+    for (int gq = 0; gq < rl; ++gq) {
+        const float4 a = red[gq * c4 + j], bq = red[(rl + gq) * c4 + j];
+        t1.x += a.x; t1.y += a.y; t1.z += a.z; t1.w += a.w;
+        t2.x += bq.x; t2.y += bq.y; t2.z += bq.z; t2.w += bq.w;
+    }
+    float *p = partial + (size_t)blockIdx.x * 2 * c;
+    *reinterpret_cast<float4 *>(p + 4 * j) = t1;
+    *reinterpret_cast<float4 *>(p + c + 4 * j) = t2;
+}
+
+__global__ void bn_gated_bwd_apply_kernel(const float *__restrict__ gy, int ld_g4, const float *__restrict__ x,
+                                          const float *__restrict__ att, int64_t total4, int c4, float inv_n,
+                                          const float *__restrict__ mean, const float *__restrict__ invstd,
+                                          const float *__restrict__ gamma, const float *__restrict__ beta,
+                                          const float *__restrict__ dbeta, const float *__restrict__ dgamma,
+                                          float *__restrict__ dx) {
+    int64_t t = (int64_t)blockIdx.x * blockDim.x + threadIdx.x;
+    if (t >= total4) return;
+    const int jj = (int)(t % c4), j = jj * 4;
+    const int64_t row = t / c4;
+    const float a = att[row];
+    float4 v = ld4(x, t);
+    float4 d = ld4(gy, row * ld_g4 + jj);
+    float4 m = *reinterpret_cast<const float4 *>(mean + j);
+    float4 is = *reinterpret_cast<const float4 *>(invstd + j);
+    float4 g = gamma ? *reinterpret_cast<const float4 *>(gamma + j) : make_float4(1.f, 1.f, 1.f, 1.f);
+    float4 b = beta ? *reinterpret_cast<const float4 *>(beta + j) : make_float4(0.f, 0.f, 0.f, 0.f);
+    float4 db = *reinterpret_cast<const float4 *>(dbeta + j);
+    float4 dg = *reinterpret_cast<const float4 *>(dgamma + j);
+    float hx = (v.x - m.x) * is.x, hy = (v.y - m.y) * is.y, hz = (v.z - m.z) * is.z, hw = (v.w - m.w) * is.w;
+    d.x = hx * g.x + b.x > 0.f ? d.x * a : 0.f;
+    d.y = hy * g.y + b.y > 0.f ? d.y * a : 0.f;
+    d.z = hz * g.z + b.z > 0.f ? d.z * a : 0.f;
+    d.w = hw * g.w + b.w > 0.f ? d.w * a : 0.f;
+    float4 o;
+    o.x = g.x * is.x * (d.x - db.x * inv_n - hx * dg.x * inv_n);
+    o.y = g.y * is.y * (d.y - db.y * inv_n - hy * dg.y * inv_n);
+    o.z = g.z * is.z * (d.z - db.z * inv_n - hz * dg.z * inv_n);
+    o.w = g.w * is.w * (d.w - db.w * inv_n - hw * dg.w * inv_n);
+    st4(dx, t, o);
+}
+
+constexpr int kBnEndTile = 64;
+__global__ void __launch_bounds__(256)
+bn_apply_rows_nchw_kernel(const float *__restrict__ u, int64_t m_total, int c, int hw, const float *__restrict__ mean,
+                          const float *__restrict__ invstd, const float *__restrict__ gamma, const float *__restrict__ beta,
+                          float *__restrict__ fused_nchw, float *__restrict__ relu_nchw, float *__restrict__ fused_rows) {
+    __shared__ float tile[kBnEndTile][kBnEndTile + 1];
+    const int64_t m0 = (int64_t)blockIdx.x * kBnEndTile;
+    const int c0 = blockIdx.y * kBnEndTile;
+    const int tx = threadIdx.x & 63, ty = threadIdx.x >> 6;
+#pragma unroll
+    for (int pass = 0; pass < 4; ++pass) {
+        const int e = threadIdx.x + pass * 256, r = e >> 4, q = e & 15;
+        const int ch = c0 + 4 * q;
+        const int64_t mm = m0 + r;
+        if (ch < c && mm < m_total) {
+            const float4 v = *reinterpret_cast<const float4 *>(u + mm * c + ch);
+            const float4 m = *reinterpret_cast<const float4 *>(mean + ch);
+            const float4 is = *reinterpret_cast<const float4 *>(invstd + ch);
+            const float4 g = gamma ? *reinterpret_cast<const float4 *>(gamma + ch) : make_float4(1.f, 1.f, 1.f, 1.f);
+            const float4 b = beta ? *reinterpret_cast<const float4 *>(beta + ch) : make_float4(0.f, 0.f, 0.f, 0.f);
+            float4 o;
+            o.x = (v.x - m.x) * is.x * g.x + b.x;
+            o.y = (v.y - m.y) * is.y * g.y + b.y;
+            o.z = (v.z - m.z) * is.z * g.z + b.z;
+            o.w = (v.w - m.w) * is.w * g.w + b.w;
+            *reinterpret_cast<float4 *>(fused_rows + mm * c + ch) = o;
+            tile[r][4 * q] = o.x; tile[r][4 * q + 1] = o.y; tile[r][4 * q + 2] = o.z; tile[r][4 * q + 3] = o.w;
+        }
+    }
+    __syncthreads();
+#pragma unroll
+    for (int k = 0; k < kBnEndTile; k += 4) {
+        const int ch = c0 + ty + k;
+        const int64_t mm = m0 + tx;
+        if (ch < c && mm < m_total) {
+            const int64_t img = mm / hw;
+            const int64_t i = (img * c + ch) * hw + (mm - img * hw);
+            const float v = tile[tx][ty + k];
+            fused_nchw[i] = v;
+            relu_nchw[i] = fmaxf(v, 0.f);
+        }
+    }
+}
+
 __global__ void bn_invstd_kernel(const float *__restrict__ var, int c, float eps, float *__restrict__ invstd) {
     int ch = blockIdx.x * blockDim.x + threadIdx.x;
     if (ch < c) invstd[ch] = 1.f / sqrtf(var[ch] + eps);
@@ -619,6 +769,8 @@
     return check_launch("u2mkd_bn_backward_apply");
 }
 
+static bool bn_gated_width_ok(int c) { return c == 4 || c == 8 || c == 16 || c == 32 || c == 64 || c == 128 || c == 256; }
+
 }
 
 using namespace u2mkd;
@@ -686,6 +838,61 @@
                                    dbeta, F32W(dx), F32W(dres), s);
 }
 
+int u2mkd_bn_gated_train_forward(const float *x, const float *att, int64_t n, int32_t c, const float *gamma, const float *beta,
+                                 float eps, float momentum, float *running_mean, float *running_var,
+                                 int64_t *num_batches_tracked, float *partial, float *mean, float *invstd, float *y, int32_t ld_y,
+                                 u2mkd_stream_t s) {
+    U2_REQUIRE(bn_gated_width_ok(c), "u2mkd_bn_gated_train_forward: c=%d must be a power of two in 4..256", c);
+    U2_REQUIRE(n > 1 && x && att && partial && mean && invstd && y && ld_y >= c && ld_y % 4 == 0,
+               "u2mkd_bn_gated_train_forward: bad arguments (n=%lld, ld_y=%d)", (long long)n, ld_y);
+    hipStream_t st = as_stream(s);
+    const int nslab = (int)u2mkd_bn_num_slabs(n);
+    bn_launch_stats_partial<float>(st, nslab, x, n, c, partial);
+    hipLaunchKernelGGL(bn_stats_finalize_kernel, dim3((unsigned)ceil_div(c, kBnFinCh)), dim3(256), 0, st, partial, nslab, n, c,
+                       eps, momentum, running_mean, running_var, mean, invstd, (float *)nullptr, num_batches_tracked);
+    const int64_t total4 = n * (c / 4);
+    hipLaunchKernelGGL(bn_gated_apply_kernel, dim3((unsigned)ceil_div(total4, 256)), dim3(256), 0, st, x, att, total4, c / 4, mean,
+                       invstd, gamma, beta, y, ld_y / 4);
+    return check_launch("u2mkd_bn_gated_train_forward");
+}
+
+int u2mkd_bn_gated_backward(const float *gy, int32_t ld_g, const float *x, const float *att, int64_t n, int32_t c,
+                            const float *mean, const float *invstd, const float *gamma, const float *beta, float *partial,
+                            float *dgamma, float *dbeta, float *dx, float *datt, u2mkd_stream_t s) {
+    U2_REQUIRE(bn_gated_width_ok(c), "u2mkd_bn_gated_backward: c=%d must be a power of two in 4..256", c);
+    U2_REQUIRE(n > 0 && gy && x && att && mean && invstd && partial && dgamma && dbeta && dx && datt && ld_g >= c && ld_g % 4 == 0,
+               "u2mkd_bn_gated_backward: bad arguments (n=%lld, ld_g=%d)", (long long)n, ld_g);
+    hipStream_t st = as_stream(s);
+    const int nslab = (int)u2mkd_bn_num_slabs(n);
+    hipLaunchKernelGGL(bn_gated_bwd_partial_kernel, dim3(nslab), dim3(kBnThreads), bn_lds_bytes(c, 2), st, gy, ld_g / 4, x, att, n,
+                       c, mean, invstd, gamma, beta, partial, datt);
+    hipLaunchKernelGGL(bn_bwd_finalize_kernel, dim3((unsigned)ceil_div(c, kBnFinCh)), dim3(256), 0, st, partial, nslab, c, dbeta,
+                       dgamma, (float *)nullptr);
+    const int64_t total4 = n * (c / 4);
+    hipLaunchKernelGGL(bn_gated_bwd_apply_kernel, dim3((unsigned)ceil_div(total4, 256)), dim3(256), 0, st, gy, ld_g / 4, x, att,
+                       total4, c / 4, 1.f / (float)n, mean, invstd, gamma, beta, dbeta, dgamma, dx);
+    return check_launch("u2mkd_bn_gated_backward");
+}
+
+int u2mkd_bn_train_forward_rows_nchw(const float *u, int32_t n_img, int64_t hw, int32_t c, const float *gamma, const float *beta,
+                                     float eps, float momentum, float *running_mean, float *running_var,
+                                     int64_t *num_batches_tracked, float *partial, float *mean, float *invstd, float *fused_nchw,
+                                     float *relu_nchw, float *fused_rows, u2mkd_stream_t s) {
+    U2_REQUIRE(c > 0 && c % 4 == 0 && c <= 1024, "u2mkd_bn_train_forward_rows_nchw: c=%d must be a multiple of 4 in 4..1024", c);
+    const int64_t n = (int64_t)n_img * hw;
+    U2_REQUIRE(n_img > 0 && hw > 0 && hw < ((int64_t)1 << 31) && n > 1 && ceil_div(n, kBnEndTile) < ((int64_t)1 << 31),
+               "u2mkd_bn_train_forward_rows_nchw: %d maps of %lld pixels", n_img, (long long)hw);
+    U2_REQUIRE(u && partial && mean && invstd && fused_nchw && relu_nchw && fused_rows, "u2mkd_bn_train_forward_rows_nchw: null pointer");
+    hipStream_t st = as_stream(s);
+    const int nslab = (int)u2mkd_bn_num_slabs(n);
+    bn_launch_stats_partial<float>(st, nslab, u, n, c, partial);
+    hipLaunchKernelGGL(bn_stats_finalize_kernel, dim3((unsigned)ceil_div(c, kBnFinCh)), dim3(256), 0, st, partial, nslab, n, c,
+                       eps, momentum, running_mean, running_var, mean, invstd, (float *)nullptr, num_batches_tracked);
+    hipLaunchKernelGGL(bn_apply_rows_nchw_kernel, dim3((unsigned)ceil_div(n, kBnEndTile), (unsigned)ceil_div(c, kBnEndTile)), dim3(256),
+                       0, st, u, n, c, (int)hw, mean, invstd, gamma, beta, fused_nchw, relu_nchw, fused_rows);
+    return check_launch("u2mkd_bn_train_forward_rows_nchw");
+}
+
 int u2mkd_bn_local_stats(const void *x, int32_t row_dtype, int64_t n, int32_t c, float *partial, float *stats,
                          u2mkd_stream_t s) {
     U2_ROW_DTYPE("u2mkd_bn_local_stats");
diff --git a/u2mkd_amd/csrc/l2c_block.hip b/u2mkd_amd/csrc/l2c_block.hip
--- /dev/null
+++ b/u2mkd_amd/csrc/l2c_block.hip
@@ -0,0 +1,253 @@
+#include "common.h"
+
+namespace u2mkd {
+
+constexpr int kGateThreads = 256;
+constexpr int kGateSlabRows = 256;
+constexpr int kGateFinLanes = 64, kGateFinCh = 4;
+
+__device__ __forceinline__ float row_lanes_sum(float v, int lanes) {
+    for (int o = lanes >> 1; o >= 1; o >>= 1) v += __shfl_xor(v, o, kWave);
+    return v;
+}
+
+__device__ __forceinline__ float4 gate_tanh(const float4 a, const float4 b, const float4 ba, const float4 bb) {
+    return make_float4(tanhf(a.x + b.x + (ba.x + bb.x)), tanhf(a.y + b.y + (ba.y + bb.y)), tanhf(a.z + b.z + (ba.z + bb.z)),
+                       tanhf(a.w + b.w + (ba.w + bb.w)));
+}
+
+__global__ void __launch_bounds__(kGateThreads)
+l2c_gate_fwd_kernel(const float4 *__restrict__ h1, const float4 *__restrict__ h2, const float4 *__restrict__ b1,
+                    const float4 *__restrict__ b2, const float4 *__restrict__ w3, const float *__restrict__ b3, int64_t m,
+                    int rc4, float *__restrict__ att) {
+    const int64_t t = (int64_t)blockIdx.x * kGateThreads + threadIdx.x;
+    const bool live = t < m * rc4;
+    const int j = (int)(t % rc4);
+    float p = 0.f;
+    if (live) {
+        const float4 th = gate_tanh(h1[t], h2[t], b1[j], b2[j]), w = w3[j];
+        p = w.x * th.x + w.y * th.y + w.z * th.z + w.w * th.w;
+    }
+    p = row_lanes_sum(p, rc4);
+    if (live && j == 0) att[t / rc4] = 1.f / (1.f + expf(-(p + *b3)));
+}
+
+__global__ void __launch_bounds__(kGateThreads)
+l2c_gate_bwd_kernel(const float *__restrict__ datt, const float *__restrict__ att, const float4 *__restrict__ h1,
+                    const float4 *__restrict__ h2, const float4 *__restrict__ b1, const float4 *__restrict__ b2,
+                    const float4 *__restrict__ w3, int64_t m, int rc4, float4 *__restrict__ dh, float *__restrict__ partial) {
+    __shared__ float4 red[2][kGateThreads];
+    __shared__ float redq[kGateThreads];
+    const int rl = kGateThreads / rc4;
+    const int j = threadIdx.x % rc4, ry = threadIdx.x / rc4;
+    const int64_t r0 = (int64_t)blockIdx.x * kGateSlabRows;
+    const int rows = (int)min((int64_t)kGateSlabRows, m - r0);
+    const float4 ba = b1[j], bb = b2[j], w = w3[j];
+    float4 sw = make_float4(0.f, 0.f, 0.f, 0.f), sb = sw;
+    float sq = 0.f;
+    for (int rr = ry; rr < rows; rr += rl) {
+        const int64_t row = r0 + rr, t = row * rc4 + j;
+        const float a = att[row], q = datt[row] * a * (1.f - a);
+        const float4 th = gate_tanh(h1[t], h2[t], ba, bb);
+        const float4 d = make_float4(q * w.x * (1.f - th.x * th.x), q * w.y * (1.f - th.y * th.y), q * w.z * (1.f - th.z * th.z),
+                                     q * w.w * (1.f - th.w * th.w));
+        dh[t] = d;
+        sw.x += q * th.x; sw.y += q * th.y; sw.z += q * th.z; sw.w += q * th.w;
+        sb.x += d.x; sb.y += d.y; sb.z += d.z; sb.w += d.w;
+        sq += q;
+    }
+    red[0][ry * rc4 + j] = sw;
+    red[1][ry * rc4 + j] = sb;
+    redq[threadIdx.x] = sq;
+    __syncthreads();
+    if (ry != 0) return;
+    float4 tw = make_float4(0.f, 0.f, 0.f, 0.f), tb = tw;
+    float tq = 0.f;
+    for (int g = 0; g < rl; ++g) {
+        const float4 x = red[0][g * rc4 + j], y = red[1][g * rc4 + j];
+        tw.x += x.x; tw.y += x.y; tw.z += x.z; tw.w += x.w;
+        tb.x += y.x; tb.y += y.y; tb.z += y.z; tb.w += y.w;
+        tq += redq[g * rc4];
+    }
+    float *p = partial + (size_t)blockIdx.x * (8 * rc4 + 4);
+    *reinterpret_cast<float4 *>(p + 4 * j) = tw;
+    *reinterpret_cast<float4 *>(p + 4 * rc4 + 4 * j) = tb;
+    if (j == 0) p[8 * rc4] = tq;
+}
+
+__global__ void __launch_bounds__(kGateFinLanes * kGateFinCh)
+l2c_gate_bwd_finalize_kernel(const float *__restrict__ partial, int nslab, int nval, int stride, int rc, float *__restrict__ sums) {
+    __shared__ float s_v[kGateFinLanes][kGateFinCh];
+    const int cl = threadIdx.x & (kGateFinCh - 1), g = threadIdx.x / kGateFinCh;
+    const int k = blockIdx.x * kGateFinCh + cl;
+    float v = 0.f;
+    if (k < nval)
+        for (int b = g; b < nslab; b += kGateFinLanes) v += partial[(size_t)b * stride + k];
+    s_v[g][cl] = v;
+    __syncthreads();
+    if (g != 0 || k >= nval) return;
+    for (int i = 1; i < kGateFinLanes; ++i) v += s_v[i][cl];
+    if (k < 2 * rc) sums[k] = v;
+    if (k >= rc) sums[k + rc] = v;
+}
+
+constexpr int kEndTile = 64;
+
+__device__ __forceinline__ int64_t nchw_index(int64_t m, int ch, int c, int hw) {
+    const int64_t img = m / hw;
+    return (img * c + ch) * hw + (m - img * hw);
+}
+
+__global__ void __launch_bounds__(256)
+l2c_nchw_to_rows_kernel(const float *__restrict__ a, const float *__restrict__ b, const float *__restrict__ mask,
+                        const float *__restrict__ add, int64_t m_total, int c, int hw, float *__restrict__ out1, int ld1,
+                        float *__restrict__ out2, int ld2) {
+    __shared__ float tile[kEndTile][kEndTile + 1];
+    const int64_t m0 = (int64_t)blockIdx.x * kEndTile;
+    const int c0 = blockIdx.y * kEndTile;
+    const int tx = threadIdx.x & 63, ty = threadIdx.x >> 6;
+#pragma unroll
+    for (int k = 0; k < kEndTile; k += 4) {
+        const int ch = c0 + ty + k;
+        const int64_t m = m0 + tx;
+        if (ch < c && m < m_total) {
+            const int64_t i = nchw_index(m, ch, c, hw);
+            float v = a ? a[i] : 0.f;
+            if (b) v += (mask && !(mask[i] > 0.f)) ? 0.f : b[i];
+            tile[tx][ty + k] = v;
+        }
+    }
+    __syncthreads();
+#pragma unroll
+    for (int pass = 0; pass < 4; ++pass) {
+        const int e = threadIdx.x + pass * 256, r = e >> 4, q = e & 15;
+        const int ch = c0 + 4 * q;
+        const int64_t m = m0 + r;
+        if (ch < c && m < m_total) {
+            float4 v = make_float4(tile[r][4 * q], tile[r][4 * q + 1], tile[r][4 * q + 2], tile[r][4 * q + 3]);
+            if (add) {
+                const float4 g = *reinterpret_cast<const float4 *>(add + m * c + ch);
+                v.x += g.x; v.y += g.y; v.z += g.z; v.w += g.w;
+            }
+            *reinterpret_cast<float4 *>(out1 + m * ld1 + ch) = v;
+            if (out2) *reinterpret_cast<float4 *>(out2 + m * ld2 + ch) = v;
+        }
+    }
+}
+
+__global__ void __launch_bounds__(256)
+l2c_rows_to_nchw_kernel(const float *__restrict__ a, int lda, const float *__restrict__ b, int ldb, int64_t m_total, int c,
+                        int hw, float *__restrict__ out) {
+    __shared__ float tile[kEndTile][kEndTile + 1];
+    const int64_t m0 = (int64_t)blockIdx.x * kEndTile;
+    const int c0 = blockIdx.y * kEndTile;
+    const int tx = threadIdx.x & 63, ty = threadIdx.x >> 6;
+#pragma unroll
+    for (int pass = 0; pass < 4; ++pass) {
+        const int e = threadIdx.x + pass * 256, r = e >> 4, q = e & 15;
+        const int ch = c0 + 4 * q;
+        const int64_t m = m0 + r;
+        if (ch < c && m < m_total) {
+            float4 v = a ? *reinterpret_cast<const float4 *>(a + m * lda + ch) : make_float4(0.f, 0.f, 0.f, 0.f);
+            if (b) {
+                const float4 g = *reinterpret_cast<const float4 *>(b + m * ldb + ch);
+                v.x += g.x; v.y += g.y; v.z += g.z; v.w += g.w;
+            }
+            tile[r][4 * q] = v.x; tile[r][4 * q + 1] = v.y; tile[r][4 * q + 2] = v.z; tile[r][4 * q + 3] = v.w;
+        }
+    }
+    __syncthreads();
+#pragma unroll
+    for (int k = 0; k < kEndTile; k += 4) {
+        const int ch = c0 + ty + k;
+        const int64_t m = m0 + tx;
+        if (ch < c && m < m_total) out[nchw_index(m, ch, c, hw)] = tile[tx][ty + k];
+    }
+}
+
+static bool gate_width_ok(int rc) { return rc == 4 || rc == 8 || rc == 16 || rc == 32 || rc == 64; }
+
+static bool ends_shape_ok(int64_t n_img, int c, int64_t hw) {
+    return n_img > 0 && hw > 0 && c > 0 && c % 4 == 0 && hw < ((int64_t)1 << 31) && ceil_div(c, kEndTile) <= 65535 &&
+           ceil_div(n_img * hw, kEndTile) < ((int64_t)1 << 31);
+}
+
+}
+
+using namespace u2mkd;
+
+extern "C" {
+
+int u2mkd_l2c_gate_forward(const float *h1, const float *h2, const float *b1, const float *b2, const float *w3, const float *b3,
+                           int64_t m, int32_t rc, float *att, u2mkd_stream_t s) {
+    U2_REQUIRE(gate_width_ok(rc), "u2mkd_l2c_gate_forward: hidden width %d must be 4, 8, 16, 32 or 64", rc);
+    if (m == 0) return 0;
+    U2_REQUIRE(m > 0 && h1 && h2 && b1 && b2 && w3 && b3 && att, "u2mkd_l2c_gate_forward: bad arguments");
+    const int rc4 = rc / 4;
+    hipLaunchKernelGGL(l2c_gate_fwd_kernel, dim3((unsigned)ceil_div(m * rc4, kGateThreads)), dim3(kGateThreads), 0, as_stream(s),
+                       reinterpret_cast<const float4 *>(h1), reinterpret_cast<const float4 *>(h2),
+                       reinterpret_cast<const float4 *>(b1), reinterpret_cast<const float4 *>(b2),
+                       reinterpret_cast<const float4 *>(w3), b3, m, rc4, att);
+    return check_launch("u2mkd_l2c_gate_forward");
+}
+
+int64_t u2mkd_l2c_gate_partial_floats(int64_t m, int32_t rc) {
+    return m > 0 ? ceil_div(m, kGateSlabRows) * (2 * (int64_t)rc + 4) : 0;
+}
+
+int u2mkd_l2c_gate_backward(const float *datt, const float *att, const float *h1, const float *h2, const float *b1,
+                            const float *b2, const float *w3, int64_t m, int32_t rc, float *partial, float *dh, float *sums,
+                            u2mkd_stream_t s) {
+    U2_REQUIRE(gate_width_ok(rc), "u2mkd_l2c_gate_backward: hidden width %d must be 4, 8, 16, 32 or 64", rc);
+    U2_REQUIRE(m > 0 && datt && att && h1 && h2 && b1 && b2 && w3 && partial && dh && sums, "u2mkd_l2c_gate_backward: bad arguments");
+    const int rc4 = rc / 4;
+    const int64_t nslab = ceil_div(m, kGateSlabRows);
+    U2_REQUIRE(nslab < ((int64_t)1 << 31), "u2mkd_l2c_gate_backward: too many rows");
+    hipStream_t st = as_stream(s);
+    hipLaunchKernelGGL(l2c_gate_bwd_kernel, dim3((unsigned)nslab), dim3(kGateThreads), 0, st, datt, att,
+                       reinterpret_cast<const float4 *>(h1), reinterpret_cast<const float4 *>(h2),
+                       reinterpret_cast<const float4 *>(b1), reinterpret_cast<const float4 *>(b2),
+                       reinterpret_cast<const float4 *>(w3), m, rc4, reinterpret_cast<float4 *>(dh), partial);
+    const int nval = 2 * rc + 1;
+    hipLaunchKernelGGL(l2c_gate_bwd_finalize_kernel, dim3((unsigned)ceil_div(nval, kGateFinCh)), dim3(kGateFinLanes * kGateFinCh), 0,
+                       st, partial, (int)nslab, nval, 2 * rc + 4, rc, sums);
+    return check_launch("u2mkd_l2c_gate_backward");
+}
+
+int u2mkd_l2c_image_in(const float *img, int32_t n_img, int32_t c, int64_t hw, float *rows, float *cat, int32_t ld_cat,
+                       u2mkd_stream_t s) {
+    U2_REQUIRE(ends_shape_ok(n_img, c, hw) && img && rows && (cat == nullptr || (ld_cat >= c && ld_cat % 4 == 0)),
+               "u2mkd_l2c_image_in: bad arguments");
+    const int64_t m = (int64_t)n_img * hw;
+    hipLaunchKernelGGL(l2c_nchw_to_rows_kernel, dim3((unsigned)ceil_div(m, kEndTile), (unsigned)ceil_div(c, kEndTile)), dim3(256), 0,
+                       as_stream(s), img, (const float *)nullptr, (const float *)nullptr, (const float *)nullptr, m, c, (int)hw,
+                       rows, c, cat, ld_cat);
+    return check_launch("u2mkd_l2c_image_in");
+}
+
+int u2mkd_l2c_image_in_backward(const float *g_rows, const float *g_cat, int32_t ld_cat, int32_t n_img, int32_t c, int64_t hw,
+                                float *g_img, u2mkd_stream_t s) {
+    U2_REQUIRE(ends_shape_ok(n_img, c, hw) && (g_rows || g_cat) && g_img && (g_cat == nullptr || (ld_cat >= c && ld_cat % 4 == 0)),
+               "u2mkd_l2c_image_in_backward: bad arguments");
+    const int64_t m = (int64_t)n_img * hw;
+    hipLaunchKernelGGL(l2c_rows_to_nchw_kernel, dim3((unsigned)ceil_div(m, kEndTile), (unsigned)ceil_div(c, kEndTile)), dim3(256), 0,
+                       as_stream(s), g_rows, c, g_cat, ld_cat, m, c, (int)hw, g_img);
+    return check_launch("u2mkd_l2c_image_in_backward");
+}
+
+int u2mkd_l2c_grad_in(const float *g_skip, const float *g_x_im, const float *fused, const float *g_rows, int32_t n_img, int32_t c,
+                      int64_t hw, float *dy_rows, u2mkd_stream_t s) {
+    U2_REQUIRE(ends_shape_ok(n_img, c, hw) && dy_rows && (g_x_im == nullptr || fused), "u2mkd_l2c_grad_in: bad arguments");
+    const int64_t m = (int64_t)n_img * hw;
+    hipStream_t st = as_stream(s);
+    if (!g_skip && !g_x_im) {
+        if (g_rows) (void)hipMemcpyAsync(dy_rows, g_rows, (size_t)m * c * sizeof(float), hipMemcpyDeviceToDevice, st);
+        else (void)hipMemsetAsync(dy_rows, 0, (size_t)m * c * sizeof(float), st);
+        return check_launch("u2mkd_l2c_grad_in");
+    }
+    hipLaunchKernelGGL(l2c_nchw_to_rows_kernel, dim3((unsigned)ceil_div(m, kEndTile), (unsigned)ceil_div(c, kEndTile)), dim3(256), 0,
+                       st, g_skip, g_x_im, fused, g_rows, m, c, (int)hw, dy_rows, c, (float *)nullptr, 0);
+    return check_launch("u2mkd_l2c_grad_in");
+}
+
+}
diff --git a/u2mkd_amd/csrc/pixhead.hip b/u2mkd_amd/csrc/pixhead.hip
--- a/u2mkd_amd/csrc/pixhead.hip
+++ b/u2mkd_amd/csrc/pixhead.hip
@@ -145,7 +145,7 @@
 }
 
 __global__ void __launch_bounds__(256)
-l2c_combine_rows_kernel(L2cGrids G, int n_img, int H, int W, int c4, float4 *__restrict__ out) {
+l2c_combine_rows_kernel(L2cGrids G, int n_img, int H, int W, int c4, float4 *__restrict__ out, float scale = 1.f) {
     const int64_t t = (int64_t)blockIdx.x * 256 + threadIdx.x;
     if (t >= (int64_t)n_img * H * W * c4) return;
     const int c = (int)(t % c4);
@@ -168,7 +168,7 @@
         acc.z += w00 * a.z + w01 * b.z + w10 * d.z + w11 * e.z;
         acc.w += w00 * a.w + w01 * b.w + w10 * d.w + w11 * e.w;
     }
-    out[t] = acc;
+    out[t] = make_float4(acc.x * scale, acc.y * scale, acc.z * scale, acc.w * scale);
 }
 
 __global__ void __launch_bounds__(256)
@@ -444,25 +444,39 @@
 
 static float l2c_ratio(int n_src, int n_dst) { return n_dst > 1 ? (float)(n_src - 1) / (float)(n_dst - 1) : 0.f; }
 
-int u2mkd_l2c_combine_forward(const float *g0, const float *g1, const float *g2, const float *g3, int32_t n_grids, int32_t n_img,
-                              int32_t h, int32_t w, int32_t c, int32_t ch1, int32_t cw1, int32_t ch2, int32_t cw2, int32_t ch3,
-                              int32_t cw3, float *out_rows, u2mkd_stream_t s) {
+static int l2c_combine_launch(const char *who, const float *g0, const float *g1, const float *g2, const float *g3, int32_t n_grids,
+                              int32_t n_img, int32_t h, int32_t w, int32_t c, int32_t ch1, int32_t cw1, int32_t ch2, int32_t cw2,
+                              int32_t ch3, int32_t cw3, float scale, float *out_rows, u2mkd_stream_t s) {
     U2_REQUIRE(n_grids >= 1 && n_grids <= 4 && c > 0 && c % 4 == 0 && n_img > 0 && h > 0 && w > 0,
-               "u2mkd_l2c_combine_forward: %d grids of %d channels (1..4 grids, channels a multiple of 4)", n_grids, c);
-    U2_REQUIRE(g0 && out_rows && (n_grids < 2 || g1) && (n_grids < 3 || g2) && (n_grids < 4 || g3), "u2mkd_l2c_combine_forward: null pointer");
+               "%s: %d grids of %d channels (1..4 grids, channels a multiple of 4)", who, n_grids, c);
+    U2_REQUIRE(g0 && out_rows && (n_grids < 2 || g1) && (n_grids < 3 || g2) && (n_grids < 4 || g3), "%s: null pointer", who);
     L2cGrids G;
     const float *gp[4] = {g0, g1, g2, g3};
     const int chs[4] = {h, ch1, ch2, ch3}, cws[4] = {w, cw1, cw2, cw3};
     for (int i = 0; i < 4; ++i) {
         G.g[i] = gp[i]; G.ch[i] = chs[i]; G.cw[i] = cws[i];
         G.ry[i] = l2c_ratio(chs[i], h); G.rx[i] = l2c_ratio(cws[i], w);
-        U2_REQUIRE(i >= n_grids || (chs[i] > 0 && cws[i] > 0 && chs[i] <= h && cws[i] <= w), "u2mkd_l2c_combine_forward: grid %d is %dx%d", i, chs[i], cws[i]);
+        U2_REQUIRE(i >= n_grids || (chs[i] > 0 && cws[i] > 0 && chs[i] <= h && cws[i] <= w), "%s: grid %d is %dx%d", who, i, chs[i], cws[i]);
     }
     G.n = n_grids;
     const int64_t total = (int64_t)n_img * h * w * (c / 4);
     hipLaunchKernelGGL(l2c_combine_rows_kernel, dim3((unsigned)ceil_div(total, 256)), dim3(256), 0, as_stream(s), G, n_img, h, w,
-                       c / 4, reinterpret_cast<float4 *>(out_rows));
-    return check_launch("u2mkd_l2c_combine_forward");
+                       c / 4, reinterpret_cast<float4 *>(out_rows), scale);
+    return check_launch(who);
+}
+
+int u2mkd_l2c_combine_forward(const float *g0, const float *g1, const float *g2, const float *g3, int32_t n_grids, int32_t n_img,
+                              int32_t h, int32_t w, int32_t c, int32_t ch1, int32_t cw1, int32_t ch2, int32_t cw2, int32_t ch3,
+                              int32_t cw3, float *out_rows, u2mkd_stream_t s) {
+    return l2c_combine_launch("u2mkd_l2c_combine_forward", g0, g1, g2, g3, n_grids, n_img, h, w, c, ch1, cw1, ch2, cw2, ch3, cw3, 1.f,
+                              out_rows, s);
+}
+
+int u2mkd_l2c_combine_forward_scaled(const float *g0, const float *g1, const float *g2, const float *g3, int32_t n_grids,
+                                     int32_t n_img, int32_t h, int32_t w, int32_t c, int32_t ch1, int32_t cw1, int32_t ch2,
+                                     int32_t cw2, int32_t ch3, int32_t cw3, float scale, float *out_rows, u2mkd_stream_t s) {
+    return l2c_combine_launch("u2mkd_l2c_combine_forward_scaled", g0, g1, g2, g3, n_grids, n_img, h, w, c, ch1, cw1, ch2, cw2, ch3,
+                              cw3, scale, out_rows, s);
 }
 
 int u2mkd_l2c_combine_backward(const float *g_rows, int32_t n_img, int32_t h, int32_t w, int32_t c, int32_t ch, int32_t cw,
diff --git a/u2mkd_amd/fusion.py b/u2mkd_amd/fusion.py
--- a/u2mkd_amd/fusion.py
+++ b/u2mkd_amd/fusion.py
@@ -7,7 +7,7 @@
 from .camera import BatchNorm2d, bn_act
 
 __all__ = ['IA_Layer', 'Atten_Fusion_Conv', 'L2CAILayer', 'L2CFusion', 'feature_gather', 'c2l_gather',
-           'l2c_scatter', 'feature_fetch', 'l2c_scatter_torch', 'c2l_gather_torch']
+           'l2c_scatter', 'l2c_fuse', 'feature_fetch', 'l2c_scatter_torch', 'c2l_gather_torch']
 
 
 def _rows_linear(x, weight, bias, before=None):
@@ -85,6 +85,171 @@
         l2c = self.l2c_ai_layer(img_features, point_features)
         fused = self.bn1(self.conv1(torch.cat([img_features, l2c], dim=1)))
         return F.relu(fused), fused
+
+    def rows_ok(self, pts, img):
+        ai = self.l2c_ai_layer
+        bns = (ai.conv1[1], self.bn1)
+        return (self.training and torch.is_grad_enabled() and not torch.is_autocast_enabled()
+                and all(type(b) is BatchNorm2d and b.training and b.momentum is not None and b.track_running_stats for b in bns)
+                and img.is_cuda and pts.is_cuda and img.dtype == torch.float32 and pts.dtype == torch.float32
+                and img.dim() == 4 and img.is_contiguous() and img.shape[1] == ai.ic and pts.dim() == 2
+                and pts.shape[1] == ai.pc and ai.ic in (16, 32, 64, 128, 256) and ai.pc % 4 == 0
+                and img.shape[0] * img.shape[2] * img.shape[3] > 1)
+
+    def forward_rows(self, pts_rows, img):
+        from .torchsparse.nn import functional as spf
+        ai = self.l2c_ai_layer
+        n_img, ic, h, w = img.shape
+        rc, pc = ai.fc1.out_channels, ai.pc
+        img_rows, cat = _L2cImageIn.apply(img)
+        h1 = spf.linear(img_rows, ai.fc1.weight.view(rc, ic))
+        h2 = spf.linear(pts_rows, ai.fc2.weight.view(rc, pc))
+        att = _L2cGate.apply(h1, h2, ai.fc1.bias, ai.fc2.bias, ai.fc3.weight.view(rc), ai.fc3.bias)
+        t = spf.linear(pts_rows, ai.conv1[0].weight.view(ic, pc), ai.conv1[0].bias, bias_feeds_batchnorm=True)
+        cat = _L2cGatedBN.apply(t, att, cat, ai.conv1[1].weight, ai.conv1[1].bias, ai.conv1[1])
+        u = spf.linear(cat, self.conv1.weight.view(ic, 2 * ic), self.conv1.bias, bias_feeds_batchnorm=True)
+        return _L2cBnOut.apply(u, self.bn1.weight, self.bn1.bias, self.bn1, n_img, h, w)
+
+
+def _bn_track(bn):
+    return float(bn.momentum), bn.running_mean, bn.running_var, bn.num_batches_tracked
+
+
+def _bn_partial(n, c, device):
+    from . import _lib as L
+    return torch.empty(max(L.load().u2mkd_bn_num_slabs(n), 1) * 2 * c, dtype=torch.float32, device=device)
+
+
+class _L2cImageIn(torch.autograd.Function):
+
+    @staticmethod
+    def forward(ctx, img):
+        from . import _lib as L
+        n_img, c, h, w = img.shape
+        ctx.shape = img.shape
+        ctx.set_materialize_grads(False)
+        rows = torch.empty(n_img * h * w, c, dtype=torch.float32, device=img.device)
+        cat = torch.empty(n_img * h * w, 2 * c, dtype=torch.float32, device=img.device)
+        L.call('u2mkd_l2c_image_in', L.ptr(img), n_img, c, h * w, L.ptr(rows), L.ptr(cat), 2 * c, L.stream())
+        return rows, cat
+
+    @staticmethod
+    @torch.autograd.function.once_differentiable
+    def backward(ctx, g_rows, g_cat):
+        from . import _lib as L
+        n_img, c, h, w = ctx.shape
+        if g_rows is None and g_cat is None:
+            return None
+        g_rows = g_rows.contiguous() if g_rows is not None else None
+        g_cat = g_cat.contiguous() if g_cat is not None else None
+        ref = g_rows if g_rows is not None else g_cat
+        g_img = torch.empty(n_img, c, h, w, dtype=torch.float32, device=ref.device)
+        L.call('u2mkd_l2c_image_in_backward', L.ptr(g_rows), L.ptr(g_cat), 2 * c, n_img, c, h * w, L.ptr(g_img), L.stream())
+        return g_img
+
+
+class _L2cGate(torch.autograd.Function):
+
+    @staticmethod
+    def forward(ctx, h1, h2, b1, b2, w3, b3):
+        from . import _lib as L
+        m, rc = h1.shape
+        h1, h2 = h1.contiguous(), h2.contiguous()
+        att = torch.empty(m, dtype=torch.float32, device=h1.device)
+        L.call('u2mkd_l2c_gate_forward', L.ptr(h1), L.ptr(h2), L.ptr(b1), L.ptr(b2), L.ptr(w3), L.ptr(b3), m, rc, L.ptr(att), L.stream())
+        ctx.save_for_backward(h1, h2, b1, b2, w3, att)
+        return att
+
+    @staticmethod
+    @torch.autograd.function.once_differentiable
+    def backward(ctx, datt):
+        from . import _lib as L
+        h1, h2, b1, b2, w3, att = ctx.saved_tensors
+        m, rc = h1.shape
+        datt = datt.contiguous()
+        partial = torch.empty(L.load().u2mkd_l2c_gate_partial_floats(m, rc), dtype=torch.float32, device=h1.device)
+        dh = torch.empty_like(h1)
+        sums = torch.empty(3 * rc + 1, dtype=torch.float32, device=h1.device)
+        L.call('u2mkd_l2c_gate_backward', L.ptr(datt), L.ptr(att), L.ptr(h1), L.ptr(h2), L.ptr(b1), L.ptr(b2), L.ptr(w3), m, rc,
+               L.ptr(partial), L.ptr(dh), L.ptr(sums), L.stream())
+        return dh, dh, sums[rc:2 * rc], sums[2 * rc:3 * rc], sums[:rc], sums[3 * rc:]
+
+
+class _L2cGatedBN(torch.autograd.Function):
+
+    @staticmethod
+    def forward(ctx, t, att, cat, gamma, beta, bn):
+        from . import _lib as L
+        n, c = t.shape
+        t = t.contiguous()
+        momentum, rm, rv, counter = _bn_track(bn)
+        mean = torch.empty(c, dtype=torch.float32, device=t.device)
+        invstd = torch.empty_like(mean)
+        L.call('u2mkd_bn_gated_train_forward', L.ptr(t), L.ptr(att), n, c, L.ptr(gamma), L.ptr(beta), float(bn.eps), momentum,
+               L.ptr(rm), L.ptr(rv), L.ptr(counter), L.ptr(_bn_partial(n, c, t.device)), L.ptr(mean), L.ptr(invstd),
+               cat.data_ptr() + 4 * c, 2 * c, L.stream())
+        torch._C._increment_version([b for b in (rm, rv, counter) if b is not None])
+        ctx.mark_dirty(cat)
+        ctx.save_for_backward(t, att, gamma, beta, mean, invstd)
+        return cat
+
+    @staticmethod
+    @torch.autograd.function.once_differentiable
+    def backward(ctx, g):
+        from . import _lib as L
+        t, att, gamma, beta, mean, invstd = ctx.saved_tensors
+        n, c = t.shape
+        g = g.contiguous()
+        dgamma = torch.empty(c, dtype=torch.float32, device=t.device)
+        dbeta = torch.empty_like(dgamma)
+        dt = torch.empty_like(t)
+        datt = torch.empty_like(att)
+        L.call('u2mkd_bn_gated_backward', g.data_ptr() + 4 * c, 2 * c, L.ptr(t), L.ptr(att), n, c, L.ptr(mean), L.ptr(invstd),
+               L.ptr(gamma), L.ptr(beta), L.ptr(_bn_partial(n, c, t.device)), L.ptr(dgamma), L.ptr(dbeta), L.ptr(dt), L.ptr(datt),
+               L.stream())
+        return dt, datt, g, (dgamma if gamma is not None else None), (dbeta if beta is not None else None), None
+
+
+class _L2cBnOut(torch.autograd.Function):
+
+    @staticmethod
+    def forward(ctx, u, gamma, beta, bn, n_img, h, w):
+        from . import _lib as L
+        n, c = u.shape
+        u = u.contiguous()
+        momentum, rm, rv, counter = _bn_track(bn)
+        mean = torch.empty(c, dtype=torch.float32, device=u.device)
+        invstd = torch.empty_like(mean)
+        x_im = torch.empty(n_img, c, h, w, dtype=torch.float32, device=u.device)
+        skip = torch.empty_like(x_im)
+        skip_rows = torch.empty_like(u)
+        L.call('u2mkd_bn_train_forward_rows_nchw', L.ptr(u), n_img, h * w, c, L.ptr(gamma), L.ptr(beta), float(bn.eps), momentum,
+               L.ptr(rm), L.ptr(rv), L.ptr(counter), L.ptr(_bn_partial(n, c, u.device)), L.ptr(mean), L.ptr(invstd), L.ptr(skip),
+               L.ptr(x_im), L.ptr(skip_rows), L.stream())
+        torch._C._increment_version([b for b in (rm, rv, counter) if b is not None])
+        ctx.set_materialize_grads(False)
+        ctx.save_for_backward(u, gamma, beta, mean, invstd, skip)
+        ctx.maps = (n_img, h, w)
+        return x_im, skip, skip_rows
+
+    @staticmethod
+    @torch.autograd.function.once_differentiable
+    def backward(ctx, g_x_im, g_skip, g_rows):
+        from . import _lib as L
+        u, gamma, beta, mean, invstd, skip = ctx.saved_tensors
+        n, c = u.shape
+        n_img, h, w = ctx.maps
+        if g_x_im is None and g_skip is None and g_rows is None:
+            return None, None, None, None, None, None, None
+        g_x_im, g_skip, g_rows = (g.contiguous() if g is not None else None for g in (g_x_im, g_skip, g_rows))
+        dy = torch.empty_like(u)
+        L.call('u2mkd_l2c_grad_in', L.ptr(g_skip), L.ptr(g_x_im), L.ptr(skip), L.ptr(g_rows), n_img, c, h * w, L.ptr(dy), L.stream())
+        dgamma = torch.empty(c, dtype=torch.float32, device=u.device)
+        dbeta = torch.empty_like(dgamma)
+        du = torch.empty_like(u)
+        L.call('u2mkd_bn_backward', L.ptr(dy), L.ptr(u), None, 0, n, c, L.ptr(mean), L.ptr(invstd), L.ptr(gamma), L.ptr(beta), 0, 1,
+               L.ptr(_bn_partial(n, c, u.device)), L.ptr(dgamma), L.ptr(dbeta), L.ptr(du), None, L.stream())
+        return du, (dgamma if gamma is not None else None), (dbeta if beta is not None else None), None, None, None, None
 
 
 def feature_gather(feature_map, xy, mode='bilinear'):
@@ -197,13 +362,14 @@
             l2c_plan(pixel_coordinates, masks, ch, cw)
 
 
-def c2l_gather(feature_maps, pixel_coordinates, masks):
+def c2l_gather(feature_maps, pixel_coordinates, masks, rows=None):
     from . import _lib
     _lib.require_cuda(feature_maps)
     from .torchsparse.nn import functional as spf
     B, ncam, C, h, w = feature_maps.shape
     idx8, w8 = c2l_plan(pixel_coordinates, masks, h, w)
-    rows = _NchwToRows.apply(feature_maps)
+    if rows is None:
+        rows = _NchwToRows.apply(feature_maps)
     if C % 4:
         rows = F.pad(rows, (0, 4 - C % 4))
     return spf.spdevoxelize(rows, idx8, w8)[:, :C]
@@ -355,16 +521,68 @@
         return (None, None) + tuple(grads)
 
 
-def l2c_scatter(point_feats, pixel_coordinates, masks, ifh, ifw, n_scales):
+class _L2cCombineRows(torch.autograd.Function):
+
+    @staticmethod
+    def forward(ctx, n_img, sizes, *grids):
+        from . import _lib as L
+        n = len(grids)
+        (h, w), c = sizes[0], grids[0].shape[1]
+        ctx.meta = (n_img, sizes, c)
+        rows = torch.empty(n_img * h * w, c, dtype=torch.float32, device=grids[0].device)
+        gp = [L.ptr(g) for g in grids] + [None] * (4 - n)
+        dims = [v for s in list(sizes[1:]) + [(0, 0)] * (4 - n) for v in s]
+        L.call('u2mkd_l2c_combine_forward_scaled', *gp, n, n_img, h, w, c, *dims, 1.0 / n, L.ptr(rows), L.stream())
+        return rows
+
+    @staticmethod
+    @torch.autograd.function.once_differentiable
+    def backward(ctx, g):
+        from . import _lib as L
+        n_img, sizes, c = ctx.meta
+        h, w = sizes[0]
+        g_rows = g * (1.0 / len(sizes))
+        grads = [g_rows]
+        for ch, cw in sizes[1:]:
+            d = torch.empty(n_img * ch * cw, c, dtype=torch.float32, device=g.device)
+            L.call('u2mkd_l2c_combine_backward', L.ptr(g_rows), n_img, h, w, c, ch, cw, L.ptr(d), L.stream())
+            grads.append(d)
+        return (None, None) + tuple(grads)
+
+
+_L2C_ROWS = os.environ.get('U2MKD_L2C_ROWS', '1') != '0'
+
+
+def l2c_fuse(block, piece, point_feats, img, pixel_coordinates, masks, n_scales):
+    from . import graphs
+    ifh, ifw = img.shape[-2:]
+    if _L2C_ROWS and not graphs.graphs_enabled():
+        pts_rows = l2c_scatter(point_feats, pixel_coordinates, masks, ifh, ifw, n_scales, rows_for=(block, img))
+        if pts_rows is not None:
+            return block.forward_rows(pts_rows, img)
+    x_im, skip = piece(l2c_scatter(point_feats, pixel_coordinates, masks, ifh, ifw, n_scales), img)
+    return x_im, skip, None
+
+
+def l2c_scatter(point_feats, pixel_coordinates, masks, ifh, ifw, n_scales, rows_for=None):
     from . import _lib
     _lib.require_cuda(point_feats)
     if point_feats.shape[1] % 4:
+        if rows_for is not None:
+            return None
         return l2c_scatter_torch(point_feats, pixel_coordinates, masks, ifh, ifw, n_scales)
     from .torchsparse.nn import functional as spf
     B, ncam, C = len(masks), masks[0].shape[0], point_feats.shape[1]
     sizes = list(_l2c_grids(ifh, ifw, n_scales))
-    if (_L2C_COMBINE and point_feats.dtype == torch.float32 and spf.row_dtype() is None and 1 <= n_scales <= 4 and B * ncam <= 65535
-            and sizes[0] == (ifh, ifw)):
+    combine = (_L2C_COMBINE and point_feats.dtype == torch.float32 and spf.row_dtype() is None and 1 <= n_scales <= 4
+               and B * ncam <= 65535 and sizes[0] == (ifh, ifw))
+    if rows_for is not None:
+        block, img = rows_for
+        if not (combine and img.shape[0] == B * ncam and tuple(img.shape[-2:]) == (ifh, ifw) and block.rows_ok(point_feats, img)):
+            return None
+        grids = [_SegmentMap.apply(point_feats, *l2c_plan(pixel_coordinates, masks, ch, cw)).float() for ch, cw in sizes]
+        return grids[0] if len(grids) == 1 else _L2cCombineRows.apply(B * ncam, tuple(sizes), *grids)
+    if combine:
         grids = [_SegmentMap.apply(point_feats, *l2c_plan(pixel_coordinates, masks, ch, cw)) for ch, cw in sizes]
         if all(g.dtype == torch.float32 for g in grids):
             return _L2cCombine.apply(B * ncam, tuple(sizes), *grids)
diff --git a/u2mkd_amd/kd.py b/u2mkd_amd/kd.py
--- a/u2mkd_amd/kd.py
+++ b/u2mkd_amd/kd.py
@@ -9,7 +9,7 @@
 from . import torchsparse
 from .camera import BNReluConv, SwiftNetRes18
 from .graphs import PieceCache, StaticPiece
-from .fusion import Atten_Fusion_Conv, L2CFusion, c2l_gather, feature_fetch, l2c_scatter
+from .fusion import Atten_Fusion_Conv, L2CFusion, c2l_gather, feature_fetch, l2c_fuse
 from .pixel_head import sampled_head_applies, sampled_pixel_logits
 from .lidar.blocks import (BasicConvolutionBlock, BasicDeconvolutionBlock, FusedSequential, PointBatchNorm1d, PointLinear,
                            ResidualBlock)
@@ -209,12 +209,12 @@
             _, ifc, ifh, ifw = skip.shape
             self._fusion_shapes.setdefault((ih, iw), {})[idx] = (ifh, ifw, n_stage - idx)
 
-            l2c_feat_map = l2c_scatter(pts_feat.F, pixel_coordinates, masks, ifh, ifw, n_stage - idx)
-            x_im, skip = self._piece('l2c%d' % idx)(l2c_feat_map, skip)
+            x_im, skip, skip_rows = l2c_fuse(self.l2c_fusion_blocks[idx], self._piece('l2c%d' % idx), pts_feat.F, skip,
+                                             pixel_coordinates, masks, n_stage - idx)
             x_im_ready = fork.mark()
             img_feats.append(skip)
 
-            img_feat_tensor = c2l_gather(skip.view(ib, ncam, ifc, ifh, ifw), pixel_coordinates, masks)
+            img_feat_tensor = c2l_gather(skip.view(ib, ncam, ifc, ifh, ifw), pixel_coordinates, masks, rows=skip_rows)
             pseudo = self.learner[idx](pts_feat.F)
             img_feat_tensor, mse = _select_and_mse(img_feat_tensor, pseudo, fov_mask)
             mse_loss.append(mse)
```
